# safijari/yag-slam

Hardware: AMD Instinct MI355X
Metric: pose hypotheses/sec (higher is better)
Workload: dtype u8

## Files before the change

include/yagmatch.h:

```cpp
#ifndef YAGMATCH_H
#define YAGMATCH_H

#include <stdint.h>

#ifdef __cplusplus
extern "C" {
#endif

#define YM_VERSION 1

enum {
    YM_OK = 0,
    YM_ERR_INVALID = -1,
    YM_ERR_NO_DEVICE = -2,
    YM_ERR_HIP = -3,
    YM_ERR_UNSUPPORTED = -4,
    YM_ERR_RANGE = -5,
    YM_ERR_BUSY = -6
};

enum { YM_SEM_KARTO = 0, YM_SEM_YAGPY = 1 };

typedef struct ym_config {
    double angle_variance_penalty;
// ... 11 lines not shown
    int32_t semantics;
} ym_config;

typedef struct ym_scan_desc {
    const double *ranges;
    int32_t n;
    int32_t reserved;
    double min_angle;
    double max_angle;
    double angle_increment;
    double min_range;
    double max_range;
    double range_threshold;
    double pose[3];
} ym_scan_desc;

typedef struct ym_result {
    double response;
    double pose[3];
    double cov[9];
    double coarse_response;
    int64_t hypotheses;
    int32_t coarse_dims[3];
    int32_t fine_dims[3];
    int32_t n_query_points;
    int32_t expansions;
    int32_t status;
    int32_t reserved;
} ym_result;

typedef struct ym_matcher ym_matcher;
typedef struct ym_scan ym_scan;

int ym_version(void);
const char *ym_build_id(void);
int ym_device_count(void);
const char *ym_last_error(void);

ym_matcher *ym_create(const ym_config *cfg, int device);
void ym_destroy(ym_matcher *m);
int ym_get_config(const ym_matcher *m, ym_config *out);
int ym_set_stream(ym_matcher *m, void *hip_stream);
int ym_synchronize(ym_matcher *m);

ym_scan *ym_scan_create(int device, const ym_scan_desc *desc);
int ym_scans_create(int device, const ym_scan_desc *descs, int n, ym_scan **out);
void ym_scans_destroy(ym_scan *const *scans, int n);
int ym_scan_set_pose(ym_scan *s, double x, double y, double heading);
int ym_scans_set_poses(ym_scan *const *scans, const double *xyz, int n);
int ym_scan_get_pose(const ym_scan *s, double pose[3]);
int ym_scan_size(const ym_scan *s);
int ym_scan_structure_trusted(const ym_scan *s, int semantics);
void ym_scan_destroy(ym_scan *s);

int ym_match(ym_matcher *m, const ym_scan_desc *query, const ym_scan_desc *base, int n_base,
             int penalize, int refine, ym_result *out);
int ym_match_scans(ym_matcher *m, const ym_scan *query, const ym_scan *const *base, int n_base,
                   int penalize, int refine, ym_result *out);

int ym_map_sequence(ym_matcher *m, ym_scan *const *scans, const double *odom, int n, int start, int buffer_len,
                    int penalize, int refine, int device_chain, ym_result *results, int32_t *n_done);

int ym_process_scan(ym_matcher *m, ym_scan *query, ym_scan *const *chain, int n_chain, const double *odom_last,
                    const double *odom_query, int penalize, int refine, ym_result *result);

int ym_sequence_stats(const ym_matcher *m, int64_t *segments, int64_t *faults, int64_t *sync_steps);

int ym_async_slots(const ym_matcher *m);
int ym_match_scans_async(ym_matcher *m, const ym_scan *query, const ym_scan *const *base, int n_base,
                         int penalize, int refine, int slot);
int ym_wait(ym_matcher *m, int slot, ym_result *out);

int ym_match_batch(ym_matcher *m, const ym_scan *query, const ym_scan *const *scans,
                   const int32_t *chain_offsets, int n_chains, int penalize, int refine,
                   ym_result *per_chain, ym_result *best, int32_t *best_chain);

typedef struct ym_batch ym_batch;
ym_batch *ym_batch_create(ym_matcher *m, const ym_scan *query, const ym_scan *const *scans,
                          const int32_t *chain_offsets, int n_chains);
void ym_batch_destroy(ym_batch *b);
int ym_batch_size(const ym_batch *b);
int ym_batch_run_async(ym_matcher *m, const ym_batch *b, int penalize, int refine, int slot,
                       int64_t chain_id_base, void *dev_best_out);
int ym_batch_wait(ym_matcher *m, int slot, ym_result *per_chain, ym_result *best, int32_t *best_chain);

int ym_match_pairs(ym_matcher *m, const ym_scan *const *queries, const ym_scan *const *scans,
                   const int32_t *chain_offsets, int n_items, int penalize, int refine, ym_result *per_item);
ym_batch *ym_pairs_create(ym_matcher *m, const ym_scan *const *queries, const ym_scan *const *scans,
                          const int32_t *chain_offsets, int n_items);

int ym_coarse_dims(const ym_matcher *m, int32_t dims[3]);
int ym_match_slice_begin(ym_matcher *m, const ym_scan *query, const ym_scan *const *base, int n_base, int penalize,
                         int refine, int k_begin, int k_end, double *dev_resp, double *dev_probs);
int ym_match_slice_finish(ym_matcher *m, ym_result *out);

typedef struct ym_map ym_map;
ym_map *ym_map_from_occupancy(ym_matcher *m, const uint8_t *image, int width, int height, int pitch, int occupied_value);
ym_map *ym_map_from_grid(ym_matcher *m, const double *cgrid, int width, int height);
int ym_map_size(const ym_map *map, int *width, int *height);
int ym_map_read(const ym_map *map, double *out, int64_t out_count);
void ym_map_destroy(ym_map *map);
typedef struct ym_map_search {
    double xy_search, xy_step;
    double angle_search, angle_step;
    double grid_resolution;
    int32_t penalize;
    int32_t reserved;
} ym_map_search;
int ym_match_map(ym_matcher *m, const ym_map *map, double ox, double oy, const ym_scan *const *queries, int n_queries,
                 int penalize, int refine, const ym_map_search *coarse, ym_result *out);

typedef struct ym_occupancy ym_occupancy;
typedef struct ym_occupancy_info {
    int32_t width, height;
    double offset_x, offset_y, resolution;
} ym_occupancy_info;
ym_occupancy *ym_occupancy_create(const ym_scan *const *scans, int n_scans, double resolution, double range_threshold);
int ym_occupancy_get_info(const ym_occupancy *og, ym_occupancy_info *info);
int ym_occupancy_read(const ym_occupancy *og, uint8_t *image, int64_t image_bytes);
void ym_occupancy_destroy(ym_occupancy *og);

typedef struct ym_raymap ym_raymap;
ym_raymap *ym_raymap_create(int device, const uint8_t *image, int width, int height, int pitch);
int ym_raymap_trace(ym_raymap *rm, const double *starts_xy, int n_starts, const double *dir_cs, int n_angles, float *end_xy,
                    double *length, int64_t *capped);
int ym_raymap_trace_each(ym_raymap *rm, const double *starts_xy, int n_starts, const double *dir_cs, int n_angles, float *end_xy,
                         double *length, int64_t *capped);
void ym_raymap_destroy(ym_raymap *rm);

typedef struct ym_segments ym_segments;
ym_segments *ym_segments_create(int device, const int32_t *labels, int width, int height, int pitch_elems);
int ym_segments_label_range(const ym_segments *sg, int32_t *min_label, int32_t *max_label);
int ym_segments_stats(ym_segments *sg, int n_labels, int64_t *count, int64_t *sum_x, int64_t *sum_y);
int ym_segments_boundaries(ym_segments *sg, uint8_t *mask, int64_t mask_bytes);
int ym_segments_pairs(ym_segments *sg, int table_slots, int cap, int32_t *pairs , int32_t *counts, int64_t *first_index,
                      int32_t *n_pairs);
void ym_segments_destroy(ym_segments *sg);

typedef struct ym_grid_info {
    int32_t width, height, pitch;
    int32_t origin_x, origin_y;
    int32_t storage_w, storage_h;
    int32_t roi_x, roi_y, roi_w, roi_h;
    double offset_x, offset_y;
} ym_grid_info;
int ym_debug_grid_info(ym_matcher *m, int item, ym_grid_info *info);
int ym_debug_grid(ym_matcher *m, int item, uint8_t *out, int64_t out_bytes);
int ym_debug_sums(ym_matcher *m, int item, int pass, uint32_t *out, int64_t out_count);
int ym_debug_query_local(ym_matcher *m, int item, double *out_xy, int32_t cap, int32_t *n);
int ym_debug_cells(ym_matcher *m, int item, int32_t *out, int64_t out_count, int32_t *max_n);

int ym_debug_option(ym_matcher *m, int option, int value);

#define YM_DEBUG_COUNTERS 8
int ym_debug_counters(ym_matcher *m, int64_t *out, int32_t count);

int ym_debug_stamps(ym_matcher *m, int enable, uint64_t *out, int32_t count);

int ym_profile_enable(ym_matcher *m, int on);
int ym_profile_read(ym_matcher *m, int which, double *ms_total, int64_t *launches, int reset);
int ym_cache_stats(const ym_matcher *m, int64_t *hits, int64_t *misses);

#ifdef __cplusplus
}
#endif
#endif
```

yag_slam_amd/_capi.py:

```python
import ctypes as C
import os
import subprocess

_HERE = os.path.dirname(os.path.abspath(__file__))
LIB_PATH = os.environ.get("YM_LIB_PATH") or os.path.join(_HERE, "libyagmatch.so")

YM_OK = 0
SEM = {"karto": 0, "yagpy": 1}

EXPORTS = (
    "ym_version", "ym_build_id", "ym_device_count", "ym_last_error", "ym_create", "ym_destroy", "ym_get_config",
    "ym_set_stream", "ym_synchronize", "ym_scan_create", "ym_scans_create", "ym_scans_destroy", "ym_scan_set_pose", "ym_scans_set_poses", "ym_scan_get_pose",
    "ym_scan_size", "ym_scan_structure_trusted", "ym_scan_destroy", "ym_match", "ym_match_scans", "ym_map_sequence", "ym_process_scan", "ym_sequence_stats", "ym_async_slots",
    "ym_match_scans_async", "ym_wait", "ym_match_batch", "ym_batch_create", "ym_batch_destroy", "ym_batch_size",
    "ym_match_pairs", "ym_pairs_create",
    "ym_batch_run_async", "ym_batch_wait", "ym_debug_grid_info",
    "ym_debug_grid", "ym_debug_sums", "ym_debug_query_local", "ym_debug_cells", "ym_debug_option", "ym_debug_stamps",
    "ym_profile_enable",
    "ym_profile_read", "ym_cache_stats", "ym_debug_counters",
    "ym_coarse_dims", "ym_match_slice_begin", "ym_match_slice_finish",
    "ym_occupancy_create", "ym_occupancy_get_info", "ym_occupancy_read", "ym_occupancy_destroy",
    "ym_map_from_occupancy", "ym_map_from_grid", "ym_map_size", "ym_map_read", "ym_map_destroy", "ym_match_map",
    "ym_raymap_create", "ym_raymap_trace", "ym_raymap_trace_each", "ym_raymap_destroy",
    "ym_segments_create", "ym_segments_label_range", "ym_segments_stats", "ym_segments_boundaries", "ym_segments_pairs",
    "ym_segments_destroy",
)


class YmError(RuntimeError):
    def __init__(self, code, msg):
        super().__init__("libyagmatch error %d: %s" % (code, msg))
        self.code = code


class YmConfig(C.Structure):
    _fields_ = [
        ("angle_variance_penalty", C.c_double),
        ("distance_variance_penalty", C.c_double),
        ("coarse_search_angle_offset", C.c_double),
        ("coarse_angle_resolution", C.c_double),
        ("fine_search_angle_resolution", C.c_double),
        ("range_threshold", C.c_double),
        ("minimum_angle_penalty", C.c_double),
        ("minimum_distance_penalty", C.c_double),
        ("search_size", C.c_double),
        ("resolution", C.c_double),
        ("smear_deviation", C.c_double),
        ("use_response_expansion", C.c_int32),
        ("semantics", C.c_int32),
    ]


class YmScanDesc(C.Structure):
    _fields_ = [
        ("ranges", C.POINTER(C.c_double)),
        ("n", C.c_int32),
        ("reserved", C.c_int32),
        ("min_angle", C.c_double),
        ("max_angle", C.c_double),
        ("angle_increment", C.c_double),
        ("min_range", C.c_double),
        ("max_range", C.c_double),
        ("range_threshold", C.c_double),
        ("pose", C.c_double * 3),
    ]


class YmResult(C.Structure):
    _fields_ = [
        ("response", C.c_double),
        ("pose", C.c_double * 3),
        ("cov", C.c_double * 9),
        ("coarse_response", C.c_double),
        ("hypotheses", C.c_int64),
        ("coarse_dims", C.c_int32 * 3),
        ("fine_dims", C.c_int32 * 3),
        ("n_query_points", C.c_int32),
        ("expansions", C.c_int32),
        ("status", C.c_int32),
        ("reserved", C.c_int32),
    ]


class YmOccupancyInfo(C.Structure):
    _fields_ = [("width", C.c_int32), ("height", C.c_int32), ("offset_x", C.c_double), ("offset_y", C.c_double),
                ("resolution", C.c_double)]


class YmMapSearch(C.Structure):
    _fields_ = [("xy_search", C.c_double), ("xy_step", C.c_double), ("angle_search", C.c_double), ("angle_step", C.c_double),
                ("grid_resolution", C.c_double), ("penalize", C.c_int32), ("reserved", C.c_int32)]


class YmGridInfo(C.Structure):
    _fields_ = [(n, C.c_int32) for n in ("width", "height", "pitch", "origin_x", "origin_y", "storage_w",
                                        "storage_h", "roi_x", "roi_y", "roi_w", "roi_h")] + [
        ("pad", C.c_int32), ("offset_x", C.c_double), ("offset_y", C.c_double)]


_lib = None


def build(verbose=False):
    cmd = ["make", "-C", os.path.join(_HERE, "csrc")]
    if not verbose:
        cmd.insert(1, "-s")
    subprocess.check_call(cmd)
    return LIB_PATH


def _share_hip_runtime_with_torch():
    import importlib.util
    import sys
    if "torch" in sys.modules or os.environ.get("YM_SKIP_TORCH_PRELOAD"):
        return
    if importlib.util.find_spec("torch") is not None:
        import torch


def lib():
    global _lib
    if _lib is not None:
        return _lib
    if not os.path.exists(LIB_PATH):
        build()
    _share_hip_runtime_with_torch()
    L = C.CDLL(LIB_PATH)
    vp, ip, dp = C.c_void_p, C.POINTER(C.c_int32), C.POINTER(C.c_double)
    L.ym_version.restype = C.c_int
    L.ym_device_count.restype = C.c_int
    L.ym_last_error.restype = C.c_char_p
    L.ym_build_id.restype = C.c_char_p
    L.ym_create.restype = vp
    L.ym_create.argtypes = [C.POINTER(YmConfig), C.c_int]
    L.ym_destroy.argtypes = [vp]
    L.ym_destroy.restype = None
    L.ym_get_config.argtypes = [vp, C.POINTER(YmConfig)]
    L.ym_set_stream.argtypes = [vp, vp]
    L.ym_synchronize.argtypes = [vp]
    L.ym_scan_create.restype = vp
    L.ym_scan_create.argtypes = [C.c_int, C.POINTER(YmScanDesc)]
    L.ym_scan_set_pose.argtypes = [vp, C.c_double, C.c_double, C.c_double]
    L.ym_scans_set_poses.argtypes = [C.POINTER(vp), dp, C.c_int]
    L.ym_scan_get_pose.argtypes = [vp, dp]
    L.ym_scan_size.argtypes = [vp]
    L.ym_scan_destroy.argtypes = [vp]
    L.ym_scans_create.argtypes = [C.c_int, vp, C.c_int, vp]
    L.ym_scans_destroy.argtypes = [vp, C.c_int]
    L.ym_scans_destroy.restype = None
    L.ym_scan_destroy.restype = None
    L.ym_match.argtypes = [vp, C.POINTER(YmScanDesc), C.POINTER(YmScanDesc), C.c_int, C.c_int, C.c_int,
                           C.POINTER(YmResult)]
    L.ym_match_scans.argtypes = [vp, vp, C.POINTER(vp), C.c_int, C.c_int, C.c_int, C.POINTER(YmResult)]
    L.ym_async_slots.argtypes = [vp]
    L.ym_match_scans_async.argtypes = [vp, vp, C.POINTER(vp), C.c_int, C.c_int, C.c_int, C.c_int]
    L.ym_wait.argtypes = [vp, C.c_int, C.POINTER(YmResult)]
    L.ym_match_batch.argtypes = [vp, vp, C.POINTER(vp), ip, C.c_int, C.c_int, C.c_int, C.POINTER(YmResult),
                                 C.POINTER(YmResult), ip]
    L.ym_batch_create.restype = vp
    L.ym_batch_create.argtypes = [vp, vp, C.POINTER(vp), ip, C.c_int]
    L.ym_pairs_create.restype = vp
    L.ym_pairs_create.argtypes = [vp, C.POINTER(vp), C.POINTER(vp), ip, C.c_int]
    L.ym_match_pairs.argtypes = [vp, C.POINTER(vp), C.POINTER(vp), ip, C.c_int, C.c_int, C.c_int, C.POINTER(YmResult)]
    L.ym_batch_destroy.argtypes = [vp]
    L.ym_batch_destroy.restype = None
    L.ym_batch_size.argtypes = [vp]
    L.ym_batch_run_async.argtypes = [vp, vp, C.c_int, C.c_int, C.c_int, C.c_int64, vp]
    L.ym_batch_wait.argtypes = [vp, C.c_int, C.POINTER(YmResult), C.POINTER(YmResult), ip]
    L.ym_debug_grid_info.argtypes = [vp, C.c_int, C.POINTER(YmGridInfo)]
    L.ym_debug_grid.argtypes = [vp, C.c_int, C.POINTER(C.c_uint8), C.c_int64]
    L.ym_debug_sums.argtypes = [vp, C.c_int, C.c_int, C.POINTER(C.c_uint32), C.c_int64]
    L.ym_debug_query_local.argtypes = [vp, C.c_int, dp, C.c_int32, ip]
    L.ym_debug_cells.argtypes = [vp, C.c_int, ip, C.c_int64, ip]
    L.ym_debug_option.argtypes = [vp, C.c_int, C.c_int]
    L.ym_debug_stamps.argtypes = [vp, C.c_int, C.POINTER(C.c_uint64), C.c_int32]
    L.ym_profile_enable.argtypes = [vp, C.c_int]
    L.ym_profile_read.argtypes = [vp, C.c_int, dp, C.POINTER(C.c_int64), C.c_int]
    L.ym_cache_stats.argtypes = [vp, C.POINTER(C.c_int64), C.POINTER(C.c_int64)]
    L.ym_debug_counters.argtypes = [vp, C.POINTER(C.c_int64), C.c_int32]
    L.ym_coarse_dims.argtypes = [vp, ip]
    L.ym_scan_structure_trusted.argtypes = [vp, C.c_int]
    L.ym_process_scan.argtypes = [vp, vp, C.POINTER(vp), C.c_int, dp, dp, C.c_int, C.c_int, C.POINTER(YmResult)]
    L.ym_sequence_stats.argtypes = [vp, C.POINTER(C.c_int64), C.POINTER(C.c_int64), C.POINTER(C.c_int64)]
    L.ym_map_sequence.argtypes = [vp, C.POINTER(vp), dp, C.c_int, C.c_int, C.c_int, C.c_int, C.c_int, C.c_int, C.POINTER(YmResult), ip]
    L.ym_match_slice_begin.argtypes = [vp, vp, C.POINTER(vp), C.c_int, C.c_int, C.c_int, C.c_int, C.c_int, vp, vp]
    L.ym_match_slice_finish.argtypes = [vp, C.POINTER(YmResult)]
    L.ym_occupancy_create.restype = vp
    L.ym_occupancy_create.argtypes = [C.POINTER(vp), C.c_int, C.c_double, C.c_double]
    L.ym_occupancy_get_info.argtypes = [vp, C.POINTER(YmOccupancyInfo)]
    L.ym_occupancy_read.argtypes = [vp, C.POINTER(C.c_uint8), C.c_int64]
    L.ym_occupancy_destroy.argtypes = [vp]
    L.ym_occupancy_destroy.restype = None
    L.ym_map_from_occupancy.restype = vp
    L.ym_map_from_occupancy.argtypes = [vp, C.POINTER(C.c_uint8), C.c_int, C.c_int, C.c_int, C.c_int]
    L.ym_map_from_grid.restype = vp
    L.ym_map_from_grid.argtypes = [vp, dp, C.c_int, C.c_int]
    L.ym_map_size.argtypes = [vp, ip, ip]
    L.ym_map_read.argtypes = [vp, dp, C.c_int64]
    L.ym_map_destroy.argtypes = [vp]
    L.ym_map_destroy.restype = None
    L.ym_match_map.argtypes = [vp, vp, C.c_double, C.c_double, C.POINTER(vp), C.c_int, C.c_int, C.c_int, C.POINTER(YmMapSearch),
                               C.POINTER(YmResult)]
    L.ym_raymap_create.restype = vp
    L.ym_raymap_create.argtypes = [C.c_int, C.POINTER(C.c_uint8), C.c_int, C.c_int, C.c_int]
    L.ym_raymap_trace.argtypes = [vp, dp, C.c_int, dp, C.c_int, C.POINTER(C.c_float), dp, C.POINTER(C.c_int64)]
    L.ym_raymap_trace_each.argtypes = [vp, dp, C.c_int, dp, C.c_int, C.POINTER(C.c_float), dp, C.POINTER(C.c_int64)]
    L.ym_raymap_destroy.argtypes = [vp]
    L.ym_raymap_destroy.restype = None
    lp = C.POINTER(C.c_int64)
    L.ym_segments_create.restype = vp
    L.ym_segments_create.argtypes = [C.c_int, ip, C.c_int, C.c_int, C.c_int]
    L.ym_segments_label_range.argtypes = [vp, ip, ip]
    L.ym_segments_stats.argtypes = [vp, C.c_int, lp, lp, lp]
    L.ym_segments_boundaries.argtypes = [vp, C.POINTER(C.c_uint8), C.c_int64]
    L.ym_segments_pairs.argtypes = [vp, C.c_int, C.c_int, ip, ip, lp, ip]
    L.ym_segments_destroy.argtypes = [vp]
    L.ym_segments_destroy.restype = None
    _lib = L
    return L


def build_id():
    return lib().ym_build_id().decode()


def check(rc):
    if rc != YM_OK:
        raise YmError(rc, lib().ym_last_error().decode(errors="replace"))
    return rc


def last_error():
    return lib().ym_last_error().decode(errors="replace")


def config_struct(cfg, semantics="karto"):
    d = cfg if isinstance(cfg, dict) else cfg.as_dict()
    c = YmConfig()
    for name, _ in YmConfig._fields_:
        if name == "semantics":
            c.semantics = SEM[semantics] if isinstance(semantics, str) else int(semantics)
        elif name == "use_response_expansion":
            c.use_response_expansion = int(bool(d["use_response_expansion"]))
        elif name == "minimum_distance_penalty":
            c.minimum_distance_penalty = float(d.get("minimum_distance_penalty", 0.5))
        else:
            setattr(c, name, float(d[name]))
    return c
```

yag_slam_amd/csrc/ym_abi_debug.hpp:

```cpp
int ym_debug_grid_info(ym_matcher *m, int item, ym_grid_info *info) {
    if (!m || !info) return set_err(YM_ERR_INVALID, "null argument");
    if (!m->last_valid || item < 0 || item >= m->last_B) return set_err(YM_ERR_INVALID, "no such item in the last call");
    const YmGeom &g = m->last_geom;
    info->width = g.win_w; info->height = g.win_w; info->pitch = g.pitch;
    info->origin_x = g.win_origin; info->origin_y = g.win_origin;
    info->storage_w = g.storage_w; info->storage_h = g.storage_w;
    info->roi_x = g.border; info->roi_y = g.border; info->roi_w = g.roi_w; info->roi_h = g.roi_w;
    YmItemState s;
    DEV_GUARD(m->device);
    HIP_TRY(hipStreamSynchronize(m->stream));
    HIP_TRY(hipMemcpy(&s, m->states.p + item, sizeof s, hipMemcpyDeviceToHost));
    info->offset_x = s.off_x; info->offset_y = s.off_y;
    return YM_OK;
}

int ym_debug_grid(ym_matcher *m, int item, uint8_t *out, int64_t out_bytes) {
    if (!m || !out) return set_err(YM_ERR_INVALID, "null argument");
    if (!m->last_valid || item < 0 || item >= m->last_B) return set_err(YM_ERR_INVALID, "no such item in the last call");
    const int64_t need = (int64_t)m->last_geom.pitch * m->last_geom.win_w;
    if (out_bytes < need) return set_err(YM_ERR_INVALID, "grid buffer too small: need %lld bytes", (long long)need);
    DEV_GUARD(m->device);
    HIP_TRY(hipStreamSynchronize(m->stream));
    HIP_TRY(hipMemcpy(out, m->grid.p + (size_t)item * m->last_grid_stride, (size_t)need, hipMemcpyDeviceToHost));
    return YM_OK;
}

int ym_debug_sums(ym_matcher *m, int item, int pass, uint32_t *out, int64_t out_count) {
    if (!m || !out || pass < 0 || pass > 1) return set_err(YM_ERR_INVALID, "bad argument");
    if (!m->last_valid || item < 0 || item >= m->last_B) return set_err(YM_ERR_INVALID, "no such item in the last call");
    const size_t n = m->last_sums_stride[pass];
    if (n == 0) return set_err(YM_ERR_INVALID, "pass %d did not run", pass);
    const size_t ncopy = std::min(n, (size_t)out_count);
    if (m->cfg.semantics == YM_SEM_KARTO && (size_t)out_count < n)
        return set_err(YM_ERR_INVALID, "sums buffer too small: need %zu entries", n);
    DEV_GUARD(m->device);
    HIP_TRY(hipStreamSynchronize(m->stream));
    HIP_TRY(hipMemcpy(out, m->sums.p + m->sums_pass_offset[pass] + (size_t)item * n, ncopy * sizeof(uint32_t),
                      hipMemcpyDeviceToHost));
    return YM_OK;
}

int ym_debug_query_local(ym_matcher *m, int item, double *out_xy, int32_t cap, int32_t *n) {
    if (!m || !out_xy || !n) return set_err(YM_ERR_INVALID, "null argument");
    if (!m->last_valid || item < 0 || item >= m->last_B) return set_err(YM_ERR_INVALID, "no such item in the last call");
    YmItemState s;
    DEV_GUARD(m->device);
    HIP_TRY(hipStreamSynchronize(m->stream));
    HIP_TRY(hipMemcpy(&s, m->states.p + item, sizeof s, hipMemcpyDeviceToHost));
    *n = s.nq;
    if (cap < s.nq) return set_err(YM_ERR_INVALID, "buffer too small: need %d points", s.nq);
    if (s.nq > 0)
        HIP_TRY(hipMemcpy(out_xy, s.ql, sizeof(double2) * s.nq, hipMemcpyDeviceToHost));
    return YM_OK;
}

int ym_debug_cells(ym_matcher *m, int item, int32_t *out, int64_t out_count, int32_t *max_n) {
    if (!m || !max_n) return set_err(YM_ERR_INVALID, "null argument");
    if (!m->last_valid || item < 0 || item >= m->last_B) return set_err(YM_ERR_INVALID, "no such item in the last call");
    *max_n = m->last_max_n;
    const size_t per = (size_t)m->last_max_base * m->last_max_n;
    if (!out) return YM_OK;
    if ((size_t)out_count < per * 2) return set_err(YM_ERR_INVALID, "buffer too small: need %zu ints", per * 2);
    DEV_GUARD(m->device);
    HIP_TRY(hipStreamSynchronize(m->stream));
    HIP_TRY(hipMemcpy(out, m->cells.p + (size_t)item * per, sizeof(int2) * per, hipMemcpyDeviceToHost));
    return YM_OK;
}

int ym_debug_option(ym_matcher *m, int option, int value) {
    if (m) { m->cache_gen++; m->list_key_valid = false; }
    if (!m) return set_err(YM_ERR_INVALID, "null matcher");
    if (option == 0) return set_err(YM_ERR_INVALID, "debug option 0 (an experimental correlate form) no longer exists");
    else if (option == 2) m->full_raster = value;
    else if (option == 3) m->corr_u = value;
    else if (option == 4) m->corr_pad_lds = value;
    else if (option == 5) m->corr_chunks = value;
    else if (option == 6) m->finish_form = value;
    else if (option == 9) m->corr_cw = value;
    else if (option == 10) m->select_global = value;
    else if (option == 41) m->select_split_max = value;
    else if (option == 11) m->finish_threads = value;
    else if (option == 12) m->keep_sums = value;
    else if (option == 13) m->corr_dedup = value;
    else if (option == 14) m->corr_region = value;
    else if (option == 15) m->corr_region_na = m->corr_region_nw = value;
    else if (option == 23) m->poll_completion = value != 0;
    else if (option == 24) m->use_scan_structure = value != 0;
    else if (option == 25) m->chain_margin = value;
    else if (option == 26) m->prepare_threads = value;
    else if (option == 28) {
        if (value == 0) { m->lds_min_batch = 64; m->rg_min_batch = 48; }
        else m->lds_min_batch = m->rg_min_batch = std::max(8, value);
    }
    else if (option == 42) m->rg_min_batch = value == 0 ? 48 : std::max(8, value);
    else if (option == 29) m->overlap_lists = value != 0;
    else if (option == 31) m->staged_queries = value != 0;
    else if (option == 30) m->tile_h_forced = value == YM_TILE_H || value == YM_TILE_H_TALL ? value : 0;
    else if (option == 16) m->raster_gx = value;
    else if (option == 17) m->corr_region_parts = value;
    else if (option == 21) m->corr_fuse_score = value;
    else if (option == 45) { m->list_cache_on = value != 0; m->list_key_valid = false; }
    else if (option == 46) m->yag_fast = value < 0 ? 0 : value > 2 ? 1 : value;
    else if (option == 43) m->rg2_h = value;
    else if (option == 44) {
#ifndef YM_EXPERIMENTAL
        return set_err(YM_ERR_UNSUPPORTED, "correlate_region2_kernel is compiled only into builds made with -DYM_EXPERIMENTAL");
#endif
        m->rg2_min_batch = value > 0 ? value : 1 << 30;
    }
    else if (option == 32) {
#ifndef YM_EXPERIMENTAL
        if (value >= 2) return set_err(YM_ERR_UNSUPPORTED, "correlate form %d is compiled only into builds made with -DYM_EXPERIMENTAL", value);
#endif
        m->corr_region_form = value;
    }
    else if (option == 33) m->corr_region_dbg = value;
    else if (option == 34) m->corr_region_rsplit = value;
    else if (option == 35) {
#ifndef YM_EXPERIMENTAL
        return set_err(YM_ERR_UNSUPPORTED, "correlate_item_kernel is compiled only into builds made with -DYM_EXPERIMENTAL");
#endif
        m->item_min_batch = value;
    }
    else if (option == 36) m->raster_planes_only = value;
    else if (option == 37) m->raster_no_rowtab = value;
    else if (option == 38) m->corr_region_pad_lds = value;
    else if (option == 39) m->keep_planes = value;
    else if (option == 40) m->tile_list_min_batch = value;
    else if (option == 19) m->corr_region_cap = value;
    else if (option == 20) m->corr_region_lds = value;
    else if (option == 18) m->raster_hits_per_tile = value;
    else if (option == 7) {
        m->cache_off = value == 1;
        m->cache_entries.clear();
        m->cache_index.clear();
        m->cache_used = 0;
    }
    else if (option == 8) {
        m->cache_limit = (size_t)std::max(1, value) << 10;
        HIP_TRY(hipStreamSynchronize(m->stream));
        m->cache_entries.clear();
        m->cache_index.clear();
        m->cache_used = 0;
        m->cache_arena.release();
    }
    else return set_err(YM_ERR_INVALID, "unknown option %d", option);
    return YM_OK;
}

int ym_debug_stamps(ym_matcher *m, int enable, uint64_t *out, int32_t count) {
    if (!m) return set_err(YM_ERR_INVALID, "null matcher");
    DEV_GUARD(m->device);
    HIP_TRY(hipStreamSynchronize(m->stream));
    if (out && count > 0)
        HIP_TRY(hipMemcpy(out, m->stamps.p, sizeof(uint64_t) * std::min(count, 32), hipMemcpyDeviceToHost));
    if (enable && !m->stamps_on) HIP_TRY(hipMemset(m->stamps.p, 0, 32 * sizeof(unsigned long long)));
    m->stamps_on = enable != 0;
    return YM_OK;
}

int ym_profile_enable(ym_matcher *m, int on) {
    if (!m) return set_err(YM_ERR_INVALID, "null matcher");
    m->profiling = on != 0;
    return YM_OK;
}

int ym_profile_read(ym_matcher *m, int which, double *ms_total, int64_t *launches, int reset) {
    if (!m || which < 0 || which > 2) return set_err(YM_ERR_INVALID, "bad argument");
    DEV_GUARD(m->device);
    HIP_TRY(hipStreamSynchronize(m->stream));
    int rc = prof_collect(m);
    if (rc) return rc;
    if (ms_total) *ms_total = m->prof[which].ms;
    if (launches) *launches = m->prof[which].launches;
    if (reset) { m->prof[which].ms = 0; m->prof[which].launches = 0; }
    return YM_OK;
}

int ym_sequence_stats(const ym_matcher *m, int64_t *segments, int64_t *faults, int64_t *sync_steps) {
    if (!m || !segments || !faults || !sync_steps) return set_err(YM_ERR_INVALID, "null argument");
    *segments = m->seq_segments; *faults = m->seq_faults; *sync_steps = m->seq_sync_steps;
    return YM_OK;
}

int ym_debug_counters(ym_matcher *m, int64_t *out, int32_t count) {
    if (!m || !out || count < 0) return set_err(YM_ERR_INVALID, "bad argument");
    int64_t v[YM_DEBUG_COUNTERS];
    std::memset(v, 0, sizeof v);
    if (m->yag_counters.p) {
        DEV_GUARD(m->device);
        unsigned long long c[4];
        HIP_TRY(hipStreamSynchronize(m->stream));
        HIP_TRY(hipMemcpy(c, m->yag_counters.p, sizeof c, hipMemcpyDeviceToHost));
        for (int i = 0; i < 4; i++) v[i] = (int64_t)c[i];
    }
    v[4] = m->list_cache_hits;
    v[5] = m->last_corr_form;
    for (int i = 0; i < std::min<int>(count, YM_DEBUG_COUNTERS); i++) out[i] = v[i];
    return YM_OK;
}

int ym_cache_stats(const ym_matcher *m, int64_t *hits, int64_t *misses) {
    if (!m) return set_err(YM_ERR_INVALID, "null matcher");
    if (hits) *hits = m->cache_hits;
    if (misses) *misses = m->cache_misses;
    return YM_OK;
}
```

yag_slam_amd/csrc/ym_host_call.hpp:

```cpp
int launch_call_body(ym_matcher *m, Slot &slot) {
    static const bool debug_host = getenv("YM_DEBUG_HOST") != nullptr;
    timespec t_[8];
    auto mark = [&](int i) { if (debug_host) clock_gettime(CLOCK_MONOTONIC, &t_[i]); };
    mark(7);
    DEV_GUARD(m->device);
    CallPlan P;
    int rc;
    mark(0);
    m->last_corr_form = -1;
    if ((rc = plan_sizes(m, slot, P))) return rc;
    mark(1);
    Call &pc = slot.call;
    const bool replay = pc.batch_uid != 0 && pc.plan_clean && pc.plan_gen == m->cache_gen && pc.pose_epoch == g_pose_epoch.load(std::memory_order_relaxed);
    if (!replay && (rc = plan_cache(m, slot, P))) return rc;
    mark(2);
    if ((rc = plan_jobs(m, slot, P, replay))) return rc;
    mark(3);
    if ((rc = plan_descriptor(m, slot, P, replay))) return rc;
    if (pc.batch_uid != 0 && !replay) {
        bool clean = !m->cache_off;
        for (const CallScan &cs : pc.scans) clean = clean && !cs.stale && !cs.qstale;
        pc.plan_clean = clean;
        pc.plan_gen = m->cache_gen;
    }
    mark(4);
    hipStream_t st = m->stream;
    hipEvent_t ev_call = nullptr;
    if ((rc = prof_begin(m, 2, &ev_call))) return rc;
    if ((rc = plan_raster(m, slot, P))) return rc;
    mark(5);

    timespec e_[8];
    auto emark = [&](int i) { if (debug_host) clock_gettime(CLOCK_MONOTONIC, &e_[i]); };
    emark(0);
    enqueue_prepare(m, P);
    emark(1);
    if (P.region26 && !P.yag) {
        ym_matcher::ListKey key;
        std::memset(&key, 0, sizeof key);
        const CallScan *q0 = P.n_qslots == 1 ? &slot.call.scans[slot.call.items[0].query] : nullptr;
        bool keyed = q0 && q0->id != 0 && m->list_cache_on && !P.stamps && !P.rg_ws;
        if (keyed) {
            key.qid = q0->id; key.pose[0] = q0->pose[0]; key.pose[1] = q0->pose[1]; key.pose[2] = q0->pose[2];
            key.g = P.g; key.lc = P.lc; key.nw = P.rg_nw; key.parts = P.rg_parts; key.nrx = P.rg_nrx; key.nry = P.rg_nry;
            key.rg_h = P.rg2 ? P.rg2_h : YM_RG_H; key.force = m->corr_region; key.nregions = P.rg_nregions; key.ng = P.rg_ng;
            key.es = P.rg_entries_stride; key.ss = P.rg_starts_stride;
            key.pe = m->rg_entries.p; key.ps = m->rg_starts.p; key.pb = m->rg_rbox.p;
            P.lists_cached = m->list_key_valid && std::memcmp(&key, &m->list_key, sizeof key) == 0;
        }
        if (P.lists_cached) m->list_cache_hits++;
        else { m->list_key = key; m->list_key_valid = keyed; }
    }
    const bool lists_aside = P.region26 && !P.yag && m->overlap_lists && !P.stamps && P.k_end > P.k_begin && !P.lists_cached;
    if (lists_aside && (rc = enqueue_region_lists_aside(m, P))) return rc;
    if ((rc = enqueue_select(m, P))) return rc;
    if ((rc = enqueue_raster(m, P))) return rc;
    if (lists_aside && (rc = enqueue_region_lists_joined(m, P))) return rc;
    emark(2);
    if (P.yag) {
        if ((rc = enqueue_yagpy_passes(m, slot, P))) return rc;
        emark(3); emark(4); emark(5);
    } else {
        if ((rc = enqueue_correlate(m, P))) return rc;
        emark(3);
        enqueue_score(m, slot, P);
        emark(4);
        if (!slot.call.slice) enqueue_finish(m, slot, P);
        else slot.plan = P;
        emark(5);
    }
    if (slot.dev_best_out)
        hipLaunchKernelGGL(ym::argbest_kernel, dim3(1), dim3(256), 0, st, m->states.p, P.B, (long long)slot.chain_id_base,
                           reinterpret_cast<double *>(slot.dev_best_out));
    HIP_TRY(hipGetLastError());
    if ((rc = prof_end(m, ev_call))) return rc;
    if (!slot.done) HIP_TRY(hipEventCreateWithFlags(&slot.done, hipEventDisableTiming));
    if (!slot.call.chain_step) HIP_TRY(hipEventRecord(slot.done, st));
    slot.in_flight = true;
    slot.n_items = P.B;
    HIP_TRY(hipGetLastError());
    mark(6);
    if (debug_host) {
        auto us = [&](int a, int b) { return (t_[b].tv_sec - t_[a].tv_sec) * 1e6 + (t_[b].tv_nsec - t_[a].tv_nsec) * 1e-3; };
        fprintf(stderr, "[ym] host us: guard %.1f sizes %.0f cache %.0f jobs %.0f descriptor %.0f raster-plan %.0f enqueue %.0f (B %d, %d scans)\n", us(7, 0), us(0, 1), us(1, 2),
                us(2, 3), us(3, 4), us(4, 5), us(5, 6), P.B, P.nscans);
        auto eus = [&](int a, int b) { return (e_[b].tv_sec - e_[a].tv_sec) * 1e6 + (e_[b].tv_nsec - e_[a].tv_nsec) * 1e-3; };
        fprintf(stderr, "[ym] enqueue us: prepare %.1f raster %.1f correlate %.1f score %.1f finish %.1f\n", eus(0, 1), eus(1, 2), eus(2, 3), eus(3, 4), eus(4, 5));
    }

    m->last_geom = P.g;
    m->last_lat[0] = P.lc;
    m->last_lat[1] = P.lf;
    m->last_B = P.B; m->last_max_n = P.max_n; m->last_max_base = P.max_base;
    m->last_nt_stride = P.nt_stride; m->last_dim_stride = P.dim_stride;
    m->last_grid_stride = P.grid_stride;
    m->last_sums_stride[0] = P.yag ? P.yvol : (m->keep_sums || (P.B < 8 && P.sums_c <= 65536)) ? P.sums_c : 0;
    m->last_sums_stride[1] = slot.call.refine ? (P.yag ? P.yvol : P.sums_f) : 0;
    m->last_valid = true;
    return YM_OK;
}

int launch_call(ym_matcher *m, Slot &slot) {
    const uint64_t before = m->call_counter;
    const int rc = launch_call_body(m, slot);
    if (rc != YM_OK) {
        if (m->side_stream && m->ev_join && hipEventRecord(m->ev_join, m->side_stream) == hipSuccess)
            (void)hipStreamWaitEvent(m->stream, m->ev_join, 0);
        if (m->call_counter != before)
            for (ym_matcher::CacheEntry &ce : m->cache_entries)
                if (ce.stale_in_call == m->call_counter) ce.pose[0] = ce.pose[1] = ce.pose[2] = std::nan("");
        slot.desc_live_bytes = 0;
        slot.call.plan_clean = false;
        slot.in_flight = false;
        m->list_key_valid = false;
    }
    return rc;
}

void state_to_result(const ym_matcher *m, const Slot &slot, const YmItemState &s, int expansions, int64_t prior_hyp,
                     ym_result *r) {
    std::memset(r, 0, sizeof *r);
    r->response = s.response;
    for (int i = 0; i < 3; i++) r->pose[i] = s.mean[i];
    for (int i = 0; i < 9; i++) r->cov[i] = s.cov[i];
    r->coarse_response = s.coarse_response;
    r->coarse_dims[0] = slot.coarse.nx; r->coarse_dims[1] = slot.coarse.ny; r->coarse_dims[2] = slot.coarse.nt;
    int64_t hyp = (int64_t)slot.coarse.nx * slot.coarse.ny * slot.coarse.nt;
    if (slot.call.refine) {
        r->fine_dims[0] = slot.fine.nx; r->fine_dims[1] = slot.fine.ny; r->fine_dims[2] = slot.fine.nt;
        hyp += (int64_t)slot.fine.nx * slot.fine.ny * slot.fine.nt;
    }
    if (m->cfg.semantics == YM_SEM_YAGPY) {
        for (int i = 0; i < 3; i++) { r->coarse_dims[i] = s.ydims[0][i]; r->fine_dims[i] = slot.call.refine ? s.ydims[1][i] : 0; }
        hyp = (int64_t)s.ydims[0][0] * s.ydims[0][1] * s.ydims[0][2];
        if (slot.call.refine) hyp += (int64_t)s.ydims[1][0] * s.ydims[1][1] * s.ydims[1][2];
    } else if (s.nq == 0) {
        hyp = 0;
        std::memset(r->coarse_dims, 0, sizeof r->coarse_dims);
        std::memset(r->fine_dims, 0, sizeof r->fine_dims);
    }
    r->hypotheses = prior_hyp + hyp;
    r->n_query_points = s.nq;
    r->expansions = expansions;
    r->status = s.status;
    (void)m;
}

int finish_call(ym_matcher *m, Slot &slot, ym_result *out ) {
    if (!slot.in_flight) return set_err(YM_ERR_BUSY, "slot has no call in flight");
    bool seen = false;
    if (slot.poll_serial) {
        const volatile uint32_t *flag = reinterpret_cast<const volatile uint32_t *>(slot.result.p + align_up(sizeof(YmItemState) * slot.n_items, 64));
        timespec t0, t1;
        clock_gettime(CLOCK_MONOTONIC, &t0);
        for (;;) {
            for (int spin = 0; spin < 2048 && !seen; spin++) {
                seen = *flag == slot.poll_serial;
                if (!seen) __builtin_ia32_pause();
            }
            if (seen) break;
            clock_gettime(CLOCK_MONOTONIC, &t1);
            if ((t1.tv_sec - t0.tv_sec) * 1e3 + (t1.tv_nsec - t0.tv_nsec) * 1e-6 > 2.0) break;
        }
        std::atomic_thread_fence(std::memory_order_acquire);
        slot.poll_serial = 0;
    }
    if (!seen) HIP_TRY(hipEventSynchronize(slot.done));
    slot.in_flight = false;
    const int B = slot.n_items;
    const YmItemState *hs = reinterpret_cast<const YmItemState *>(slot.result.p);
    std::vector<int> redo;
    std::vector<int64_t> prior(B, 0);
    for (int i = 0; i < B; i++) {
        state_to_result(m, slot, hs[i], 0, 0, &out[i]);
        if (m->cfg.semantics == YM_SEM_KARTO && m->cfg.use_response_expansion &&
            kt_double_equal_h(hs[i].coarse_response, 0.0))
            redo.push_back(i);
    }
    const Call base_call = slot.call;
    const int64_t nxy = (int64_t)slot.coarse.nx * slot.coarse.ny;
    const bool any_redo = !redo.empty();
    double off = m->cfg.coarse_search_angle_offset;
    for (int attempt = 1; attempt <= 3 && !redo.empty(); attempt++) {
        const int64_t prev_hyp = nxy * (int64_t)(kt_round_h(off * 2.0 / m->cfg.coarse_angle_resolution) + 1);
        off += 20.0 * YM_KT_PI / 180.0;
        Slot &s2 = m->slots[kAsyncSlots];
        if (&s2 != &slot && s2.in_flight && s2.call.slice)
            return set_err(YM_ERR_BUSY, "an angle-sliced match is in flight on this matcher: finish it (ym_match_slice_finish) first");
        Call sub;
        sub.scans = base_call.scans;
        sub.penalize = base_call.penalize;
        sub.refine = base_call.refine;
        sub.coarse_angle_off = off;
        for (int i : redo) {
            prior[i] += prev_hyp;
            sub.items.push_back(base_call.items[i]);
        }
        s2.call = sub;
// ... 150 lines not shown
```

yag_slam_amd/csrc/ym_host_enqueue.hpp:

```cpp
void enqueue_prepare(ym_matcher *m, const CallPlan &P) {
    ym::PrepareArgs a;
    a.scans = P.d_scans; a.items = P.d_items; a.g = P.g; a.lat = P.lc; a.states = m->states.p; a.qlocal = m->qlocal.p;
    a.cells = m->cells.p; a.bbox = m->bbox.p; a.ctrig = m->ctrig.p; a.hypcell = m->hypcell.p; a.probs = P.probs;
    a.max_n = P.max_n; a.max_base = P.max_base; a.nt_stride = P.nt_stride; a.dim_stride = P.dim_stride; a.stamps = P.stamps;
    a.use_inline = P.inline_desc ? 1 : 0;
    a.pad0 = 0;
    std::memset(&a.inl, 0, sizeof a.inl);
    if (a.use_inline) {
        a.inl.item = P.hi[0];
        for (int i = 0; i < P.nscans; i++) a.inl.scans[i] = P.hs[i];
    }
    a.qnp = m->qnp.p; a.jobs = P.d_jobs; a.job_slot = P.d_job_slot;
    a.fault = nullptr; a.step = 0; a.pad1 = 0;
    for (int k = 0; k < 4; k++) a.cell_box[k] = P.cell_box[k];
    if (P.chain_step) { a.fault = m->seq_fault.p; a.step = P.chain_step; }
    a.tile_max_zero = P.use_tile_list ? m->tile_max.p : nullptr;
    const size_t lds = YM_PREP_LDS_BYTES(P.max_n);
    if (P.split_prepare) {
        if (P.n_jobs > 0) hipLaunchKernelGGL(ym::points_kernel, dim3(P.n_jobs), dim3(YM_POINTS_THREADS), lds, m->stream, a);
        hipLaunchKernelGGL(ym::cells_kernel, dim3(P.max_base + 1, P.B), dim3(256), 0, m->stream, a);
    } else {
        if (P.B == 1 && m->prepare_threads != 512)
            hipLaunchKernelGGL(ym::prepare_kernel<1024>, dim3(P.max_base + 2, P.B), dim3(1024), lds, m->stream, a);
        else
// ... 11 lines not shown
                       m->cfg.smear_deviation / m->cfg.resolution);
    if (log2cap > 14 || m->select_global) {
        const size_t cap = (size_t)1 << log2cap;
        const int nb = 5;
        int rc = m->sel_scratch.ensure((size_t)P.B * cap * (3 + (nb - 1)));
        if (rc) return rc;
        ym::SelectGlobalArgs g;
        g.cells = m->cells.p; g.max_n = P.max_n; g.max_base = P.max_base; g.z2max = m->z2max; g.log2cap = log2cap;
        g.keys = m->sel_scratch.p; g.status = g.keys + (size_t)P.B * cap; g.minidx = g.status + (size_t)P.B * cap; g.nbr = g.minidx + (size_t)P.B * cap;
        HIP_TRY(hipMemsetAsync(g.keys, 0, (size_t)2 * P.B * cap * sizeof(unsigned), m->stream));
        HIP_TRY(hipMemsetAsync(g.minidx, 0xff, (size_t)P.B * cap * sizeof(unsigned), m->stream));
        const size_t lds = cap;
        hipLaunchKernelGGL(ym::select_global_kernel<5>, dim3(P.B), dim3(1024), lds, m->stream, g);
        return YM_OK;
    }
    if (m->z2max <= 1 && P.B <= m->select_split_max) {
        const size_t cap = (size_t)1 << log2cap;
        const size_t had = m->sel_tables.cap;
        int rc = m->sel_tables.ensure((size_t)2 * P.B * cap);
        if (rc) return rc;
        if (m->sel_tables.cap != had) HIP_TRY(hipMemsetAsync(m->sel_tables.p, 0, m->sel_tables.cap * sizeof(unsigned), m->stream));
        if ((rc = m->sel_rec.ensure((size_t)P.B * 12 * 1024))) return rc;
        if ((rc = m->sel_slot.ensure((size_t)P.B * pts))) return rc;
        ym::SelectSplitArgs s;
        s.cells = m->cells.p; s.max_n = P.max_n; s.max_base = P.max_base; s.log2cap = log2cap; s.pad = 0;
        s.keys = m->sel_tables.p; s.mx = s.keys + (size_t)P.B * cap; s.rec = m->sel_rec.p; s.slot_of = m->sel_slot.p; s.stamps = P.stamps;
        const dim3 grid((unsigned)((pts + YM_SELECT_SPLIT_THREADS - 1) / YM_SELECT_SPLIT_THREADS), P.B);
        hipLaunchKernelGGL(ym::select_hash_kernel, grid, dim3(YM_SELECT_SPLIT_THREADS), 0, m->stream, s);
        hipLaunchKernelGGL(ym::select_neighbours_kernel, grid, dim3(YM_SELECT_SPLIT_THREADS), 0, m->stream, s);
        hipLaunchKernelGGL(ym::select_relax_kernel, dim3(P.B), dim3(1024), cap, m->stream, s);
        return YM_OK;
    }
    ym::SelectArgs a;
    a.cells = m->cells.p; a.max_n = P.max_n; a.max_base = P.max_base; a.z2max = m->z2max; a.log2cap = log2cap; a.stamps = P.stamps;
    const size_t lds = (size_t)9 << log2cap;
    hipLaunchKernelGGL(ym::select_kernel<5>, dim3(P.B), dim3(1024), lds, m->stream, a);
    return YM_OK;
}

int enqueue_raster(ym_matcher *m, const CallPlan &P) {
    hipStream_t st = m->stream;
    const YmGeom &g = P.g;
    if (P.use_tile_list) {
        ym::TilesArgs t;
        t.bbox = m->bbox.p; t.tile_list = m->tile_list.p; t.tile_count = m->tile_count.p; t.tile_zero = m->tile_zero.p;
        t.tile_max = m->tile_max.p;
        t.hits = P.use_tile_hits ? m->tile_hits.p : nullptr; t.tile_h = P.tile_h;
        t.hit_limit = m->raster_hits_per_tile > 0 ? std::min(m->raster_hits_per_tile, YM_TILE_HITS) : YM_TILE_HITS;
        t.max_n = P.max_n; t.max_base = P.max_base; t.half_kernel = g.half_kernel;
        t.tiles_x = P.tiles_x; t.tiles_y = P.tiles_y; t.tile_cap = P.tile_cap;
        for (int k = 0; k < 4; k++) t.launch[k] = P.launch[k];
        hipLaunchKernelGGL(ym::tiles_kernel, dim3(P.B), dim3(YM_TILES_THREADS),
                           (size_t)4 * ((P.tiles_x * P.tiles_y + 31) / 32) + (P.use_tile_hits ? (size_t)8 * P.tile_cap : 0), st, t);
    }
    ym::RasterArgs a;
    a.tiles_x = P.tiles_x; a.tiles_y = P.tiles_y; a.tile_x0 = P.launch[0]; a.tile_y0 = P.launch[1]; a.ltx = P.ltx;
    a.tile_list = P.use_tile_list ? m->tile_list.p : nullptr; a.tile_count = m->tile_count.p; a.tile_cap = P.tile_cap;
    a.cells = m->cells.p; a.bbox = m->bbox.p; a.states = m->states.p; a.g = g; a.grid = m->grid.p;
    a.grid_stride = P.grid_stride; a.planes = m->planes.p; a.lut = m->ktab.p; a.max_n = P.max_n; a.max_base = P.max_base; a.stamps = P.stamps;
    a.tile_zero = m->tile_zero.p; a.sub_zero = m->sub_zero.p; a.planes_only = m->raster_planes_only;
    a.n_rowtab = m->raster_no_rowtab ? 0 : m->n_rowtab; a.rowtab = reinterpret_cast<const uint2 *>(m->rowtab.p); a.rowtab_shift = m->rowtab_shift; a.no_planes = P.win_only ? 1 : 0;
    const size_t rlds = YM_RASTER_LDS_BYTES(P.tile_h, g.half_kernel, a.n_rowtab);
    a.tile_max = m->tile_max.p; a.tile_max_host = P.use_tile_list ? m->tile_max_host : nullptr;
    a.hits = (P.use_tile_list && P.use_tile_hits) ? m->tile_hits.p : nullptr; a.lty = P.lty; a.pad0 = 0;
    int rc;
    hipEvent_t ev_k = nullptr;
    if ((rc = prof_begin(m, 1, &ev_k))) return rc;
    if (P.ltx > 0 && P.lty > 0) {
        const int hint = m->tile_max_host ? *reinterpret_cast<volatile int32_t *>(m->tile_max_host) : 0;
        const int gx = m->raster_gx > 0 ? std::min(P.ltx * P.lty, m->raster_gx)
                                        : hint > 0 ? std::min(P.ltx * P.lty, hint + hint / 8 + 2) : P.ltx * P.lty;
        a.first_overflow = gx;
        if (P.use_tile_list) {
            if (P.tile_h == YM_TILE_H_TALL) {
                hipLaunchKernelGGL((ym::raster_kernel<128, false, YM_TILE_H_TALL, true>), dim3(gx, P.B), dim3(128), rlds, st, a);
                if (gx < P.ltx * P.lty) hipLaunchKernelGGL((ym::raster_kernel<128, true, YM_TILE_H_TALL, true>), dim3(4, P.B), dim3(128), rlds, st, a);
            } else {
                hipLaunchKernelGGL((ym::raster_kernel<128, false, YM_TILE_H, true>), dim3(gx, P.B), dim3(128), rlds, st, a);
                if (gx < P.ltx * P.lty) hipLaunchKernelGGL((ym::raster_kernel<128, true, YM_TILE_H, true>), dim3(4, P.B), dim3(128), rlds, st, a);
            }
        } else {
            if (P.tile_h == YM_TILE_H_TALL) hipLaunchKernelGGL((ym::raster_kernel<256, false, YM_TILE_H_TALL, false>), dim3(P.ltx * P.lty, P.B), dim3(256), rlds, st, a);
            else hipLaunchKernelGGL((ym::raster_kernel<256, false, YM_TILE_H, false>), dim3(P.ltx * P.lty, P.B), dim3(256), rlds, st, a);
        }
    }
    return prof_end(m, ev_k);
}

int enqueue_correlate(ym_matcher *m, const CallPlan &P);
void enqueue_score(ym_matcher *m, Slot &slot, const CallPlan &P);

int enqueue_yagpy_passes(ym_matcher *m, Slot &slot, const CallPlan &P) {
    const Call &call = slot.call;
    const YmGeom &g = P.g;
    m->sums_pass_offset[0] = 0;
    m->sums_pass_offset[1] = (size_t)P.B * P.yvol;
    for (int pass = 0; pass < (call.refine ? 2 : 1); pass++) {
        ym::YagArgs a;
        std::memset(&a, 0, sizeof a);
        a.g = g; a.pass = pass; a.penalize = call.penalize; a.refine = call.refine;
        a.last = (pass == 1 || !call.refine) ? 1 : 0;
        if (pass == 0) {
            a.search_xy = m->cfg.search_size * 0.5; a.step_xy = g.res * 2;
            a.search_t = m->cfg.coarse_search_angle_offset * 0.5; a.step_t = m->cfg.coarse_angle_resolution;
        } else {
            a.search_xy = g.res * 2; a.step_xy = g.res; a.search_t = 0.0349 * 0.5; a.step_t = 0.00349;
        }
        a.coarse_angle_res = m->cfg.coarse_angle_resolution;
        a.states = m->states.p; a.host_out = reinterpret_cast<YmItemState *>(slot.result.dp);
        a.qlocal = m->qlocal.p; a.axes = m->yaxes.p; a.rot = nullptr;
        a.sums = m->sums.p + m->sums_pass_offset[pass]; a.out = m->resp.p;
        a.grid = m->grid.p; a.grid_stride = P.grid_stride; a.vol_stride = P.yvol;
        a.max_n = P.max_n; a.maxd = P.ymaxd; a.maxt = P.ymaxt;
        hipLaunchKernelGGL(ym::yag_setup_kernel, dim3(1, P.B), dim3(256), 0, m->stream, a);
        if (pass == 0 && P.lc.nx > 0) {
            a.lat_nx = P.lc.nx; a.lat_ny = P.lc.ny; a.lat_nt = P.lc.nt; a.step_cells = P.sx;
            a.nt_stride = P.nt_stride; a.dim_stride = P.dim_stride; a.ctrig = m->ctrig.p; a.hypcell = m->hypcell.p;
            a.lsums = m->sums.p + (size_t)2 * P.B * P.yvol; a.lsums_stride = P.sums_c; a.counters = m->yag_counters.p;
            hipLaunchKernelGGL(ym::yag_lattice_kernel, dim3(P.B), dim3(256), 0, m->stream, a);
            int rc = enqueue_correlate(m, P);
            if (rc) return rc;
            enqueue_score(m, slot, P);
        }
        if (pass == 1 && m->yag_fast) {
            a.fine_rows = m->yag_fast;
            a.n_items = P.B;
            if (P.B >= 64) hipLaunchKernelGGL(ym::yag_fine_kernel<64>, dim3(8 * P.ymaxt * ((P.B + 7) / 8)), dim3(64), 0, m->stream, a);
            else hipLaunchKernelGGL(ym::yag_fine_kernel<256>, dim3(8 * P.ymaxt * ((P.B + 7) / 8)), dim3(256), 0, m->stream, a);
        }
        hipLaunchKernelGGL(ym::yag_score_kernel, dim3((P.ymaxd * P.ymaxd + 255) / 256, P.ymaxt, P.B), dim3(256), 0, m->stream, a);
        if (P.B >= 16) hipLaunchKernelGGL(ym::yag_reduce_kernel<256>, dim3(P.B), dim3(256), 0, m->stream, a);
        else hipLaunchKernelGGL(ym::yag_reduce_kernel<1024>, dim3(P.B), dim3(1024), 0, m->stream, a);
    }
    return YM_OK;
}

ym::RegionArgs region_args(ym_matcher *m, const CallPlan &P) {
    ym::RegionArgs r;
    r.g = P.g; r.lat = P.lc; r.grid = m->grid.p; r.planes = m->planes.p; r.grid_stride = P.grid_stride; r.ctrig = m->ctrig.p;
    r.hypcell = m->hypcell.p; r.states = m->states.p; r.qrep = P.d_qrep; r.entries = m->rg_entries.p; r.entries_stride = P.rg_entries_stride;
    r.starts = m->rg_starts.p; r.starts_stride = P.rg_starts_stride; r.partial = m->partial.p; r.partial_stride = P.partial_stride;
    r.rbox = m->rg_rbox.p; r.rbox_stride = (size_t)P.rg_nregions * P.rg_parts; r.nw = P.rg_nw; r.parts = P.rg_parts;
    r.nt_stride = P.nt_stride; r.dim_stride = P.dim_stride; r.nrx = P.rg_nrx; r.nry = P.rg_nry; r.ng = P.rg_ng; r.nbins = P.rg_nbins;
    r.force_irregular = (m->corr_region == 2 || m->corr_region == 3) ? m->corr_region - 1 : 0; r.pad = m->corr_region_dbg; r.stamps = P.stamps;
    r.fuse_score = P.fuse_score ? 1 : 0; r.resp = P.resp; r.sums_stride = P.sums_c; r.blockmax = m->blockmax.p;
    r.probs = P.probs; r.probs_stride = (size_t)P.lc.nx * P.lc.ny; r.n_blocks = P.score_blocks;
    r.rg_h = YM_RG_H; r.rg_cls = YM_RG_CLS; r.rg_zero = YM_RG_ZERO; r.pad2 = 0;
#ifdef YM_EXPERIMENTAL
    r.rg_h = P.rg_ws ? YM_WS_H : YM_RG_H; r.rg_cls = P.rg_ws ? YM_WS_CLS : P.rg_item ? YM_IT_CLS : YM_RG_CLS;
    r.rg_zero = P.rg_ws ? YM_WS_ZERO : P.rg_item ? YM_IT_ZERO : YM_RG_ZERO;
#endif
    if (P.rg2) { r.rg_h = P.rg2_h; r.rg_cls = YM_RG_PITCH * (P.rg2_h + 26); r.rg_zero = 4 * r.rg_cls; }
    r.pad2 = ((1 << 21) + r.rg_h - 1) / r.rg_h;
    r.rg_w = 0; r.rg_pitch = YM_RG_PITCH; r.nregions = P.rg_nregions; r.pad3 = 0;
    r.walk = m->rg_walk.p; r.nitems = P.B; r.rsplit = P.rg_rsplit; r.pad4 = 0;
    r.lnw = P.rg_lnw; r.lparts = P.rg_lparts; r.entries_pstride = P.rg_entries_pstride;
    r.gpx = std::max(1, std::min((2 * std::max(m->n_cus, 8) / 8) / std::max(1, P.rg_parts), (P.B + 7) / 8));
    return r;
}

int enqueue_region_lists(ym_matcher *m, const CallPlan &P, hipStream_t st) {
    const ym::RegionArgs r = region_args(m, P);
#ifdef YM_EXPERIMENTAL
    if (P.rg_lparts == 1 && P.rg_lnw == P.lc.nt && (P.rg_ws || P.rg2 || P.rg_item || P.rg_pool)) {
        const size_t bin_lds = YM_BIN_LDS_BYTES(P.rg_nbins, P.rg_entries_stride, P.rg_nregions * P.rg_parts);
        if (bin_lds > m->bin_lds_limit) {
            HIP_TRY(hipFuncSetAttribute(reinterpret_cast<const void *>(ym::bin_whole_kernel<false>), hipFuncAttributeMaxDynamicSharedMemorySize, (int)bin_lds));
            m->bin_lds_limit = bin_lds;
        }
        hipLaunchKernelGGL(ym::bin_whole_kernel<false>, dim3(P.n_qslots), dim3(YM_BIN_THREADS), bin_lds, st, r);
        if (P.rg_ws) hipLaunchKernelGGL(ym::region_walk_kernel, dim3(P.rg_parts, P.n_qslots), dim3(64), 0, st, r);
        return YM_OK;
    }
#endif
    const size_t bin_lds = YM_BINP_LDS_BYTES(P.rg_nbins, P.rg_entries_pstride, P.rg_nregions);
    if (bin_lds > m->binp_lds_limit) {
#define YM_BINP_ATTR(Y, M) HIP_TRY(hipFuncSetAttribute(reinterpret_cast<const void *>(ym::bin_kernel<Y, M>), hipFuncAttributeMaxDynamicSharedMemorySize, (int)bin_lds))
        YM_BINP_ATTR(false, 18); YM_BINP_ATTR(false, 32); YM_BINP_ATTR(false, 64); YM_BINP_ATTR(true, 18); YM_BINP_ATTR(true, 32); YM_BINP_ATTR(true, 64);
#undef YM_BINP_ATTR
        m->binp_lds_limit = bin_lds;
    }
    const int per_thread = (P.rg_lnw * P.max_n + YM_BINP_THREADS - 1) / YM_BINP_THREADS;
    const dim3 bgrid(P.rg_lparts, P.n_qslots);
#define YM_BINP_LAUNCH(Y, M) hipLaunchKernelGGL((ym::bin_kernel<Y, M>), bgrid, dim3(YM_BINP_THREADS), bin_lds, st, r)
    if (P.yag) { if (per_thread <= 18) YM_BINP_LAUNCH(true, 18); else if (per_thread <= 32) YM_BINP_LAUNCH(true, 32); else YM_BINP_LAUNCH(true, 64); }
    else { if (per_thread <= 18) YM_BINP_LAUNCH(false, 18); else if (per_thread <= 32) YM_BINP_LAUNCH(false, 32); else YM_BINP_LAUNCH(false, 64); }
#undef YM_BINP_LAUNCH
    return YM_OK;
}

int enqueue_region_lists_aside(ym_matcher *m, CallPlan &P) {
    if (!m->side_stream) {
        HIP_TRY(hipStreamCreateWithFlags(&m->side_stream, hipStreamNonBlocking));
        pool_register_stream(m->device, m->side_stream, true);
        HIP_TRY(hipEventCreateWithFlags(&m->ev_fork, hipEventDisableTiming));
        HIP_TRY(hipEventCreateWithFlags(&m->ev_join, hipEventDisableTiming));
    }
    HIP_TRY(hipEventRecord(m->ev_fork, m->stream));
    return YM_OK;
}
int enqueue_region_lists_joined(ym_matcher *m, CallPlan &P) {
    HIP_TRY(hipStreamWaitEvent(m->side_stream, m->ev_fork, 0));
    int rc = enqueue_region_lists(m, P, m->side_stream);
    if (rc) return rc;
    HIP_TRY(hipEventRecord(m->ev_join, m->side_stream));
    P.lists_on_side_stream = true;
    return YM_OK;
}

int enqueue_correlate(ym_matcher *m, const CallPlan &P) {
    hipStream_t st = m->stream;
    ym::CorrArgs a;
    a.g = P.g; a.lat = P.lc; a.grid = m->grid.p; a.grid_stride = P.grid_stride; a.planes = m->planes.p; a.ctrig = m->ctrig.p;
    a.qlocal = m->qlocal.p; a.hypcell = m->hypcell.p; a.states = m->states.p; a.partial = m->partial.p; a.partial_stride = P.partial_stride;
    a.max_n = P.max_n; a.nt_stride = P.nt_stride; a.dim_stride = P.dim_stride; a.chunk = P.chunk; a.n_chunks = P.n_chunks;
    a.ngx = P.ngx; a.nx_pad = P.nx_pad; a.sx = P.sx; a.stamps = P.stamps; a.tpb = P.tpb; a.cw = P.cw;
    a.k_begin = P.k_begin; a.nk = std::max(0, P.k_end - P.k_begin);
    a.dedup = P.dedup; a.pad2 = 0;
    if (a.nk == 0) return YM_OK;
    int rc;
    hipEvent_t ev_k = nullptr;
    m->last_corr_form = P.region26 ? 1 : P.region ? 2 : 0;
    if (P.region26) {
        const ym::RegionArgs r = region_args(m, P);
        if (P.lists_on_side_stream) HIP_TRY(hipStreamWaitEvent(st, m->ev_join, 0));
        else if (!P.lists_cached && (rc = enqueue_region_lists(m, P, st))) return rc;
        if ((rc = prof_begin(m, 0, &ev_k))) return rc;
        const dim3 rgrid(P.rg_parts * P.rg_rsplit, P.B);
#ifdef YM_EXPERIMENTAL
        if (P.rg2) {
            const size_t lds = (size_t)r.rg_zero + 26 * YM_RG_PITCH + 32 + (size_t)m->corr_region_pad_lds;
            if (lds > m->rg2_lds_limit) {
                const int want = 144 * 1024;
                HIP_TRY(hipFuncSetAttribute(reinterpret_cast<const void *>(ym::correlate_region2_kernel<80>), hipFuncAttributeMaxDynamicSharedMemorySize, want));
                HIP_TRY(hipFuncSetAttribute(reinterpret_cast<const void *>(ym::correlate_region2_kernel<100>), hipFuncAttributeMaxDynamicSharedMemorySize, want));
                HIP_TRY(hipFuncSetAttribute(reinterpret_cast<const void *>(ym::correlate_region2_kernel<128>), hipFuncAttributeMaxDynamicSharedMemorySize, want));
                m->rg2_lds_limit = (size_t)want;
            }
            if (P.rg2_h == 80) hipLaunchKernelGGL(ym::correlate_region2_kernel<80>, rgrid, dim3(64 * YM_R2_NW), lds, st, r);
            else if (P.rg2_h == 100) hipLaunchKernelGGL(ym::correlate_region2_kernel<100>, rgrid, dim3(64 * YM_R2_NW), lds, st, r);
            else hipLaunchKernelGGL(ym::correlate_region2_kernel<128>, rgrid, dim3(64 * YM_R2_NW), lds, st, r);
            return prof_end(m, ev_k);
        }
#endif
#ifdef YM_EXPERIMENTAL
        if (P.rg_item) {
            const size_t lds = YM_IT_ACC_BYTES(P.lc.nt);
            if (!m->item_lds_set) {
                HIP_TRY(hipFuncSetAttribute(reinterpret_cast<const void *>(ym::correlate_item_kernel), hipFuncAttributeMaxDynamicSharedMemorySize, (int)YM_IT_ACC_BYTES(YM_IT_MAX_NT)));
                m->item_lds_set = true;
            }
            hipLaunchKernelGGL(ym::correlate_item_kernel, dim3(P.B), dim3(64 * YM_IT_NW), lds, st, r);
            return prof_end(m, ev_k);
        }
        if (P.rg_pool) {
            if (P.win_only) hipLaunchKernelGGL(ym::correlate_pool_kernel<true>, rgrid, dim3(64 * YM_PL_NW), 0, st, r);
            else hipLaunchKernelGGL(ym::correlate_pool_kernel<false>, rgrid, dim3(64 * YM_PL_NW), 0, st, r);
            return prof_end(m, ev_k);
        }
        if (P.rg_ws) {
            hipLaunchKernelGGL(ym::correlate_region_ws_kernel, dim3(8 * r.gpx * P.rg_parts), dim3(64 * (YM_WS_NG + YM_WS_NL)), 0, st, r);
            hipLaunchKernelGGL(ym::region_percell_kernel, rgrid, dim3(64 * YM_WS_NG), 0, st, r);
            return prof_end(m, ev_k);
        }
#endif
        switch (P.rg_nw) {
        case 4: hipLaunchKernelGGL(ym::correlate_region_kernel<4>, rgrid, dim3(256), 0, st, r); break;
        case 5: hipLaunchKernelGGL(ym::correlate_region_kernel<5>, rgrid, dim3(320), 0, st, r); break;
        case 6: hipLaunchKernelGGL(ym::correlate_region_kernel<6>, rgrid, dim3(384), 0, st, r); break;
        case 7: hipLaunchKernelGGL(ym::correlate_region_kernel<7>, rgrid, dim3(448), 0, st, r); break;
        case 10: hipLaunchKernelGGL(ym::correlate_region_kernel<10>, rgrid, dim3(640), 0, st, r); break;
        case 11: hipLaunchKernelGGL(ym::correlate_region_kernel<11>, rgrid, dim3(704), 0, st, r); break;
        case 16: hipLaunchKernelGGL(ym::correlate_region_kernel<16>, rgrid, dim3(1024), 0, st, r); break;
        default:
            if (P.win_only) hipLaunchKernelGGL((ym::correlate_region_kernel<8, true>), rgrid, dim3(512), (size_t)m->corr_region_pad_lds, st, r);
            else hipLaunchKernelGGL(ym::correlate_region_kernel<8>, rgrid, dim3(512), (size_t)m->corr_region_pad_lds, st, r);
            break;
        }
        return prof_end(m, ev_k);
    }
    if (P.region) {
        ym::GatherArgs r;
        std::memset(&r, 0, sizeof r);
        r.g = P.g; r.lat = P.lc; r.grid = m->grid.p; r.planes = m->planes.p; r.grid_stride = P.grid_stride; r.ctrig = m->ctrig.p;
        r.hypcell = m->hypcell.p; r.states = m->states.p; r.qrep = P.d_qrep;
        r.units = m->ga_units.p; r.units_stride = P.ga_units_stride; r.starts = m->ga_starts.p; r.starts_stride = P.ga_starts_stride;
        r.work = m->ga_work.p; r.work_stride = P.ga_work_stride; r.counters = m->ga_counters.p; r.lane_job = m->ga_lane_job.p;
        r.partial = m->partial.p; r.partial_stride = P.partial_stride; r.nt_stride = P.nt_stride; r.dim_stride = P.dim_stride;
        r.W = P.ga_W; r.H = P.ga_H; r.P = P.ga_P; r.rows = P.ga_rows; r.nrx = P.ga_nrx; r.nry = P.ga_nry; r.nseg = P.ga_nseg; r.NP = P.ga_np;
        r.ng = P.ga_ng; r.parts = P.ga_parts; r.kpp = P.ga_kpp; r.unit_cap = P.ga_cap;
        r.force_irregular = (m->corr_region == 2 || m->corr_region == 3) ? m->corr_region - 1 : 0; r.stamps = P.stamps;
        r.sums = P.yag ? m->sums.p + (size_t)2 * P.B * P.yvol : m->keep_sums ? m->sums.p : nullptr; r.resp = P.resp; r.sums_stride = P.sums_c; r.blockmax = m->blockmax.p;
        r.probs = P.probs; r.probs_stride = (size_t)P.lc.nx * P.lc.ny; r.n_blocks = P.score_blocks;
        HIP_TRY(hipMemsetAsync(m->ga_counters.p, 0, (size_t)P.n_qslots * 4 * P.ga_nbins2 * YM_GA_CLS * sizeof(uint32_t), st));
        const dim3 pgrid(((unsigned)P.lc.nt * P.max_n + YM_GBIN_THREADS - 1) / YM_GBIN_THREADS, P.n_qslots);
        hipLaunchKernelGGL(ym::gbin_pieces_kernel<false>, pgrid, dim3(YM_GBIN_THREADS), 0, st, r);
        hipLaunchKernelGGL(ym::gbin_scan_kernel, dim3(P.n_qslots), dim3(1024), 0, st, r);
        hipLaunchKernelGGL(ym::gbin_pieces_kernel<true>, pgrid, dim3(YM_GBIN_THREADS), 0, st, r);
        if (P.ga_lds > m->ga_lds_limit) {
            const int want = (int)std::min<size_t>(160 * 1024, P.ga_lds);
#ifdef YM_EXPERIMENTAL
#define YM_GA_512(NA, NP) reinterpret_cast<const void *>(ym::gather_kernel<NA, NP, YM_GA_PER, 512>)
#else
#define YM_GA_512(NA, NP) reinterpret_cast<const void *>(ym::gather_kernel<NA, NP, YM_GA_PER>)
#endif
            const void *kernels[21] = {
#define YM_GA_BOTH(NA, NP) reinterpret_cast<const void *>(ym::gather_kernel<NA, NP, YM_GA_PER>), YM_GA_512(NA, NP), reinterpret_cast<const void *>(ym::gather_percell_kernel<NA, NP>)
                YM_GA_BOTH(1, 1), YM_GA_BOTH(2, 1), YM_GA_BOTH(3, 1), YM_GA_BOTH(4, 1), YM_GA_BOTH(1, 2), YM_GA_BOTH(2, 2), YM_GA_BOTH(1, 3)};
#undef YM_GA_BOTH
#undef YM_GA_512
            for (const void *k : kernels) HIP_TRY(hipFuncSetAttribute(k, hipFuncAttributeMaxDynamicSharedMemorySize, want));
            m->ga_lds_limit = P.ga_lds;
        }
        if ((rc = prof_begin(m, 0, &ev_k))) return rc;
        const dim3 rgrid(P.ga_parts, P.B), rblock(64 * P.ga_nwv);
#ifdef YM_EXPERIMENTAL
#define YM_GA_LAUNCH_512(NA, NP) if (P.ga_nwv <= 8 && m->corr_region_form == 6) hipLaunchKernelGGL((ym::gather_kernel<NA, NP, YM_GA_PER, 512>), rgrid, rblock, P.ga_lds, st, r); else
#else
#define YM_GA_LAUNCH_512(NA, NP)
#endif
#define YM_GA_LAUNCH(NA, NP)                                                                                               \
    do {                                                                                                                   \
        YM_GA_LAUNCH_512(NA, NP)                                                                                           \
        hipLaunchKernelGGL((ym::gather_kernel<NA, NP, YM_GA_PER>), rgrid, rblock, P.ga_lds, st, r);                        \
        hipLaunchKernelGGL((ym::gather_percell_kernel<NA, NP>), rgrid, rblock, P.ga_lds, st, r);                           \
    } while (0)
        if (P.ga_np == 1) {
            if (P.ga_na == 1) YM_GA_LAUNCH(1, 1);
            else if (P.ga_na == 2) YM_GA_LAUNCH(2, 1);
            else if (P.ga_na == 3) YM_GA_LAUNCH(3, 1);
            else YM_GA_LAUNCH(4, 1);
        } else if (P.ga_np == 2) {
            if (P.ga_na == 1) YM_GA_LAUNCH(1, 2);
            else YM_GA_LAUNCH(2, 2);
        } else YM_GA_LAUNCH(1, 3);
#undef YM_GA_LAUNCH
#undef YM_GA_LAUNCH_512
        return prof_end(m, ev_k);
    }
    if ((rc = prof_begin(m, 0, &ev_k))) return rc;
    const dim3 grid_dim(P.job_blocks, a.nk * P.n_groups, P.B);
    const size_t pad_lds = (size_t)m->corr_pad_lds;
    {
#define YM_CORR_LAUNCH(SX, U, CW) hipLaunchKernelGGL((ym::correlate_kernel<SX, U, CW>), grid_dim, dim3(YM_CORR_THREADS), pad_lds, st, a)
#define YM_CORR_BY_CW(SX, U)                                  \
    do {                                                      \
        if (P.cw == 4) YM_CORR_LAUNCH(SX, U, 4);              \
        else if (P.cw == 2) YM_CORR_LAUNCH(SX, U, 2);         \
        else YM_CORR_LAUNCH(SX, U, 1);                        \
    } while (0)
        if (P.sx == 2 && P.corr_u == 16) YM_CORR_BY_CW(2, 16);
        else if (P.sx == 2 && P.corr_u == 32) YM_CORR_BY_CW(2, 32);
        else if (P.sx == 2) YM_CORR_LAUNCH(2, 48, 1);
        else YM_CORR_BY_CW(1, 16);
#undef YM_CORR_BY_CW
#undef YM_CORR_LAUNCH
    }
    return prof_end(m, ev_k);
}

void enqueue_score(ym_matcher *m, Slot &slot, const CallPlan &P) {
    hipStream_t st = m->stream;
    const YmLattice &lc = P.lc;
    if (!P.yag) {
        m->sums_pass_offset[0] = 0;
        m->sums_pass_offset[1] = (size_t)P.B * P.sums_c;
    }
    ym::ScoreArgs a;
    a.g = P.g; a.lat = lc; a.partial = m->partial.p; a.partial_stride = P.partial_stride; a.states = m->states.p;
    a.sums = (m->keep_sums || (P.B < 8 && P.sums_c <= 65536)) ? m->sums.p : nullptr;
    if (P.yag) a.sums = m->sums.p + (size_t)2 * P.B * P.yvol;
    a.sums_stride = P.sums_c; a.resp = P.resp; a.blockmax = m->blockmax.p;
    a.n_chunks = P.n_groups; a.nx_pad = P.nx_pad; a.n_blocks = P.score_blocks; a.stamps = P.stamps;
    a.probs = P.probs; a.probs_stride = (size_t)lc.nx * lc.ny;
    a.k_begin = P.k_begin; a.k_end = P.k_end; a.lane_layout = P.region26 ? 1 : 0;
// ... 45 lines not shown
```

yag_slam_amd/csrc/ym_host_matcher.hpp:

```cpp
struct ym_map {
    int device;
    int width, height;
    double *d_cgrid;
    uint8_t *d_g8;
};

struct ym_occupancy {
    int device;
    ym_occupancy_info info;
    std::vector<uint8_t> image;
};

struct ym_batch {
    std::vector<const ym_scan *> queries;
    std::vector<int32_t> item_query;
    std::vector<const ym_scan *> scans;
    std::vector<int32_t> offsets;
    mutable std::vector<int> cache_hints;
    mutable std::vector<int> query_hints;
    uint64_t uid = 0;
};

struct ym_matcher {
    ym_config cfg;
    int device;
    hipStream_t own_stream, stream;
    hipStream_t side_stream = nullptr;
    hipEvent_t ev_fork = nullptr, ev_join = nullptr;
    bool overlap_lists = true;
    bool staged_queries = true;
    int tile_h_forced = 0;
    int sticky_tall_left = 0;
    int tall_pattern = 0;
    bool tall_alternates = false;
    int tall_tiles_min_window = 768;
    YmGeom geom;
    std::vector<uint8_t> kernel;
    std::vector<double> kernel_f;
    DevBuf<double> kernel_f_dev;
    DevBuf<double2> map_pts;
    int z2max = 0;
    DevBuf<uint8_t> ktab;
    DevBuf<uint8_t> rowtab;
    int n_rowtab = 0, rowtab_shift = -1;
    DevBuf<unsigned char> desc_dev;
    DevBuf<YmItemState> states;
    DevBuf<double2> qlocal;
    DevBuf<int32_t> qnp;
    DevBuf<unsigned char> tmp_cache;
    DevBuf<int2> cells;
    DevBuf<int4> bbox;
    DevBuf<uint8_t> grid;
    DevBuf<uint8_t> planes;
    DevBuf<uint8_t> tile_zero;
    DevBuf<uint8_t> sub_zero;
    size_t tz_sig[6] = {0, 0, 0, 0, 0, 0};
    std::vector<std::array<int, 4>> item_dirty;
    int tz_covered = 0;
    std::vector<unsigned char> planes_stale;
    DevBuf<double2> ctrig;
    DevBuf<int32_t> foffsets;
    DevBuf<int32_t> hypcell;
    DevBuf<uint16_t> partial;
    DevBuf<uint16_t> rg_entries;
    DevBuf<int32_t> rg_starts;
    DevBuf<uint32_t> rg_rbox;
    DevBuf<uint32_t> rg_walk;
    int n_cus = 0;
    size_t bin_lds_limit = 64 * 1024;
    size_t binp_lds_limit = 64 * 1024;
    int chain_margin = 1;
    uint64_t cache_gen = 1;
    int64_t seq_segments = 0, seq_faults = 0, seq_sync_steps = 0;
    int lds_min_batch = 64;
    int rg_min_batch = 48;
    int prepare_threads = 0;
    int last_wh = 0;
    bool use_scan_structure = true;
    bool poll_completion = true;
    int corr_region_nw = 0;
    int item_min_batch = 1 << 30;
    bool item_lds_set = false;
    int raster_planes_only = 0;
    int raster_no_rowtab = 0;
    int corr_region_rsplit = 0;
    int tile_list_min_batch = 48;
    int keep_planes = 0;
    int corr_region_pad_lds = 0;
    int corr_region_dbg = 0;
    int corr_region_form = 0;
    struct ListKey {
        uint64_t qid; double pose[3]; YmGeom g; YmLattice lc;
        int32_t nw, parts, nrx, nry, rg_h, force, nregions, ng; size_t es, ss; const void *pe, *ps, *pb;
    };
    ListKey list_key;
    bool list_key_valid = false, list_cache_on = true;
    int64_t list_cache_hits = 0;
    int rg2_min_batch = 1 << 30;
    int rg2_h = 128;
    size_t rg2_lds_limit = 0;
    int corr_fuse_score = 0;
    DevBuf<uint32_t> ga_units;
    DevBuf<int32_t> ga_starts;
    DevBuf<int32_t> ga_work;
    DevBuf<uint32_t> ga_counters;
    DevBuf<uint32_t> ga_lane_job;
    std::vector<uint32_t> ga_lane_job_host;
    size_t ga_lds_limit = 64 * 1024;
    DevBuf<uint32_t> sums;
    DevBuf<double> resp;
    DevBuf<double> blockmax;
    DevBuf<double> probs;
    int yag_fast = 1;
    int last_corr_form = -1;
    DevBuf<unsigned long long> yag_counters;
    DevBuf<double> yaxes;
    DevBuf<double2> yrot;
    DevBuf<double> seq_pose;
    DevBuf<int32_t> seq_fault;
    PinnedBuf seq_results;
    DevBuf<unsigned long long> stamps;
    bool stamps_on = false;
    int corr_u = 0;
    int full_raster = 0;
    struct CacheEntry { uint64_t id; size_t off; int n; double pose[3]; uint64_t stale_in_call; };
    uint64_t call_counter = 0;
    std::vector<CacheEntry> cache_entries;
    std::unordered_map<uint64_t, int> cache_index;
    DevBuf<unsigned char> cache_arena;
    size_t cache_used = 0;
    size_t cache_limit = (size_t)16 << 30;
    int cache_off = 0;
    int64_t cache_hits = 0, cache_misses = 0;
    DevBuf<unsigned> sel_scratch;
    DevBuf<unsigned> sel_tables;
    DevBuf<uint4> sel_rec;
    DevBuf<unsigned> sel_slot;
    DevBuf<uint32_t> tile_list;
    DevBuf<int32_t> tile_count;
    DevBuf<int32_t> tile_max;
    DevBuf<uint16_t> tile_hits;
    int32_t *tile_max_host = nullptr;
    int finish_form = 0;
    int corr_chunks = 0;
    int corr_pad_lds = 0;
    int corr_cw = 0;
    int corr_dedup = 0;
    int corr_region = 0;
    int corr_region_na = 0;
    int corr_region_parts = 0;
    int corr_region_cap = 0;
    int corr_region_lds = 0;
    int raster_gx = 0;
    int raster_hits_per_tile = 0;
    int keep_sums = 0;
    int finish_threads = 0;
    int select_global = 0;
    int select_split_max = 8;
    DevBuf<double> tmp_ranges;
    PinnedBuf tmp_ranges_host;
    Slot slots[kAsyncSlots + 1];
    YmGeom last_geom;
    YmLattice last_lat[2];
    int last_B = 0, last_max_n = 0, last_max_base = 0, last_nt_stride = 0, last_dim_stride = 0;
    size_t last_grid_stride = 0, last_sums_stride[2] = {0, 0};
    size_t sums_pass_offset[2] = {0, 0};
    bool last_valid = false;
    bool profiling = false;
    ProfEvents prof[3];
};
```

yag_slam_amd/csrc/ym_host_plan.hpp:

```cpp
int plan_sizes(ym_matcher *m, Slot &slot, CallPlan &P) {
    Call &call = slot.call;
    P.B = (int)call.items.size();
    P.nscans = (int)call.scans.size();
    if (P.B <= 0) return set_err(YM_ERR_INVALID, "empty call");
    const int B = P.B;
    YmGeom &g = P.g;
    g = m->geom;
    double rq = 0;
    for (const CallItem &it : call.items) {
        P.max_base = std::max(P.max_base, it.base_count);
        rq = std::max(rq, call.scans[it.query].max_valid);
    }
    for (const CallScan &s : call.scans) P.max_n = std::max(P.max_n, s.n);
    const int max_n = P.max_n, max_base = P.max_base;
    const bool wrap = g.semantics == YM_SEM_KARTO && rq > m->cfg.range_threshold;
    g.kpitch = wrap ? (g.storage_w + 7) / 8 * 8 : 0;
    if (max_n > YM_MAX_BEAMS) return set_err(YM_ERR_UNSUPPORTED, "scan has %d readings; limit is %d", max_n, YM_MAX_BEAMS);

    const bool yag = P.yag = g.semantics == YM_SEM_YAGPY;
    P.chain_step = call.chain_step;
    const double coarse_off = yag ? 0.5 * m->cfg.search_size : 0.5 * (g.side - 1) * g.res;
    const double coarse_step = 2 * g.res;
    YmLattice &lc = P.lc, &lf = P.lf;
    if (yag) {
        std::memset(&lc, 0, sizeof lc);
        std::memset(&lf, 0, sizeof lf);
        lc.step_x = lc.step_y = coarse_step;
        lc.angle_res = m->cfg.coarse_angle_resolution;
        lf.fine = 1;
        if (m->yag_fast) {
            lc.nx = lc.ny = (int)std::floor(m->cfg.search_size / coarse_step + 1e-6) + 1;
            lc.nt = (int)std::floor(m->cfg.coarse_search_angle_offset / m->cfg.coarse_angle_resolution + 1e-6) + 1;
            lc.off_x = lc.off_y = coarse_off;
            lc.angle_off = 0.5 * m->cfg.coarse_search_angle_offset;
            if (lc.nx > YM_YAG_MAX_DIM || lc.nt > YM_MAX_COARSE_NT) lc.nx = lc.ny = lc.nt = 0;
        }
    } else {
        lc = make_lattice(g, coarse_off, coarse_step, call.coarse_angle_off, m->cfg.coarse_angle_resolution, 0,
                          call.penalize);
        lf = make_lattice(g, coarse_step * 0.5, g.res, 0.5 * m->cfg.coarse_angle_resolution,
                          m->cfg.fine_search_angle_resolution, 1, call.penalize);
    }
    slot.coarse = lc;
    slot.fine = lf;

    const int centre = g.border + (g.roi_w - 1) / 2;
    const double reach = rq + coarse_off + (yag ? 3 : 1) * g.res;
    int wh = (int)std::ceil(reach / g.res) + 3;
    wh = (wh + 63) / 64 * 64;
    if (m->last_wh >= wh && m->last_wh - wh <= 256) wh = m->last_wh;
    m->last_wh = wh;
    wh = wrap ? centre : std::min(wh, centre);
    g.win_origin = centre - wh;
    g.win_w = std::min(2 * wh + 1 + (yag ? 1 : 0), g.storage_w - g.win_origin);
    if (wrap) { g.win_origin = 0; g.win_w = g.storage_w; }
    {
        bool tall = B >= 512 && g.win_w >= m->tall_tiles_min_window;
        if (tall) {
            if (m->tall_pattern == 2) m->tall_alternates = true;
            m->tall_pattern = 1;
            m->sticky_tall_left = m->tall_alternates ? 64 : 0;
        } else if (g.win_w >= m->tall_tiles_min_window && !call.chain_step) {
            if (m->tall_pattern == 1) m->tall_pattern = 2;
            if (m->sticky_tall_left > 0) { tall = true; m->sticky_tall_left--; }
        }
        P.tile_h = m->tile_h_forced ? m->tile_h_forced : tall ? YM_TILE_H_TALL : YM_TILE_H;
    }
    P.tiles_x = (g.win_w + YM_TILE_W - 1) / YM_TILE_W;
    P.tiles_y = (g.win_w + P.tile_h - 1) / P.tile_h;
    g.pitch = P.tiles_x * YM_TILE_W + 64;
    P.grid_stride = align_up((size_t)g.pitch * g.win_w + 64, 256);
    if ((double)g.pitch * g.win_w > 2.0e9) return set_err(YM_ERR_UNSUPPORTED, "correlation window too large");
    if (lf.nx > 64 || lf.ny > 64 || lf.nt > YM_MAX_FINE_NT || (int64_t)lf.nx * lf.ny * lf.nt > YM_MAX_FINE_HYP)
        return set_err(YM_ERR_UNSUPPORTED, "fine lattice %dx%dx%d exceeds the built-in limit", lf.nx, lf.ny, lf.nt);
    if (lc.nt > YM_MAX_COARSE_NT)
        return set_err(YM_ERR_UNSUPPORTED, "%d coarse angles exceed the built-in limit of %d", lc.nt, YM_MAX_COARSE_NT);

    P.sx = yag ? 2 : (int)kt_round_h(lc.step_x * g.scale);
    if (P.sx != 1 && P.sx != 2) return set_err(YM_ERR_UNSUPPORTED, "coarse lattice step of %d cells", P.sx);
    P.ymaxd = yag ? std::max(8, (int)std::ceil(m->cfg.search_size / coarse_step) + 2) : 0;
    P.ymaxt = yag ? std::max(13, (int)std::ceil(m->cfg.coarse_search_angle_offset / m->cfg.coarse_angle_resolution) + 2) : 0;
    if (yag && (P.ymaxd > YM_YAG_MAX_DIM || P.ymaxt > YM_YAG_MAX_NT))
        return set_err(YM_ERR_UNSUPPORTED, "yagpy lattice %d x %d x %d exceeds the built-in limit", P.ymaxd, P.ymaxd, P.ymaxt);
    P.yvol = (size_t)P.ymaxt * P.ymaxd * P.ymaxd;
    const int G = 16;
    P.ngx = (lc.nx + G - 1) / G;
    P.nx_pad = P.ngx * G;
    const int njobs = P.njobs = lc.ny * P.ngx;
    P.tpb = 1;
    P.ktiles = lc.nt;
    P.cw = m->corr_cw > 0 ? m->corr_cw : njobs <= 64 ? 4 : njobs <= 128 ? 2 : 1;
    P.job_blocks = (njobs + (4 / P.cw) * 64 - 1) / ((4 / P.cw) * 64);
    const double waves_one_chunk = (double)((njobs + 63) / 64) * lc.nt * B;
    int n_chunks = (int)std::ceil(2048.0 / std::max(1.0, waves_one_chunk));
    n_chunks = std::max(1, std::min(n_chunks, (max_n + 31) / 32));
    n_chunks = std::max(n_chunks, (max_n + 511) / 512);
    if (njobs <= 128) n_chunks = std::max(n_chunks, (max_n + 63) / 64);
    if (m->corr_chunks > 0) n_chunks = std::max(m->corr_chunks, (max_n + 511) / 512);
    int chunk = (max_n + n_chunks - 1) / n_chunks;
    P.corr_u = m->corr_u > 0 ? m->corr_u : (chunk <= 32 && njobs <= 128 ? 32 : 16);
    chunk = (chunk + P.corr_u - 1) / P.corr_u * P.corr_u;
    while (P.cw > 1 && P.cw * chunk > 640) P.cw /= 2;
    if (P.corr_u == 48) P.cw = 1;
    P.job_blocks = (njobs + (4 / P.cw) * 64 - 1) / ((4 / P.cw) * 64);
    P.chunk = chunk;
    P.n_chunks = (max_n + chunk - 1) / chunk;
    P.n_groups = (P.n_chunks + P.cw - 1) / P.cw;
    {
        const double spacing = call.scans[call.items[0].query].beam_spacing;
        const bool likely = spacing > 0 && spacing < 0.6 * g.res;
        P.dedup = (!wrap && P.sx == 2 && chunk == 64 && (m->corr_dedup ? m->corr_dedup == 1 : likely)) ? 1 : 0;
    }

    {
        const int half_w = (g.win_w + 1) / 2;
        P.rg_nw = m->corr_region_nw > 0 ? std::min(m->corr_region_nw, 16) : lc.nt <= 8 ? lc.nt : 8;
        if (P.rg_nw < 4 || P.rg_nw == 9 || (P.rg_nw > 11 && P.rg_nw != 16)) P.rg_nw = lc.nt <= 4 ? 4 : 8;
        P.rg_parts = (lc.nt + P.rg_nw - 1) / P.rg_nw;
        int rg_h = YM_RG_H;
#ifdef YM_EXPERIMENTAL
        P.rg_ws = m->corr_region_nw == 0 && m->corr_region_form == 2;
        if (P.rg_ws) {
            P.rg_nw = YM_WS_NG;
            P.rg_parts = (lc.nt + YM_WS_NG - 1) / YM_WS_NG;
        }
        P.rg2 = !P.rg_ws && m->corr_region_nw == 0 && !m->keep_planes && lc.nt > 0 &&
                (m->corr_region_form == 5 || (m->corr_region_form == 0 && B >= m->rg2_min_batch && 3 * B >= 2 * m->n_cus));
        P.rg2_h = m->rg2_h == 80 ? 80 : m->rg2_h == 100 ? 100 : 128;
        if (P.rg2) { P.rg_nw = lc.nt <= 8 ? lc.nt : 8; P.rg_parts = (lc.nt + P.rg_nw - 1) / P.rg_nw; }
        rg_h = P.rg_ws ? YM_WS_H : P.rg2 ? P.rg2_h : YM_RG_H;
#endif
        P.rg_nrx = (half_w + YM_RG_W - 1) / YM_RG_W;
        P.rg_nry = (half_w + rg_h - 1) / rg_h;
        P.rg_nregions = P.rg_nrx * P.rg_nry;
        P.rg_ng = ((max_n * 23 + 19) / 20 + YM_RG_FLUSH - 1) / YM_RG_FLUSH;
        P.rg_nbins = P.rg_nregions * lc.nt;
        P.region26 = !wrap && (!yag || lc.nx > 0) && !P.dedup && !call.slice && P.sx == 2 && B >= m->rg_min_batch && m->corr_region != 1 && m->corr_region != 4 && lc.nx <= 2 * YM_RG_G &&
                     lc.ny <= 32 && P.rg_ng <= 8 && (int64_t)lc.nt * max_n <= YM_RG_MAX_ENTRIES && P.rg_nbins < YM_RG_MAX_BINS && max_n < 2048 &&
                     half_w <= 4096;
        if (P.region26) {
            P.rg_rsplit = 1;
            if (!P.rg_ws && !P.rg2 && m->corr_region_rsplit != 1 && m->corr_region_form != 3 && m->corr_region_form != 4) {
                const int blocks = B * P.rg_parts;
                P.rg_rsplit = m->corr_region_rsplit > 1 ? m->corr_region_rsplit : std::max(1, std::min(8, (3 * m->n_cus) / std::max(1, blocks)));
            }
            P.n_groups = P.rg_ng * P.rg_rsplit;
#ifdef YM_EXPERIMENTAL
            P.rg_item = !P.rg_ws && !P.rg2 && P.rg_rsplit == 1 && lc.nt <= YM_IT_MAX_NT && m->corr_region_form != 1 &&
                        (m->corr_region_form == 3 || B >= m->item_min_batch);
            P.n_groups = P.rg_ng * P.rg_rsplit * (P.rg2 ? YM_R2_MAX_WPA : 1);
            P.rg_pool = !P.rg_ws && !P.rg2 && !P.rg_item && P.rg_rsplit == 1 && m->corr_region_form == 4 && lc.nt <= 2 * YM_PL_MAX_NK && m->corr_region_nw == 0;
            if (P.rg_pool) {
                P.rg_nw = lc.nt <= YM_PL_MAX_NK ? lc.nt : (lc.nt + 1) / 2;
                P.rg_parts = (lc.nt + P.rg_nw - 1) / P.rg_nw;
            }
#endif
            P.win_only = !P.rg_ws && !P.rg_item && (P.rg_nw == 8 || P.rg_pool || P.rg2) && !m->keep_planes;
            const bool whole = P.rg_ws || P.rg2 || P.rg_item || P.rg_pool;
            P.rg_lnw = whole ? lc.nt : P.rg_nw;
            P.rg_lparts = whole ? 1 : P.rg_parts;
            P.rg_nbins = P.rg_nregions * P.rg_lnw;
            P.rg_entries_pstride = std::min((size_t)YM_RG_MAX_ENTRIES, ((size_t)P.rg_lnw * max_n * 11 / 10 + 63) / 64 * 64);
            P.rg_entries_stride = P.rg_entries_pstride * P.rg_lparts;
            P.rg_starts_stride = ((size_t)P.rg_lparts * (P.rg_nbins + 1) + P.rg_lparts + 15) / 16 * 16;
        }
    }
    P.region = !wrap && !P.region26 && (!yag || lc.nx > 0) && !call.slice && P.sx == 2 && B >= m->lds_min_batch && m->corr_region != 1 && lc.nx <= 16 * YM_GA_MAX_SEG && lc.ny <= 64;
    if (P.region) {
        std::vector<std::vector<uint32_t>> groups;
        P.ga_nseg = (lc.nx + YM_GA_G - 1) / YM_GA_G;
        for (int sgm = 0; sgm < P.ga_nseg; sgm++) {
            groups.emplace_back();
            for (int r = 0; r < std::min(lc.ny, 32); r++) groups.back().push_back((uint32_t)r | (uint32_t)sgm << 8 | 1u << 16);
        }
        if (lc.ny > 32) {
            const int tn = lc.ny - 32, per = 32 / tn;
            for (int sgm = 0; sgm < P.ga_nseg; sgm++) {
                if (sgm % per == 0) groups.emplace_back();
                for (int r = 32; r < lc.ny; r++) groups.back().push_back((uint32_t)r | (uint32_t)sgm << 8 | 1u << 16);
            }
        }
        P.ga_np = ((int)groups.size() + 1) / 2;
        std::vector<uint32_t> tab((size_t)P.ga_np * 64);
        for (int w = 0; w < P.ga_np; w++)
            for (int l = 0; l < 64; l++) {
                const size_t gi = (size_t)2 * w + l / 32;
                uint32_t v = groups[2 * w][0] & 0xffffu;
                if (gi < groups.size()) v = (size_t)(l % 32) < groups[gi].size() ? groups[gi][l % 32] : (groups[gi][0] & 0xffffu);
                tab[(size_t)w * 64 + l] = v;
            }
        if (P.ga_np > YM_GA_MAX_NP) P.region = false;
        if (P.region && tab != m->ga_lane_job_host) {
            int rc2 = m->ga_lane_job.ensure(tab.size());
            if (rc2) return rc2;
            HIP_TRY(hipStreamSynchronize(m->stream));
            HIP_TRY(hipMemcpy(m->ga_lane_job.p, tab.data(), tab.size() * sizeof(uint32_t), hipMemcpyHostToDevice));
            m->ga_lane_job_host = tab;
        }
    }
    if (P.region) {
        int parts = m->corr_region_parts > 0 ? m->corr_region_parts : (lc.nt + 7) / 8;
        parts = std::min(parts, lc.nt);
        const int na_max = P.ga_np == 1 ? 4 : P.ga_np == 2 ? 2 : 1;
        for (;; parts++) {
            P.ga_kpp = (lc.nt + parts - 1) / parts;
            P.ga_na = m->corr_region_na > 0 ? std::min(na_max, m->corr_region_na) : 1;
            if ((P.ga_kpp + P.ga_na - 1) / P.ga_na > 16 && m->corr_region_na <= 0) P.ga_na = na_max;
            P.ga_nwv = (P.ga_kpp + P.ga_na - 1) / P.ga_na;
            if (P.ga_nwv <= 16) break;
        }
        if (P.ga_nwv == 7) P.ga_nwv = 8;
        P.ga_parts = (lc.nt + P.ga_kpp - 1) / P.ga_kpp;
        P.ga_cap = std::min(64 * P.ga_nwv, m->corr_region_cap > 0 ? (m->corr_region_cap + 63) / 64 * 64 : 512);
        const int per = YM_GA_PER;
        const int blocks_per_cu = std::max(1, std::min(3, 32 / P.ga_nwv));
        const size_t budget = m->corr_region_lds > 0 ? (size_t)m->corr_region_lds : (size_t)(160 * 1024) / blocks_per_cu - 512;
        const int tasks = per * 64 * P.ga_nwv;
        const int half_w = (g.win_w + 1) / 2;
        double best = 1e300;
        for (int nrx = 1; nrx <= 256; nrx++) {
            const int W = (half_w + nrx - 1) / nrx;
            if (nrx > 1 && (half_w + nrx - 2) / (nrx - 1) == W) continue;
            const int cpr = (W + YM_GA_G * P.ga_nseg + 3 + 15) / 16, Pp = 16 * cpr + 8;
            for (int nry = 1; nry <= 256; nry++) {
                const int H = (half_w + nry - 1) / nry, rows = H + lc.ny;
                const int rows_lds = (tasks + cpr - 1) / cpr + 1;
                if (cpr * rows > tasks || (size_t)Pp * rows > 65528 || YM_GA_LDS_BYTES(Pp, rows_lds, P.ga_cap, P.ga_kpp) > budget) continue;
                const double cost = (double)nrx * nry * Pp * rows;
                if (cost < best) { best = cost; P.ga_W = W; P.ga_H = H; P.ga_P = Pp; P.ga_rows = rows_lds; P.ga_nrx = nrx; P.ga_nry = nry; }
                break;
            }
        }
        if (best == 1e300) P.region = false;
    }
    if (P.region) {
        P.ga_lds = YM_GA_LDS_BYTES(P.ga_P, P.ga_rows, P.ga_cap, P.ga_kpp);
        const size_t epi = (size_t)lc.nx * lc.ny * 16 + (size_t)P.ga_kpp * ((lc.nx * lc.ny + YM_SCORE_THREADS - 1) / YM_SCORE_THREADS) * 8;
        P.ga_lds = std::max(P.ga_lds, epi + 64);
        P.ga_ng = max_n / (YM_GA_FLUSH - 16) + 1;
        P.ga_nbins2 = P.ga_nrx * P.ga_nry * 4 * lc.nt * 2;
        P.ga_units_stride = ((size_t)lc.nt * max_n + 128 + 63) / 64 * 64;
        P.ga_starts_stride = ((size_t)2 * P.ga_nbins2 + 1 + 64 + 15) / 16 * 16;
        P.ga_work_stride = 1 + 3 * ((size_t)P.ga_nrx * P.ga_nry * 4 + P.ga_units_stride / P.ga_cap + 1);
        P.n_groups = P.ga_ng;
    }
    {
        static const bool debug_plan = getenv("YM_DEBUG_PLAN") != nullptr;
        if (debug_plan)
            fprintf(stderr, "[ym] B %d region %d gather %d W %d H %d P %d rows %d nrx %d nry %d nseg %d np %d parts %d kpp %d na %d nwv %d lds %zu max_n %d nx %d ny %d nt %d\n",
                    B, (int)P.region26, (int)P.region, P.ga_W, P.ga_H, P.ga_P, P.ga_rows, P.ga_nrx, P.ga_nry, P.ga_nseg, P.ga_np, P.ga_parts, P.ga_kpp, P.ga_na,
                    P.ga_nwv, P.ga_lds, max_n, lc.nx, lc.ny, lc.nt);
    }

    P.nt_stride = lc.nt;
    P.dim_stride = std::max(lc.nx, lc.ny);
    P.sums_c = (size_t)lc.nt * lc.ny * lc.nx;
    P.sums_f = (size_t)lf.nt * lf.ny * lf.nx;
    P.partial_stride = P.region26 ? (size_t)P.n_groups * lc.nt * 64 * 16 : P.region ? (size_t)P.ga_ng * lc.nt * P.ga_np * 64 * 16 : (size_t)P.n_groups * lc.nt * lc.ny * P.nx_pad;
    P.cell_blocks = (lc.nx * lc.ny + YM_SCORE_THREADS - 1) / YM_SCORE_THREADS;
    P.score_blocks = P.cell_blocks * lc.nt;

    int rc;
    if ((rc = m->states.ensure(B))) return rc;
    if ((rc = m->qlocal.ensure((size_t)B * max_n))) return rc;
    if ((rc = m->qnp.ensure(B))) return rc;
    if ((rc = m->cells.ensure((size_t)B * max_base * max_n))) return rc;
    if ((rc = m->bbox.ensure((size_t)B * max_base * YM_N_BOXES(max_n)))) return rc;
    size_t window_slack = YM_RG_WINDOW_SLACK(g.pitch), planes_slack = YM_RG_PLANES_SLACK(g.pitch / 2);
#ifdef YM_EXPERIMENTAL
    window_slack = std::max(window_slack, YM_R2_WINDOW_SLACK(g.pitch, 128));
    planes_slack = std::max(planes_slack, YM_WS_PLANES_SLACK(g.pitch / 2));
#endif
    if ((rc = m->grid.ensure((size_t)B * P.grid_stride + window_slack))) return rc;
    if ((rc = m->planes.ensure((size_t)B * P.grid_stride + std::max(planes_slack, YM_GA_PLANES_SLACK(g.pitch / 2, std::max(P.ga_rows, P.ga_nry + P.ga_H), lc.ny, P.ga_P))))) return rc;
    if ((rc = m->ctrig.ensure((size_t)B * P.nt_stride))) return rc;
    if ((rc = m->foffsets.ensure((size_t)B * lf.nt * max_n))) return rc;
    if ((rc = m->hypcell.ensure((size_t)B * 2 * P.dim_stride))) return rc;
    if ((rc = m->partial.ensure((size_t)B * P.partial_stride + 16))) return rc;
    if ((rc = m->sums.ensure((size_t)B * std::max(P.sums_c + P.sums_f, 2 * P.yvol + (yag ? P.sums_c : 0))))) return rc;
    if ((rc = m->resp.ensure((size_t)B * std::max(P.sums_c, P.yvol)))) return rc;
    if (yag) {
        if (!m->yag_counters.p) {
            if ((rc = m->yag_counters.ensure(8))) return rc;
            HIP_TRY(hipMemsetAsync(m->yag_counters.p, 0, m->yag_counters.cap * sizeof(unsigned long long), m->stream));
        }
        if ((rc = m->yaxes.ensure((size_t)B * 3 * YM_YAG_MAX_DIM))) return rc;
    }
    if ((rc = m->blockmax.ensure((size_t)B * P.score_blocks))) return rc;
    if ((rc = m->probs.ensure((size_t)B * lc.nx * lc.ny))) return rc;
    P.resp = call.ext_resp ? call.ext_resp : m->resp.p;
    P.probs = call.ext_probs ? call.ext_probs : m->probs.p;
    P.fuse_score = P.region26 && !P.rg_ws && P.rg_rsplit == 1 && !m->keep_sums && m->corr_fuse_score != 2 && !yag;
    P.k_begin = call.slice ? std::max(0, call.k_begin) : 0;
    P.k_end = call.slice ? std::min(lc.nt, call.k_end) : lc.nt;
    if (call.slice && (yag || B != 1)) return set_err(YM_ERR_UNSUPPORTED, "angle-sliced matches are single Karto matches");
    P.stamps = m->stamps_on ? m->stamps.p : nullptr;
    return YM_OK;
}

int plan_cache(ym_matcher *m, Slot &slot, const CallPlan &P) {
    Call &call = slot.call;
    const int n = (int)call.scans.size();
    for (CallScan &s : call.scans) {
        s.cache = s.qcache = nullptr;
        s.stale = s.qstale = 0;
        s.direct = m->use_scan_structure && s.gov && s.cidx && std::fabs(s.pose[0]) < YM_CHAIN_POSE_LIMIT && std::fabs(s.pose[1]) < YM_CHAIN_POSE_LIMIT &&
                   std::fabs(s.pose[2]) < YM_CHAIN_HEADING_LIMIT;
    }
    if (m->cache_off) return YM_OK;
    const uint64_t this_call = ++m->call_counter;
    std::vector<unsigned char> role(n, 0);
    for (const CallItem &it : call.items) {
        for (int j = 0; j < it.base_count; j++) role[it.base_begin + j] |= 1;
        if (P.B >= 8 && call.scans[it.query].query_uses > 0) role[it.query] |= 2;
    }
    struct Want { int scan, kind; };
    std::vector<Want> wants;
    for (int i = 0; i < n; i++) {
        if (call.scans[i].id == 0 || call.scans[i].n <= 0) continue;
        if ((role[i] & 1) && !(P.B < 8 && call.scans[i].direct)) wants.push_back(Want{i, 0});
        if (role[i] & 2) wants.push_back(Want{i, 1});
    }
    auto bytes_of = [](const CallScan &s, int kind) { return align_up(kind ? YM_QCACHE_BYTES(s.n) : YM_CACHE_BYTES(s.n), 16); };
    for (int attempt = 0; attempt < 2; attempt++) {
        size_t need = 0;
        std::vector<int> found(wants.size(), -1);
        for (size_t w = 0; w < wants.size(); w++) {
            CallScan &s = call.scans[wants[w].scan];
            const uint64_t key = s.id * 2 + wants[w].kind;
            const int hint = wants[w].kind ? s.qcache_hint : s.cache_hint;
            int e = -1;
            if (hint >= 0 && (size_t)hint < m->cache_entries.size() && m->cache_entries[hint].id == key)
                e = hint;
            else {
                auto it = m->cache_index.find(key);
                if (it != m->cache_index.end()) e = it->second;
            }
            if (e >= 0 && m->cache_entries[e].n != s.n) e = -1;
            found[w] = e;
            if (e < 0) need += bytes_of(s, wants[w].kind);
        }
        if (m->cache_used + need > m->cache_arena.cap) {
            if (attempt == 0 && need <= m->cache_limit) {
                size_t want = std::max(m->cache_used + need, 2 * m->cache_arena.cap);
                if (want > m->cache_limit) want = std::max(need, std::min(m->cache_limit, 2 * need));
                m->cache_entries.clear();
                m->cache_index.clear();
                m->cache_used = 0;
                m->cache_gen++;
                if (want > m->cache_arena.cap) {
                    HIP_TRY(hipStreamSynchronize(m->stream));
                    int rc = m->cache_arena.ensure(want);
                    if (rc) return rc;
                }
                continue;
            }
        }
        for (size_t w = 0; w < wants.size(); w++) {
            CallScan &s = call.scans[wants[w].scan];
            const int kind = wants[w].kind;
            const uint64_t key = s.id * 2 + kind;
            int e = found[w];
            int stale = 0;
            if (e < 0) {
                auto it = m->cache_index.find(key);
                if (it != m->cache_index.end()) e = it->second;
            }
            if (e < 0) {
                const size_t bytes = bytes_of(s, kind);
                if (m->cache_used + bytes > m->cache_arena.cap) continue;
                e = (int)m->cache_entries.size();
                m->cache_entries.push_back(ym_matcher::CacheEntry{key, m->cache_used, s.n, {s.pose[0], s.pose[1], s.pose[2]}, this_call});
                m->cache_index.emplace(key, e);
                m->cache_used += bytes;
                stale = 1;
                m->cache_misses++;
            } else {
                ym_matcher::CacheEntry &ce = m->cache_entries[e];
                if (ce.stale_in_call == this_call) {
                    stale = 1;
                } else if (ce.pose[0] != s.pose[0] || ce.pose[1] != s.pose[1] || ce.pose[2] != s.pose[2]) {
                    ce.pose[0] = s.pose[0]; ce.pose[1] = s.pose[1]; ce.pose[2] = s.pose[2];
                    ce.stale_in_call = this_call;
                    stale = 1;
                    m->cache_misses++;
                } else {
                    m->cache_hits++;
                }
            }
            unsigned char *p = m->cache_arena.p + m->cache_entries[e].off;
            if (kind) { s.qcache = p; s.qstale = stale; s.qcache_hint = e; }
            else { s.cache = p; s.stale = stale; s.cache_hint = e; }
            if (stale) m->cache_gen++;
        }
        break;
    }
    return YM_OK;
}

int plan_jobs(ym_matcher *m, Slot &slot, CallPlan &P, bool replay = false) {
    Call &call = slot.call;
    P.split_prepare = P.B >= 8;
    if (!P.split_prepare) return YM_OK;
    const int n = (int)call.scans.size();
    auto ensure_lists = [&](int n_q) {
        int rc;
        if (P.region26) {
            if ((rc = m->rg_entries.ensure((size_t)n_q * P.rg_entries_stride))) return rc;
            if ((rc = m->rg_starts.ensure((size_t)n_q * P.rg_starts_stride))) return rc;
            if ((rc = m->rg_rbox.ensure((size_t)n_q * P.rg_nregions * P.rg_parts))) return rc;
#ifdef YM_EXPERIMENTAL
            if (P.rg_ws && (rc = m->rg_walk.ensure((size_t)n_q * P.rg_parts * YM_WS_WALK_WORDS))) return rc;
#endif
        }
        if (P.region) {
            if ((rc = m->ga_units.ensure((size_t)n_q * P.ga_units_stride))) return rc;
            if ((rc = m->ga_starts.ensure((size_t)n_q * P.ga_starts_stride))) return rc;
            if ((rc = m->ga_work.ensure((size_t)n_q * P.ga_parts * P.ga_work_stride))) return rc;
            if ((rc = m->ga_counters.ensure((size_t)n_q * 4 * P.ga_nbins2 * YM_GA_CLS))) return rc;
        }
        return (int)YM_OK;
    };
    if (replay) {
        P.jobs = call.plan_jobs; P.job_slot = call.plan_job_slot; P.qrep = call.plan_qrep;
        P.n_jobs = (int)P.jobs.size();
// ... 227 lines not shown
```

yag_slam_amd/csrc/ym_host_types.hpp:

```cpp
struct ScanStage;

namespace {

thread_local std::string g_err;

std::atomic<uint64_t> g_pose_epoch{1};

int set_err(int code, const char *fmt, ...) {
    char buf[512];
    va_list ap;
    va_start(ap, fmt);
    vsnprintf(buf, sizeof buf, fmt, ap);
    va_end(ap);
    g_err = buf;
    return code;
}

#define HIP_TRY(expr)                                                                          \
    do {                                                                                       \
        hipError_t e_ = (expr);                                                                \
        if (e_ != hipSuccess)                                                                  \
            return set_err(YM_ERR_HIP, "%s failed: %s (%s:%d)", #expr, hipGetErrorString(e_),  \
                           __FILE__, __LINE__);                                                \
    } while (0)

double kt_round_h(double v) { return v >= 0.0 ? std::floor(v + 0.5) : std::ceil(v - 0.5); }
bool kt_double_equal_h(double a, double b) {
    double d = a - b;
    return d < 0.0 ? d >= -YM_KT_TOLERANCE : d <= YM_KT_TOLERANCE;
}
size_t align_up(size_t v, size_t a) { return (v + a - 1) / a * a; }

constexpr int kAsyncSlots = 64;

struct DevGuard {
    int prev = -1, dev;
    bool ok = true;
    explicit DevGuard(int d) : dev(d) {
        if (hipGetDevice(&prev) != hipSuccess) prev = -1;
        if (prev != dev) ok = hipSetDevice(dev) == hipSuccess;
    }
    ~DevGuard() {
        if (prev >= 0 && prev != dev) (void)hipSetDevice(prev);
    }
    DevGuard(const DevGuard &) = delete;
    DevGuard &operator=(const DevGuard &) = delete;
};
#define DEV_GUARD(d)                                                                     \
    DevGuard dev_guard_(d);                                                              \
    if (!dev_guard_.ok) return set_err(YM_ERR_HIP, "cannot make device %d current", (d))

template <typename T>
struct DevBuf {
    T *p = nullptr;
    size_t cap = 0;
    int ensure(size_t n) {
        if (n <= cap) return YM_OK;
        if (p) (void)hipFree(p);
        p = nullptr;
        cap = 0;
        size_t want = n + n / 4 + 64;
        HIP_TRY(hipMalloc(reinterpret_cast<void **>(&p), want * sizeof(T)));
        cap = want;
        return YM_OK;
    }
    void release() {
        if (p) (void)hipFree(p);
        p = nullptr;
        cap = 0;
    }
};

struct PinnedBuf {
    unsigned char *p = nullptr;
    unsigned char *dp = nullptr;
    size_t cap = 0;
    int ensure(size_t n) {
        if (n <= cap) return YM_OK;
        if (p) (void)hipHostFree(p);
        p = dp = nullptr;
        cap = 0;
        size_t want = align_up(n + n / 4 + 256, 256);
        HIP_TRY(hipHostMalloc(reinterpret_cast<void **>(&p), want, hipHostMallocMapped));
        HIP_TRY(hipHostGetDevicePointer(reinterpret_cast<void **>(&dp), p, 0));
        cap = want;
        return YM_OK;
    }
    void release() {
        if (p) (void)hipHostFree(p);
        p = dp = nullptr;
        cap = 0;
    }
};

struct CallScan {
    const double *d_ranges;
    int n;
    double min_angle, angle_inc, min_range, range_threshold;
    double pose[3];
    double max_valid;
    double lbox[4];
    double wbox[4];
    double beam_spacing = 0;
    uint64_t id = 0;
    int cache_hint = -1;
    unsigned char *cache = nullptr;
    int stale = 0;
    ScanStage *staged = nullptr;
    int qcache_hint = -1;
    unsigned char *qcache = nullptr;
    int qstale = 0;
    uint32_t query_uses = 1;
    const int32_t *gov = nullptr;
    const int32_t *cidx = nullptr;
    int cnp = 0;
    bool direct = false;
    const double *pose_dev = nullptr;
};

struct CallItem {
    int query;
    int base_begin, base_count;
    int qslot = 0;
};

struct Call {
    std::vector<CallScan> scans;
    std::vector<CallItem> items;
    int penalize = 1, refine = 1;
    double coarse_angle_off = 0;
    int expansions = 0;
    int k_begin = 0, k_end = -1;
    double *ext_resp = nullptr, *ext_probs = nullptr;
    bool slice = false;
    uint64_t batch_uid = 0, pose_epoch = 0, plan_gen = 0;
    bool plan_clean = false;
    std::vector<int32_t> plan_jobs, plan_job_slot, plan_qrep;
    int plan_want[4] = {0, 0, -1, -1};
    int plan_want_geom[3] = {0, 0, 0};
    bool plan_want_valid = false;
    int chain_step = 0;
    double *chain_pose_out = nullptr;
    double chain_next_diff[3] = {0, 0, 0};
    YmItemState *chain_out = nullptr;
};

struct CallPlan {
    int B = 0, nscans = 0, max_n = 1, max_base = 1;
    int tile_h = YM_TILE_H;
    bool lists_cached = false;
    bool lists_on_side_stream = false;
    bool yag = false;
    YmGeom g;
    YmLattice lc, lf;
    int tiles_x = 0, tiles_y = 0;
    size_t grid_stride = 0;
    int sx = 2, ngx = 0, nx_pad = 0, njobs = 0, tpb = 1, job_blocks = 0, ktiles = 0, n_chunks = 1, chunk = 0, corr_u = 16;
    int dedup = 0;
    int cw = 1, n_groups = 1;
    bool region26 = false;
    bool fuse_score = false;
    int rg_nrx = 0, rg_nry = 0, rg_ng = 1, rg_nbins = 0, rg_nw = 7, rg_parts = 1, rg_nregions = 0;
    int rg_rsplit = 1;
    bool rg_item = false;
    bool rg_pool = false;
    bool win_only = false;
    bool rg_ws = false;
    bool rg2 = false;
    int rg2_h = 0;
    size_t rg_entries_stride = 0, rg_starts_stride = 0, rg_entries_pstride = 0;
    int rg_lnw = 0, rg_lparts = 1;
    bool region = false;
    int ga_W = 0, ga_H = 0, ga_P = 0, ga_rows = 0, ga_nrx = 0, ga_nry = 0, ga_nseg = 1, ga_np = 1, ga_ng = 1, ga_parts = 1, ga_kpp = 1;
    int ga_na = 1, ga_nwv = 1, ga_cap = 512, ga_nbins2 = 0, n_qslots = 1;
    size_t ga_units_stride = 0, ga_starts_stride = 0, ga_work_stride = 0, ga_lds = 0;
    std::vector<int32_t> qrep;
    const int32_t *d_qrep = nullptr;
    int ymaxd = 0, ymaxt = 0;
    size_t yvol = 0;
    int nt_stride = 0, dim_stride = 0, score_blocks = 0, cell_blocks = 0;
    size_t sums_c = 0, sums_f = 0, partial_stride = 0;
    size_t scans_bytes = 0, desc_bytes = 0;
    bool inline_desc = false;
    YmScanRef *hs = nullptr;
    YmItem *hi = nullptr;
    const YmScanRef *d_scans = nullptr;
    const YmItem *d_items = nullptr;
    int launch[4] = {0, 0, -1, -1}, ltx = 0, lty = 0, tile_cap = 1;
    int chain_step = 0;
    int cell_box[4] = {INT32_MIN, INT32_MIN, INT32_MAX, INT32_MAX};
    bool use_tile_list = false;
    bool use_tile_hits = false;
    unsigned long long *stamps = nullptr;
    bool split_prepare = false;
    int n_jobs = 0;
    std::vector<int32_t> jobs, job_slot;
    double *resp = nullptr, *probs = nullptr;
    int k_begin = 0, k_end = 0;
    const int32_t *d_jobs = nullptr, *d_job_slot = nullptr;
};

struct Slot {
    PinnedBuf desc;
    DevBuf<unsigned char> desc_dev;
    size_t desc_live_bytes = 0;
    PinnedBuf result;
    hipEvent_t done = nullptr;
    bool in_flight = false;
    Call call;
    YmLattice coarse{}, fine{};
    int n_items = 0;
    int64_t chain_id_base = 0;
    CallPlan plan;
    void *dev_best_out = nullptr;
    void *dev_best_user = nullptr;
    uint32_t poll_serial = 0;
    uint32_t serial_counter = 0;
};

struct ProfEvents {
    std::vector<std::pair<hipEvent_t, hipEvent_t>> pairs;
    size_t used = 0;
    double ms = 0;
    int64_t launches = 0;
};

}
```

yag_slam_amd/csrc/ym_k_region.hpp:

```cpp
#pragma once

namespace ym {

#ifndef YM_RG_PROF
#define YM_RG_PROF 0
#endif
#if YM_RG_PROF
#if YM_RG_PROF == 2
#define YM_RG_PH(i) do { if ((i) == 7 || (i) == 8 || (i) == 1 || (i) == 2 || (i) == 5) { const uint32_t t_ = (uint32_t)__builtin_amdgcn_s_memtime(); \
    if ((i) != 5) ph[(i) == 7 ? 0 : (i) == 8 ? 1 : (i) == 1 ? 2 : 3] += t_ - pt; pt = t_; } } while (0)
#else
#define YM_RG_PH(i) do { const uint32_t t_ = (uint32_t)__builtin_amdgcn_s_memtime(); if ((i) >= 2 && (i) <= 5) ph[(i) - 2] += t_ - pt; pt = t_; } while (0)
#endif
#else
#define YM_RG_PH(i) do { } while (0)
#endif

#ifndef YM_RG_ABLATE
#define YM_RG_ABLATE 0
#endif
#ifndef YM_RG_PRIO
#define YM_RG_PRIO 0
#endif
#define YM_RG_W 64
#ifndef YM_RG_H
#define YM_RG_H 80
#endif
#define YM_RG_PITCH 100
#define YM_RG_ROWS (YM_RG_H + 26)
#define YM_RG_SEGS 6
#define YM_RG_CLS (YM_RG_PITCH * YM_RG_ROWS)
#define YM_RG_G 13
#define YM_RG_ZERO (4 * YM_RG_CLS)
#define YM_RG_LDS_BYTES (YM_RG_ZERO + 26 * YM_RG_PITCH + 32)
#define YM_RG_PLANES_SLACK(half_pitch) ((size_t)(2 * YM_RG_ROWS + 2 * YM_RG_H + 2) * (size_t)(half_pitch) + 256)
#define YM_RG_WINDOW_SLACK(pitch) ((size_t)(2 * YM_RG_ROWS + 2 * YM_RG_H + 2) * (size_t)(pitch) + 512)
static_assert(2 * YM_RG_ROWS + 2 * YM_RG_H + 2 >= 2 * (YM_RG_H - 1 + YM_RG_ROWS - 1) + 1 + 1, "YM_RG_PLANES_SLACK does not cover the rows a staged region reads");
static_assert(256 >= 16 * YM_RG_SEGS, "YM_RG_PLANES_SLACK does not cover the bytes a staged row reads");
static_assert(16 * YM_RG_SEGS >= YM_RG_W + 2 * YM_RG_G + 3 && YM_RG_PITCH >= 16 * YM_RG_SEGS && (YM_RG_PITCH / 4) % 2 == 1,
              "a staged row must hold the region, the patch margin and the misalignment, at an odd number of dwords per row");
#define YM_RG_MAX_BINS 8192
#define YM_RG_MAX_REGIONS 96
#define YM_RG_MAX_ENTRIES 28672
#define YM_RG_FLUSH 652
#define YM_BIN_THREADS 1024
#ifndef YM_BIN_MIN_WAVES
#define YM_BIN_MIN_WAVES 8
#endif
#define YM_BIN_LDS_BYTES(nbins, entries, nboxes) ((size_t)(YM_BIN_THREADS / 64 + YM_MAX_COARSE_NT + YM_RG_MAX_BINS / 32 + 1) * 4 + (size_t)(nbins) * 8 + ((size_t)(entries) * 2 + 15) / 16 * 16 + (size_t)(nboxes) * 16)

struct RegionArgs {
    YmGeom g;
    YmLattice lat;
    const uint8_t *grid;
    const uint8_t *planes;
    size_t grid_stride;
    const double2 *ctrig;
    const int32_t *hypcell;
    const YmItemState *states;
    const int32_t *qrep;
    uint16_t *entries;
    size_t entries_stride;
    int32_t *starts;
    size_t starts_stride;
    uint32_t *rbox;
    size_t rbox_stride;
    int32_t nw, parts;
    uint16_t *partial;
    size_t partial_stride;
    int32_t nt_stride, dim_stride;
    int32_t nrx, nry, ng, nbins;
    int32_t force_irregular;
    int32_t fuse_score;
    double *resp;
    size_t sums_stride;
    double *blockmax;
    double *probs;
    size_t probs_stride;
    int32_t n_blocks, pad;
    int32_t rg_h, rg_cls, rg_zero, pad2;
    int32_t rg_w, rg_pitch, nregions, pad3;
    uint32_t *walk;
    int32_t nitems, gpx;
    int32_t rsplit, pad4;
    unsigned long long *stamps;
    int32_t lnw, lparts;
    size_t entries_pstride;
};
__device__ __forceinline__ const int32_t *rg_part_starts(const RegionArgs &a, int qslot, int p) {
    return a.starts + (size_t)qslot * a.starts_stride + (size_t)p * (a.nbins + 1);
}
__device__ __forceinline__ bool rg_part_listed(const RegionArgs &a, int qslot, int p) {
    return a.starts[(size_t)qslot * a.starts_stride + (size_t)a.lparts * (a.nbins + 1) + p] >= 0;
}

__device__ __forceinline__ bool region_entry(const RegionArgs &a, int2 cell, int cx0, int cy0, int k, int &bin, unsigned &entry, int &region,
                                             unsigned &er, unsigned &ex, int bin_nw = -1) {
    const int X = cx0 + cell.x, Y = cy0 + cell.y;
    if (X < 0 || Y < 0) return false;
    const unsigned xc = (unsigned)X >> 1, yc = (unsigned)Y >> 1;
    const unsigned cls = (unsigned)((X & 1) | ((Y & 1) << 1));
#ifdef YM_EXPERIMENTAL
    if (a.rg_w) {
        const unsigned rx = xc / (unsigned)a.rg_w, ry = yc / (unsigned)a.rg_h;
        if ((int)rx >= a.nrx || (int)ry >= a.nry) return false;
        region = (int)((ry * (unsigned)a.nrx + rx) * 4u + cls);
        bin = region * a.lat.nt + k;
        er = yc - ry * (unsigned)a.rg_h;
        ex = xc - rx * (unsigned)a.rg_w;
        entry = er * (unsigned)a.rg_pitch + ex;
        return true;
    }
#endif
    if (yc >= 4096u) return false;
    const unsigned rx = xc / (unsigned)YM_RG_W, ry = __umul24(yc, (unsigned)a.pad2) >> 21;
    if ((int)rx >= a.nrx || (int)ry >= a.nry) return false;
    region = (int)(__umul24(ry, (unsigned)a.nrx) + rx);
    bin = (int)__umul24((unsigned)region, (unsigned)(bin_nw < 0 ? a.lat.nt : bin_nw)) + k;
    er = yc - __umul24(ry, (unsigned)a.rg_h);
    ex = xc - rx * YM_RG_W;
    entry = __umul24(cls, (unsigned)a.rg_cls) + __umul24(er, (unsigned)YM_RG_PITCH) + ex;
    return true;
}

#define YM_BINP_THREADS 512
#define YM_BINP_LDS_BYTES(nbins, entries, nboxes) ((size_t)(YM_BINP_THREADS / 64 + 16 + YM_RG_MAX_BINS / 32 + 1) * 4 + (size_t)(nbins) * 8 + ((size_t)(entries) * 2 + 15) / 16 * 16 + (size_t)(nboxes) * 16)
template <bool YAG, int MAXP>
__global__ __launch_bounds__(YM_BINP_THREADS, MAXP <= 18 ? 4 : 2) void bin_kernel(RegionArgs a) {
    constexpr int NT = YM_BINP_THREADS;
    extern __shared__ __attribute__((aligned(16))) unsigned char bin_smem[];
    int *wave_tot = reinterpret_cast<int *>(bin_smem);
    int *angle_tot = wave_tot + NT / 64;
    unsigned *region_bits = reinterpret_cast<unsigned *>(angle_tot + 16);
    int *regions_used = reinterpret_cast<int *>(region_bits + YM_RG_MAX_BINS / 32);
    unsigned (*cnt)[2] = reinterpret_cast<unsigned (*)[2]>(regions_used + 1);
    unsigned short *ent = reinterpret_cast<unsigned short *>(cnt + a.nbins);
    const int nboxes = a.nregions;
    unsigned (*box)[4] = reinterpret_cast<unsigned (*)[4]>(bin_smem + ((reinterpret_cast<unsigned char *>(ent + a.entries_pstride) - bin_smem) + 15) / 16 * 16);
    const int part = blockIdx.x, qs = blockIdx.y, b = a.qrep[qs], tid = threadIdx.x, lane = tid & 63;
    const YmItemState &st = a.states[b];
    const int nw = a.lnw, k_lo = part * nw, nk = min(a.lat.nt, k_lo + nw) - k_lo;
    const int nq = st.nq;
    const int total = nq * nk;
    const int32_t *cx = a.hypcell + (size_t)b * 2 * a.dim_stride;
    const int cx0 = cx[0], cy0 = cx[a.dim_stride];
    const double off_x = st.off_x, off_y = st.off_y;
    const double2 *ql = reinterpret_cast<const double2 *>(st.ql);
    const double2 *trig = a.ctrig + (size_t)b * a.nt_stride + k_lo;
    int32_t *starts = a.starts + (size_t)qs * a.starts_stride + (size_t)part * (a.nbins + 1);
    int32_t *flag = a.starts + (size_t)qs * a.starts_stride + (size_t)a.lparts * (a.nbins + 1) + part;
    const int pos0 = part * (int)a.entries_pstride;
    double2 *qls = reinterpret_cast<double2 *>(bin_smem + ((reinterpret_cast<unsigned char *>(ent) - bin_smem) + 15) / 16 * 16);
    const bool ql_in_lds = (size_t)(nq + nk) * sizeof(double2) + 16 <= (size_t)a.entries_pstride * 2;
    double2 *trigs = qls + nq;
    if (ql_in_lds) {
        for (int i = tid; i < nq; i += NT) qls[i] = ql[i];
        if (tid < nk) trigs[tid] = trig[tid];
    }
    for (int i = tid; i < a.nbins * 2; i += NT) (&cnt[0][0])[i] = 0u;
    if (tid < 16) angle_tot[tid] = 0;
    if (tid < YM_RG_MAX_BINS / 32) region_bits[tid] = 0u;
    if (tid == 0) *regions_used = 0;
    for (int i = tid; i < nboxes; i += NT) { box[i][0] = 255u; box[i][1] = 0u; box[i][2] = 255u; box[i][3] = 0u; }
    __syncthreads();
    unsigned key[MAXP];
    unsigned rank_hi[(MAXP + 3) / 4];
#pragma unroll
    for (int q = 0; q < (MAXP + 3) / 4; q++) rank_hi[q] = 0u;
    const int per_thread = (total + NT - 1) / NT;
    const int p0 = tid * per_thread;
    int k = p0 / max(nq, 1), i = p0 - k * nq;
    int cur = -1;
    unsigned r0 = 255u, r1 = 0u, x0 = 255u, x1 = 0u;
    auto send_box = [&]() {
        if (cur >= 0) {
            unsigned *bx = box[cur];
            atomicMin(&bx[0], r0); atomicMax(&bx[1], r1); atomicMin(&bx[2], x0); atomicMax(&bx[3], x1);
        }
    };
    bool overflow = per_thread > MAXP;
    auto pass1 = [&](auto point_of, auto trig_of) {
#pragma unroll
        for (int q = 0; q < MAXP; q++) {
            const int pp = p0 + q;
            key[q] = 0xffffffffu;
            if (q < per_thread && pp < total) {
                const double2 cs = trig_of(k);
                const double2 pt = point_of(i);
                int bin, region; unsigned e, er, ex;
                const int2 lc = YAG ? lookup_cell_sem(a.g, pt, cs.x, cs.y, off_x, off_y, st.ylat[0], st.ylat[1]) : lookup_cell(pt, cs.x, cs.y, off_x, off_y, a.g.scale);
                if (region_entry(a, lc, cx0, cy0, k, bin, e, region, er, ex, nw)) {
                    const unsigned rank = (atomicAdd(&cnt[bin][(e >> 1) & 1u], 1u << (16 * (e & 1u))) >> (16 * (e & 1u))) & 0xffffu;
                    key[q] = (rank & 7u) << 29 | (unsigned)bin << 16 | e;
                    rank_hi[q >> 2] |= ((rank >> 3) & 0xffu) << (8 * (q & 3));
                    if (region != cur) { send_box(); cur = region; r0 = r1 = er; x0 = x1 = ex; }
                    else { r0 = min(r0, er); r1 = max(r1, er); x0 = min(x0, ex); x1 = max(x1, ex); }
                }
            }
            if (++i >= nq) { i = 0; k++; }
        }
    };
    if (ql_in_lds) pass1([&](int i_) { return qls[i_]; }, [&](int k_) { return trigs[k_]; });
    else pass1([&](int i_) { return ql[i_]; }, [&](int k_) { return trig[k_]; });
    send_box();
    __syncthreads();
    {
        uint32_t *rb = a.rbox + (size_t)qs * a.rbox_stride;
        for (int r = tid; r < nboxes; r += NT) rb[(size_t)r * a.lparts + part] = box[r][0] | box[r][1] << 8 | box[r][2] << 16 | box[r][3] << 24;
    }
    const int per = (a.nbins + NT - 1) / NT;
    const int first = tid * per;
    int padded_total;
    {
        int local = 0;
        for (int j = 0; j < per; j++)
            if (first + j < a.nbins) {
                const unsigned c01 = cnt[first + j][0], c23 = cnt[first + j][1];
                const int c[4] = {(int)(c01 & 0xffffu), (int)(c01 >> 16), (int)(c23 & 0xffffu), (int)(c23 >> 16)};
                const int padded = (((c[0] + 1) & ~1) + ((c[1] + 1) & ~1) + ((c[2] + 1) & ~1) + ((c[3] + 1) & ~1) + 3) & ~3;
                local += padded;
                if (padded) {
                    atomicAdd(&angle_tot[(first + j) % nw], padded);
                    const int R = (first + j) / nw;
                    atomicOr(&region_bits[R >> 5], 1u << (R & 31));
                }
            }
        int incl = local;
#pragma unroll
        for (int d = 1; d < 64; d <<= 1) {
            const int v = __shfl_up(incl, d);
            if (lane >= d) incl += v;
        }
        if (lane == 63) wave_tot[tid >> 6] = incl;
        __syncthreads();
        if (tid < YM_RG_MAX_BINS / 32 && region_bits[tid]) atomicAdd(regions_used, __popc(region_bits[tid]));
        __syncthreads();
        int base = 0, all = 0;
        for (int w = 0; w < NT / 64; w++) {
            if (w < (tid >> 6)) base += wave_tot[w];
            all += wave_tot[w];
        }
        padded_total = all;
        bool fits = all <= (int)a.entries_pstride && pos0 + all <= 65532 && a.force_irregular != 2 && !overflow;
        for (int kk = 0; kk < nk; kk++) fits = fits && angle_tot[kk] <= a.ng * YM_RG_FLUSH;
        fits = fits && *regions_used <= YM_RG_MAX_REGIONS;
        int run = base + incl - local;
        for (int j = 0; j < per; j++)
            if (first + j < a.nbins) {
                const unsigned c01 = cnt[first + j][0], c23 = cnt[first + j][1];
                const int c[4] = {(int)(c01 & 0xffffu), (int)(c01 >> 16), (int)(c23 & 0xffffu), (int)(c23 >> 16)};
                starts[first + j] = pos0 + run;
                int pos = run;
                unsigned fill[4];
                for (int r = 0; r < 4; r++) {
                    fill[r] = (unsigned)pos;
                    if (fits && (c[r] & 1)) ent[pos + c[r]] = (unsigned short)(a.rg_zero + r);
                    pos += (c[r] + 1) & ~1;
                }
                if (fits && ((pos - run) & 3)) { ent[pos] = (unsigned short)a.rg_zero; ent[pos + 1] = (unsigned short)a.rg_zero; }
                pos = run + ((pos - run + 3) & ~3);
                cnt[first + j][0] = fill[0] | fill[1] << 16;
                cnt[first + j][1] = fill[2] | fill[3] << 16;
                run = pos;
            }
        if (tid == 0) {
            starts[a.nbins] = pos0 + all;
            *flag = fits ? all : -1;
            if (a.stamps && qs == 0 && part == 0) a.stamps[26] = (unsigned long long)all;
        }
        if (!fits) return;
    }
    __syncthreads();
#pragma unroll
    for (int q = 0; q < MAXP; q++) {
        if (key[q] == 0xffffffffu) continue;
        const unsigned bin = (key[q] >> 16) & 0x1fffu, e = key[q] & 0xffffu;
        const unsigned rank = key[q] >> 29 | ((rank_hi[q >> 2] >> (8 * (q & 3))) & 0xffu) << 3;
        const unsigned f = cnt[bin][(e >> 1) & 1u];
        ent[((e & 1u) ? f >> 16 : f & 0xffffu) + rank] = (unsigned short)e;
    }
    __syncthreads();
    uint32_t *out = reinterpret_cast<uint32_t *>(a.entries + (size_t)qs * a.entries_stride + pos0);
    const uint32_t *src = reinterpret_cast<const uint32_t *>(ent);
    for (int i2 = tid; i2 < (padded_total + 1) / 2; i2 += NT) out[i2] = src[i2];
}

typedef unsigned int rg_u32x2 __attribute__((ext_vector_type(2)));
__device__ __forceinline__ void rg_perm_pair(const rg_u32x2 &pa, const rg_u32x2 &qa, const rg_u32x2 &pb, const rg_u32x2 &qb, uint32_t rr,
                                             uint32_t (&e)[4], uint32_t (&o)[4]) {
    const uint32_t s0 = pa.x + pb.x, s1 = pa.y + pb.y, s2 = qa.x + qb.x, s3 = qa.y + qb.y;
    const uint32_t selE = rr * 0x00010001u + 0x0c020c00u, selO = selE + 0x00010001u;
    e[0] = __builtin_amdgcn_perm(s1, s0, selE); o[0] = __builtin_amdgcn_perm(s1, s0, selO);
    e[1] = __builtin_amdgcn_perm(s2, s1, selE); o[1] = __builtin_amdgcn_perm(s2, s1, selO);
    e[2] = __builtin_amdgcn_perm(s3, s2, selE); o[2] = __builtin_amdgcn_perm(s3, s2, selO);
    e[3] = __builtin_amdgcn_perm(0u, s3, selE);
    o[3] = 0u;
}
__device__ __forceinline__ void rg_gather4(uint32_t (&acc)[8], uint32_t lane_off, uint2 ee ) {
    const uint32_t ad0 = lane_off + (ee.x & 0xffffu), ad1 = lane_off + (ee.x >> 16), ad2 = lane_off + (ee.y & 0xffffu), ad3 = lane_off + (ee.y >> 16);
#if YM_RG_ABLATE & 1
    acc[0] += ad0 ^ ad1 ^ ad2 ^ ad3;
    return;
#endif
    rg_u32x2 p0, q0, p1, q1, p2, q2, p3, q3;
    asm volatile("ds_read2_b32 %0, %8 offset1:1\n\tds_read2_b32 %1, %8 offset0:2 offset1:3\n\t"
                 "ds_read2_b32 %2, %9 offset1:1\n\tds_read2_b32 %3, %9 offset0:2 offset1:3\n\t"
                 "ds_read2_b32 %4, %10 offset1:1\n\tds_read2_b32 %5, %10 offset0:2 offset1:3\n\t"
                 "ds_read2_b32 %6, %11 offset1:1\n\tds_read2_b32 %7, %11 offset0:2 offset1:3\n\t"
                 "s_waitcnt lgkmcnt(4)"
                 : "=&v"(p0), "=&v"(q0), "=&v"(p1), "=&v"(q1), "=&v"(p2), "=&v"(q2), "=&v"(p3), "=&v"(q3)
                 : "v"(ad0 & ~3u), "v"(ad1 & ~3u), "v"(ad2 & ~3u), "v"(ad3 & ~3u)
                 : "memory");
    uint32_t e[2][4], o[2][4];
    rg_perm_pair(p0, q0, p1, q1, ad0 & 3u, e[0], o[0]);
    asm volatile("s_waitcnt lgkmcnt(0)" : "+v"(p2), "+v"(q2), "+v"(p3), "+v"(q3) : : "memory");
    rg_perm_pair(p2, q2, p3, q3, ad2 & 3u, e[1], o[1]);
#pragma unroll
    for (int j = 0; j < 4; j++) {
        acc[2 * j] = acc[2 * j] + e[0][j] + e[1][j];
        if (j < 3) acc[2 * j + 1] = acc[2 * j + 1] + o[0][j] + o[1][j];
    }
}

__device__ __forceinline__ void rg_odd(uint32_t (&)[8]) {}

template <int NW, bool WIN = false>
__global__ __launch_bounds__(64 * NW, NW <= 8 ? (3 * NW + 3) / 4 : 1 ) void correlate_region_kernel(RegionArgs a) {
    constexpr int NT = 64 * NW;
    constexpr int PER = (YM_RG_ROWS + (NT / 4) / YM_RG_SEGS - 1) / ((NT / 4) / YM_RG_SEGS);
    __shared__ __attribute__((aligned(16))) unsigned char region[YM_RG_LDS_BYTES];
    __shared__ int rlist[YM_RG_MAX_REGIONS];
    __shared__ uint32_t rboxl[YM_RG_MAX_REGIONS];
    __shared__ unsigned short seginfo[NW][YM_RG_MAX_REGIONS][2];
    __shared__ int rcount;
    int p;
    const int b = xcd_item_of_block_2d(p);
    const int rsplit = a.rsplit > 1 ? a.rsplit : 1, rsi = p / a.parts;
    p -= rsi * a.parts;
    const int tid = threadIdx.x, lane = tid & 63, wave = __builtin_amdgcn_readfirstlane(tid >> 6);
    const YmItemState &st = a.states[b];
    const int nt = a.lat.nt, nx = a.lat.nx, ny = a.lat.ny, ng = a.ng;
    const int k = p * NW + wave;
    const bool kvalid = k < nt;
    const int row = lane & 31, half = lane >> 5;
    const bool job = row < ny && half * YM_RG_G < nx;
    const int half_pitch = a.g.pitch / 2;
    const int plane_bytes = half_pitch * a.g.win_w;
    const uint8_t *__restrict__ planes = a.planes + (size_t)b * a.grid_stride;
    const int32_t *__restrict__ starts = rg_part_starts(a, st.qslot, p);
    const uint16_t *__restrict__ entries = a.entries + (size_t)st.qslot * a.entries_stride;
    const uint32_t lds0 = (uint32_t)(size_t)region;
    const uint32_t lane_off = lds0 + (uint32_t)((job ? row : 0) * YM_RG_PITCH + (half * YM_RG_G < nx ? half * YM_RG_G : 0));
    uint32_t acc[8];
#pragma unroll
    for (int j = 0; j < 8; j++) acc[j] = 0u;
    int in_set = 0, flushed = 0;
    auto flush = [&]() {
        if (flushed < ng) {
            rg_odd(acc);
            store_partial16(a.partial + (size_t)b * a.partial_stride + (((size_t)(rsi * ng + flushed) * nt + k) * 64 + lane) * 16, acc);
        }
#pragma unroll
        for (int j = 0; j < 8; j++) acc[j] = 0u;
        flushed++;
        in_set = 0;
    };
#if !YM_RG_PROF
    YM_STAMP(a, 8);
#endif
#if YM_RG_PROF
    uint32_t ph[4] = {0u, 0u, 0u, 0u};
    uint32_t pt = (uint32_t)__builtin_amdgcn_s_memtime();
    const uint32_t pt_begin = pt;
    const unsigned long long rt_begin = __builtin_amdgcn_s_memrealtime();
#endif
    const bool regular = st.regular[0] && a.force_irregular != 1 && rg_part_listed(a, st.qslot, p);
    if (regular) {
        const int k_lo = p * NW, k_hi = min(nt, k_lo + NW);
        const int nreg = a.nrx * a.nry;
        for (int i = tid; i < (YM_RG_LDS_BYTES - YM_RG_ZERO) / 4; i += NT) reinterpret_cast<uint32_t *>(region + YM_RG_ZERO)[i] = 0u;
        if (wave == 0) {
            int n = 0;
            for (int R0 = 0; R0 < nreg; R0 += 64) {
                const int R = R0 + lane;
                const bool has = R < nreg && starts[(size_t)R * NW] != starts[(size_t)R * NW + (k_hi - k_lo)];
                const unsigned long long mask = __ballot(has);
                const int at = n + __popcll(mask & ((1ull << lane) - 1ull));
                if (has && at % rsplit == rsi) rlist[at / rsplit] = R;
                n += __popcll(mask);
            }
            if (lane == 0) rcount = n > rsi ? (n - rsi + rsplit - 1) / rsplit : 0;
        }
        __syncthreads();
        const int nlist = rcount;
        {
            const uint32_t *rb = a.rbox + (size_t)st.qslot * a.rbox_stride;
            const uint32_t reach = (uint32_t)(nx > YM_RG_G ? 15 + YM_RG_G : 15);
            for (int i = tid; i < nlist; i += NT) {
                const uint32_t v = rb[(size_t)rlist[i] * a.parts + p];
                const uint32_t r0 = v & 0xffu, r1 = min((uint32_t)(YM_RG_ROWS - 1), ((v >> 8) & 0xffu) + (uint32_t)ny - 1u);
                const uint32_t s0 = ((v >> 16) & 0xfcu) >> 4, s1 = min((uint32_t)(YM_RG_SEGS - 1), ((v >> 24) + reach) >> 4);
                rboxl[i] = r0 | r1 << 8 | s0 << 16 | s1 << 24;
            }
        }
        if (kvalid)
            for (int i = lane; i < nlist; i += 64) {
                const int32_t *srow = starts + (size_t)rlist[i] * NW + wave;
                seginfo[wave][i][0] = (unsigned short)srow[0]; seginfo[wave][i][1] = (unsigned short)srow[1];
            }
        __syncthreads();
        constexpr int TPC = WIN ? NT / 2 : NT / 4;
        constexpr int NSEG = WIN ? 2 * YM_RG_SEGS : YM_RG_SEGS;
        constexpr int LPS = TPC / NSEG;
        constexpr int RSTEP = LPS;
        static_assert(LPS >= 1 && LPS * PER >= YM_RG_ROWS, "the copy tasks must cover a class image");
        const uint32_t cls = WIN ? 2u * ((uint32_t)tid / TPC) : (uint32_t)tid / TPC, j = (uint32_t)tid % TPC;
        const uint32_t seg = j % NSEG, r0 = j / NSEG;
        const bool copier = j < (uint32_t)(LPS * NSEG);
        const uint32_t src0 = WIN ? (2u * r0 + (cls >> 1)) * (uint32_t)a.g.pitch + 16u * seg
                                  : (cls & 1u) * (uint32_t)plane_bytes + (2u * r0 + (cls >> 1)) * (uint32_t)half_pitch + 16u * seg;
        const uint32_t src_step = WIN ? 2u * RSTEP * (uint32_t)a.g.pitch : 2u * RSTEP * (uint32_t)half_pitch;
        const uint32_t dst0 = (cls * YM_RG_ROWS + r0) * YM_RG_PITCH + (WIN ? 8u : 16u) * seg;
        uint4 v[PER];
        auto in_box = [&](int q, uint32_t bx, bool seg_in) {
            (void)q; (void)bx;
            return seg_in;
        };
        auto band_in = [&](int q, uint32_t bx) {
            return (uint32_t)(q * RSTEP) <= ((bx >> 8) & 0xffu) && (uint32_t)(q * RSTEP + RSTEP - 1) >= (bx & 0xffu);
        };
        const uint8_t *__restrict__ window = a.grid + (size_t)b * a.grid_stride;
        auto seg_inside = [&](uint32_t bx) {
            return WIN ? copier && seg >= 2u * ((bx >> 16) & 0xffu) && seg <= 2u * (bx >> 24) + 1u
                       : copier && seg >= ((bx >> 16) & 0xffu) && seg <= (bx >> 24);
        };
        auto stage_load = [&](int R, uint32_t bx) {
            const int RX = R % a.nrx, RY = R / a.nrx;
            const uint8_t *src = WIN ? window + ((size_t)(2 * RY * YM_RG_H) * a.g.pitch + (size_t)RX * (2 * YM_RG_W))
                                     : planes + ((size_t)(2 * RY * YM_RG_H) * half_pitch + (size_t)RX * YM_RG_W);
            const bool seg_in = seg_inside(bx);
#pragma unroll
            for (int q = 0; q < PER; q++)
#if YM_RG_ABLATE & 2
                v[q] = make_uint4((uint32_t)(size_t)src, seg_in, bx, q);
#else
                if (band_in(q, bx)) v[q] = *reinterpret_cast<const uint4 *>(src + (in_box(q, bx, seg_in) ? src0 + (uint32_t)q * src_step : 0u));
#endif
        };
        auto stage_store = [&](uint32_t bx) {
            const bool seg_in = seg_inside(bx);
#pragma unroll
            for (int q = 0; q < PER; q++) {
                uint32_t *d = reinterpret_cast<uint32_t *>(region + dst0 + (uint32_t)(q * RSTEP * YM_RG_PITCH));
                if (band_in(q, bx) && in_box(q, bx, seg_in) && (!(YM_RG_ABLATE & 4) || v[q].x == 0x12345u)) {
                    if (WIN) {
                        d[0] = __builtin_amdgcn_perm(v[q].y, v[q].x, 0x06040200u); d[1] = __builtin_amdgcn_perm(v[q].w, v[q].z, 0x06040200u);
                        d[YM_RG_CLS / 4] = __builtin_amdgcn_perm(v[q].y, v[q].x, 0x07050301u); d[YM_RG_CLS / 4 + 1] = __builtin_amdgcn_perm(v[q].w, v[q].z, 0x07050301u);
                    } else { d[0] = v[q].x; d[1] = v[q].y; d[2] = v[q].z; d[3] = v[q].w; }
                }
            }
        };
        auto segment = [&](int ri, int &t0, int &t2) {
            t0 = t2 = 0;
            if (kvalid) {
                t0 = __builtin_amdgcn_readfirstlane((int)seginfo[wave][ri][0]);
                t2 = __builtin_amdgcn_readfirstlane((int)seginfo[wave][ri][1]);
            }
        };
        const uint2 *__restrict__ entries4 = reinterpret_cast<const uint2 *>(entries);
        uint2 ev = make_uint2(0u, 0u), cev = make_uint2(0u, 0u);
        auto entries_load = [&](int t0, int t2) {
            ev = make_uint2(0u, 0u);
            if (t0 + 4 * lane < t2) ev = entries4[(t0 >> 2) + lane];
        };
        auto gather = [&](int lo, int hi) {
            const int lds_hi = min(hi, lo + 256);
#if YM_RG_PRIO
            {
                const int n = hi - lo;
                if (n >= 3 * YM_RG_PRIO) __builtin_amdgcn_s_setprio(3);
                else if (n >= 2 * YM_RG_PRIO) __builtin_amdgcn_s_setprio(2);
                else if (n >= YM_RG_PRIO) __builtin_amdgcn_s_setprio(1);
            }
#endif
            if (lo < lds_hi) {
                const int n4 = (lds_hi - lo) >> 2;
                for (int c = 0; c < n4; c++) {
                    rg_gather4(acc, lane_off, make_uint2(__builtin_amdgcn_readlane(cev.x, c), __builtin_amdgcn_readlane(cev.y, c)));
                    in_set += 4;
                    if (in_set == YM_RG_FLUSH) flush();
                }
            }
            for (int c = lds_hi; c < hi; c += 4) {
                rg_gather4(acc, lane_off, entries4[c >> 2]);
                in_set += 4;
                if (in_set == YM_RG_FLUSH) flush();
            }
#if YM_RG_PRIO
            __builtin_amdgcn_s_setprio(0);
#endif
        };
        int s0 = 0, s2 = 0;
        if (nlist > 0) {
            const uint32_t bx = __builtin_amdgcn_readfirstlane(rboxl[0]);
            segment(0, s0, s2);
            entries_load(s0, s2);
            stage_load(rlist[0], bx);
            stage_store(bx);
            cev = ev;
        }
        __syncthreads();
        YM_RG_PH(0);
        for (int ri = 0; ri < nlist; ri++) {
            const bool has_next = ri + 1 < nlist;
            int n0 = 0, n2 = 0;
            uint32_t nbx = 0u;
            if (has_next) {
                nbx = __builtin_amdgcn_readfirstlane(rboxl[ri + 1]);
                segment(ri + 1, n0, n2);
                YM_RG_PH(7);
                entries_load(n0, n2);
                YM_RG_PH(8);
                stage_load(rlist[ri + 1], nbx);
            }
            YM_RG_PH(1);
            gather(s0, s2);
            YM_RG_PH(2);
            __syncthreads();
            YM_RG_PH(3);
            if (has_next) {
                stage_store(nbx);
                cev = ev;
            }
            s0 = n0; s2 = n2;
            YM_RG_PH(4);
            __syncthreads();
            YM_RG_PH(5);
        }
    } else if (kvalid && job && rsi == 0) {
        const uint8_t *__restrict__ grid = a.grid + (size_t)b * a.grid_stride;
        const unsigned limit = (unsigned)(a.g.pitch * a.g.win_w);
        const int32_t *cx = a.hypcell + (size_t)b * 2 * a.dim_stride;
        const int32_t *cy = cx + a.dim_stride;
        const double2 cs = a.ctrig[(size_t)b * a.nt_stride + k];
        const double2 *ql = reinterpret_cast<const double2 *>(st.ql);
        const int nq = st.nq;
        const double add_x = a.g.semantics == 1 ? st.ylat[0] : st.off_x, add_y = a.g.semantics == 1 ? st.ylat[1] : st.off_y;
        for (int g = 0; g < ng; g++) {
            for (int j = 0; j < YM_RG_G; j++) {
                const int ix = half * YM_RG_G + j;
                if (ix >= nx) break;
                const int base = cy[row] * lin_pitch(a.g) + cx[ix];
                unsigned sum = 0;
                const int i1 = min(nq, (g + 1) * YM_RG_FLUSH);
                for (int i = g * YM_RG_FLUSH; i < i1; i++)
                    sum += cell_value(a.g, grid, limit, (unsigned)(base + lookup_offset_sem(a.g, ql[i], cs.x, cs.y, st.off_x, st.off_y, add_x, add_y, lin_pitch(a.g))));
                acc[2 * (j >> 2) + (j & 1)] += sum << (16 * ((j >> 1) & 1));
            }
            flush();
        }
    }
#if !YM_RG_PROF
    YM_STAMP(a, 9);
#endif
#if YM_RG_PROF
    auto prof_out = [&]() {
        if (a.stamps && lane == 0) {
            for (int i = 0; i < 4; i++) atomicAdd(a.stamps + 10 + i, (unsigned long long)ph[i]);
            atomicAdd(a.stamps + 8, (unsigned long long)(pt - pt_begin));
            atomicAdd(a.stamps + 9, __builtin_amdgcn_s_memrealtime() - rt_begin);
        }
    };
#endif
    if (!a.fuse_score) {
        if (!kvalid) return;
        while (flushed < ng) flush();
        return;
    }
    unsigned long long *pmax = reinterpret_cast<unsigned long long *>(region);
    const int nxy = nx * ny;
    double *dpen = reinterpret_cast<double *>(region) + ((nxy + 1) & ~1);
    __syncthreads();
    for (int i = tid; i < nxy; i += NT) {
        pmax[i] = 0ull;
        const int iy = i / nx, ix = i - iy * nx;
        const double x = -a.lat.off_x + ix * a.lat.step_x, y = -a.lat.off_y + iy * a.lat.step_y;
        dpen[i] = dist_penalty(a.g, x * x + y * y);
    }
    __syncthreads();
    if (kvalid) {
        unsigned tot[YM_RG_G];
        rg_odd(acc);
// ... 43 lines not shown
```

yag_slam_amd/scan_matching.py:

```python
import ctypes as C
import os
import struct
from collections import namedtuple

import numpy as np

from . import _capi
from .config import default_config, default_config_loop, make_config
from .models import LocalizedRangeScan
from .transform import Transform

ScanMatcherResult = namedtuple('ScanMatcherResult', ['response', 'covariance', 'best_pose', 'meta'])


def _pose_of(scan):
    p = scan.corrected_pose
    return float(p.x), float(p.y), float(p.euler[-1])


def _desc_of(scan, keep):
    d = _capi.YmScanDesc()
    r = np.ascontiguousarray(scan.ranges, dtype=np.float64)
    keep.append(r)
    d.ranges = r.ctypes.data_as(C.POINTER(C.c_double))
# ... 222 lines not shown
        if not queries:
            return BatchResults(np.zeros(0, dtype=_RESULT_DTYPE))
        flat, offs = [], [0]
        for ch in chains:
            flat.extend(ch)
            offs.append(len(flat))
        hq = (C.c_void_p * len(queries))(*self._handles(queries))
        hs = (C.c_void_p * max(1, len(flat)))(*self._handles(flat))
        co = (C.c_int32 * len(offs))(*offs)
        per = (_capi.YmResult * len(chains))()
        _capi.check(self._lib.ym_match_pairs(self._m, hq, hs, co, len(chains), int(bool(penalty)), int(bool(do_fine)), per))
        return _results(per, check=True)

    def make_pairs_batch(self, queries, chains):
        return MatchBatch(self, queries, chains, pairs=True)

    def _handles(self, scans):
        dev, out = self.device, []
        for s in scans:
            h = getattr(s, "_native", None)
            if h is None or getattr(s, "_native_device", None) != dev or not isinstance(s, LocalizedRangeScan):
                h = self._require_native(s)
            out.append(h)
        return out

    def _require_native(self, scan):
        h = self._native(scan)
        if h is None:
            raise TypeError("match_scan_batch needs yag_slam_amd.models.LocalizedRangeScan instances")
        return h

    def coarse_dims(self):
        d = (C.c_int32 * 3)()
        _capi.check(self._lib.ym_coarse_dims(self._m, d))
        return tuple(d[:])

    def slice_begin(self, query, base_scans, penalty, do_fine, k_begin, k_end, dev_resp, dev_probs):
        hq = self._require_native(query)
        arr = (C.c_void_p * max(1, len(base_scans)))(*self._handles(base_scans))
        _capi.check(self._lib.ym_match_slice_begin(self._m, hq, arr, len(base_scans), int(bool(penalty)), int(bool(do_fine)),
                                                   int(k_begin), int(k_end), C.c_void_p(dev_resp), C.c_void_p(dev_probs)))

    def slice_finish(self):
        res = _capi.YmResult()
        _capi.check(self._lib.ym_match_slice_finish(self._m, C.byref(res)))
        if res.status != 0:
            raise _capi.YmError(res.status, "Mapper FATAL ERROR - unable to find best position / index out of range")
        return _result(res)

    def correlation_grid_from_occupancy(self, map_im, occupied_value=0):
        im = np.ascontiguousarray(map_im, dtype=np.uint8)
        if im.ndim != 2:
            raise ValueError("occupancy image must be 2-D")
        h = self._lib.ym_map_from_occupancy(self._m, im.ctypes.data_as(C.POINTER(C.c_uint8)), im.shape[1], im.shape[0],
                                            im.strides[0], int(occupied_value))
        if not h:
            raise _capi.YmError(-1, _capi.last_error())
        return CorrelationMap(self, h)

    def upload_correlation_grid(self, cgrid):
        g = np.ascontiguousarray(cgrid, dtype=np.float64)
        if g.ndim != 2:
            raise ValueError("correlation grid must be 2-D")
        h = self._lib.ym_map_from_grid(self._m, g.ctypes.data_as(C.POINTER(C.c_double)), g.shape[1], g.shape[0])
        if not h:
            raise _capi.YmError(-1, _capi.last_error())
        return CorrelationMap(self, h)

    def match_scan_sets_with_map(self, cgrid, ox, oy, query_scans, penalty=True, do_fine=True, coarse=None):
        own = not isinstance(cgrid, CorrelationMap)
        mp = self.upload_correlation_grid(cgrid) if own else cgrid
        try:
            hs = (C.c_void_p * len(query_scans))(*[self._require_native(q) for q in query_scans])
            cs = None
            if coarse:
                cs = _capi.YmMapSearch(float(coarse.get("xy_search", 0.25)), float(coarse.get("xy_step", 0.01)),
                                       float(coarse.get("angle_search", 0.1)), float(coarse.get("angle_step", 0.01)),
                                       float(coarse.get("grid_resolution", 0.05)), int(bool(coarse.get("penalize", False))), 0)
            res = _capi.YmResult()
            _capi.check(self._lib.ym_match_map(self._m, mp._h, float(ox), float(oy), hs, len(query_scans), int(bool(penalty)),
                                               int(bool(do_fine)), C.byref(cs) if cs else None, C.byref(res)))
        finally:
            if own:
                mp.close()
        if res.status != 0:
            raise _capi.YmError(res.status, "empty search lattice or no query point")
        r = _result(res)
        xs = [float(q.corrected_pose.x) for q in query_scans]
        ys = [float(q.corrected_pose.y) for q in query_scans]
        oxy = Transform.from_position_euler(sum(xs) / float(len(xs)), sum(ys) / float(len(ys)), 0, 0, 0, 0)
        diff = r.best_pose - oxy
        r.meta["centre"] = (oxy.x, oxy.y, 0.0)
        r.meta["corrected_centre"] = (r.best_pose.x, r.best_pose.y, r.best_pose.euler[-1])
        return ScanMatcherResult(r.response, r.covariance, [q.corrected_pose + diff for q in query_scans], r.meta)

    def match_scan_async(self, query, base_scans, penalty=True, do_fine=False, slot=0):
        hq = self._require_native(query)
        arr = (C.c_void_p * max(1, len(base_scans)))(*self._handles(base_scans))
        _capi.check(self._lib.ym_match_scans_async(self._m, hq, arr, len(base_scans), int(bool(penalty)),
                                                   int(bool(do_fine)), int(slot)))

    def wait(self, slot=0):
        res = _capi.YmResult()
        _capi.check(self._lib.ym_wait(self._m, int(slot), C.byref(res)))
        return _result(res)

    def synchronize(self):
        _capi.check(self._lib.ym_synchronize(self._m))

    def set_stream(self, stream_handle):
        _capi.check(self._lib.ym_set_stream(self._m, C.c_void_p(stream_handle) if stream_handle else None))

    def debug_grid(self, item=0):
        info = _capi.YmGridInfo()
        _capi.check(self._lib.ym_debug_grid_info(self._m, item, C.byref(info)))
        buf = np.zeros((info.height, info.pitch), dtype=np.uint8)
        _capi.check(self._lib.ym_debug_grid(self._m, item, buf.ctypes.data_as(C.POINTER(C.c_uint8)), buf.size))
        return buf[:, :info.width], info

    def debug_sums(self, pass_=0, item=0, dims=None):
        nx, ny, nt = dims
        buf = np.zeros((nt, ny, nx), dtype=np.uint32)
        _capi.check(self._lib.ym_debug_sums(self._m, item, pass_, buf.ctypes.data_as(C.POINTER(C.c_uint32)), buf.size))
        return buf

    def debug_query_local(self, item=0, cap=8192):
        buf = np.zeros((cap, 2))
        n = C.c_int32()
        _capi.check(self._lib.ym_debug_query_local(self._m, item, buf.ctypes.data_as(C.POINTER(C.c_double)), cap,
                                                   C.byref(n)))
        return buf[:n.value].copy()

    def debug_cells(self, item=0, cap=1 << 16):
        buf = np.zeros((cap, 2), dtype=np.int32)
        max_n = C.c_int32()
        _capi.check(self._lib.ym_debug_cells(self._m, item, buf.ctypes.data_as(C.POINTER(C.c_int32)), buf.size,
                                             C.byref(max_n)))
        return buf.reshape(-1, 2), max_n.value

    def debug_option(self, option, value):
        _capi.check(self._lib.ym_debug_option(self._m, int(option), int(value)))

    def debug_stamps(self, enable=True):
        buf = (C.c_uint64 * 32)()
        _capi.check(self._lib.ym_debug_stamps(self._m, int(bool(enable)), buf, 32))
        return list(buf)

    def cache_stats(self):
        h, ms = C.c_int64(0), C.c_int64(0)
        _capi.check(self._lib.ym_cache_stats(self._m, C.byref(h), C.byref(ms)))
        return int(h.value), int(ms.value)

    def debug_counters(self):
        buf = (C.c_int64 * 8)()
        _capi.check(self._lib.ym_debug_counters(self._m, buf, 8))
        return dict(yag_fast_items=int(buf[0]), yag_fallback_items=int(buf[1]), yag_pairs_checked=int(buf[2]),
                    yag_pairs_failed=int(buf[3]), list_cache_hits=int(buf[4]),
                    last_correlate={-1: None, 0: "correlate_kernel", 1: "correlate_region_kernel", 2: "gather_kernel"}[int(buf[5])])

    def profile(self, on=True):
        _capi.check(self._lib.ym_profile_enable(self._m, int(bool(on))))

    def profile_read(self, which=0, reset=True):
        ms, n = C.c_double(), C.c_int64()
        _capi.check(self._lib.ym_profile_read(self._m, which, C.byref(ms), C.byref(n), int(bool(reset))))
        return ms.value, n.value


class CorrelationMap(object):

    def __init__(self, matcher, handle):
        self.m, self._h = matcher, handle
        w, h = C.c_int32(), C.c_int32()
        _capi.check(matcher._lib.ym_map_size(handle, C.byref(w), C.byref(h)))
        self.shape = (h.value, w.value)

    def to_numpy(self):
        out = np.empty(self.shape, dtype=np.float64)
        _capi.check(self.m._lib.ym_map_read(self._h, out.ctypes.data_as(C.POINTER(C.c_double)), out.size))
        return out

    def close(self):
        if getattr(self, "_h", None):
            self.m._lib.ym_map_destroy(self._h)
            self._h = None

    def __del__(self):
        try:
            self.close()
        except Exception:
            pass


class MatchBatch(object):

    def __init__(self, matcher, query, chains, pairs=False):
        self.m = matcher
        self.query = query
        self.chains = [list(c) for c in chains]
        self._queries = list(query) if pairs else [query]
        if pairs and len(self._queries) != len(self.chains):
            raise ValueError("a pairs batch needs one chain per query")
        flat, offs = [], [0]
        for ch in self.chains:
            flat.extend(ch)
            offs.append(len(flat))
        self._flat = flat
        hs = (C.c_void_p * max(1, len(flat)))(*matcher._handles(flat))
        co = (C.c_int32 * len(offs))(*offs)
        if pairs:
            hq = (C.c_void_p * max(1, len(self._queries)))(*matcher._handles(self._queries))
            self._h = matcher._lib.ym_pairs_create(matcher._m, hq, hs, co, len(self.chains))
        else:
            hq = matcher._require_native(query)
            self._h = matcher._lib.ym_batch_create(matcher._m, hq, hs, co, len(self.chains))
        if not self._h:
            raise _capi.YmError(-1, _capi.last_error())
        self.n = len(self.chains)

    @classmethod
    def from_handles(cls, matcher, query_handles, scan_handles, offsets):
        self = cls.__new__(cls)
        self.m, self.query, self.chains, self._queries, self._flat = matcher, None, None, None, None
        qh = np.ascontiguousarray(query_handles, dtype=np.uint64)
        sh = np.ascontiguousarray(scan_handles, dtype=np.uint64)
        co = np.ascontiguousarray(offsets, dtype=np.int32)
        if co.shape[0] != qh.shape[0] + 1:
            raise ValueError("a pairs batch needs one chain per query")
        self._h = matcher._lib.ym_pairs_create(matcher._m, qh.ctypes.data_as(C.POINTER(C.c_void_p)), sh.ctypes.data_as(C.POINTER(C.c_void_p)),
                                               co.ctypes.data_as(C.POINTER(C.c_int32)), int(qh.shape[0]))
        if not self._h:
            raise _capi.YmError(-1, _capi.last_error())
        self.n = int(qh.shape[0])
        return self

    def close(self):
        if getattr(self, "_h", None):
            try:
                self.m._lib.ym_batch_destroy(self._h)
            except Exception:
                pass
            self._h = None

    def __del__(self):
        self.close()

    def push_poses(self):
        scans = self._queries + self._flat
        hs = self.m._handles(scans)
        xyz = np.array([_pose_of(s) for s in scans], dtype=np.float64).reshape(len(scans), 3)
        _capi.check(self.m._lib.ym_scans_set_poses((C.c_void_p * len(hs))(*hs), xyz.ctypes.data_as(C.POINTER(C.c_double)), len(hs)))

    def run_async(self, penalty=False, do_fine=False, slot=0, chain_id_base=0, dev_best_out=None):
        _capi.check(self.m._lib.ym_batch_run_async(self.m._m, self._h, int(bool(penalty)), int(bool(do_fine)), int(slot),
                                                   int(chain_id_base), C.c_void_p(dev_best_out) if dev_best_out else None))

    def wait(self, slot=0, per_chain=True):
        per = (_capi.YmResult * self.n)() if per_chain else None
        best = _capi.YmResult()
        bi = C.c_int32(-1)
        _capi.check(self.m._lib.ym_batch_wait(self.m._m, int(slot), per, C.byref(best), C.byref(bi)))
        return (_results(per, check=True) if per_chain else None), _result(best), int(bi.value)


Scan2DMatcherCpp = ScanMatcher
Scan2DMatcher = ScanMatcher
```

Before: 13.46 billion.

## Anchor region grid at per-part minimum cell to cut occupied regions

Measured after the change: 13.69 billion (median of 6 runs). +1.7%, better.

```diff
diff --git a/include/yagmatch.h b/include/yagmatch.h
--- a/include/yagmatch.h
+++ b/include/yagmatch.h
@@ -187,8 +187,10 @@
 
 int ym_debug_option(ym_matcher *m, int option, int value);
 
-#define YM_DEBUG_COUNTERS 8
+#define YM_DEBUG_COUNTERS 12
+#define YM_REGION_TOTALS 5
 int ym_debug_counters(ym_matcher *m, int64_t *out, int32_t count);
+int ym_debug_region_rounds(ym_matcher *m, int32_t *out, int64_t out_count, int32_t *parts, int32_t *items);
 
 int ym_debug_stamps(ym_matcher *m, int enable, uint64_t *out, int32_t count);
 
diff --git a/yag_slam_amd/_capi.py b/yag_slam_amd/_capi.py
--- a/yag_slam_amd/_capi.py
+++ b/yag_slam_amd/_capi.py
@@ -17,7 +17,7 @@
     "ym_batch_run_async", "ym_batch_wait", "ym_debug_grid_info",
     "ym_debug_grid", "ym_debug_sums", "ym_debug_query_local", "ym_debug_cells", "ym_debug_option", "ym_debug_stamps",
     "ym_profile_enable",
-    "ym_profile_read", "ym_cache_stats", "ym_debug_counters",
+    "ym_profile_read", "ym_cache_stats", "ym_debug_counters", "ym_debug_region_rounds",
     "ym_coarse_dims", "ym_match_slice_begin", "ym_match_slice_finish",
     "ym_occupancy_create", "ym_occupancy_get_info", "ym_occupancy_read", "ym_occupancy_destroy",
     "ym_map_from_occupancy", "ym_map_from_grid", "ym_map_size", "ym_map_read", "ym_map_destroy", "ym_match_map",
@@ -178,6 +178,7 @@
     L.ym_profile_read.argtypes = [vp, C.c_int, dp, C.POINTER(C.c_int64), C.c_int]
     L.ym_cache_stats.argtypes = [vp, C.POINTER(C.c_int64), C.POINTER(C.c_int64)]
     L.ym_debug_counters.argtypes = [vp, C.POINTER(C.c_int64), C.c_int32]
+    L.ym_debug_region_rounds.argtypes = [vp, C.POINTER(C.c_int32), C.c_int64, C.POINTER(C.c_int32), C.POINTER(C.c_int32)]
     L.ym_coarse_dims.argtypes = [vp, ip]
     L.ym_scan_structure_trusted.argtypes = [vp, C.c_int]
     L.ym_process_scan.argtypes = [vp, vp, C.POINTER(vp), C.c_int, dp, dp, C.c_int, C.c_int, C.POINTER(YmResult)]
diff --git a/yag_slam_amd/csrc/ym_abi_debug.hpp b/yag_slam_amd/csrc/ym_abi_debug.hpp
--- a/yag_slam_amd/csrc/ym_abi_debug.hpp
+++ b/yag_slam_amd/csrc/ym_abi_debug.hpp
@@ -102,6 +102,8 @@
     else if (option == 45) { m->list_cache_on = value != 0; m->list_key_valid = false; }
     else if (option == 46) m->yag_fast = value < 0 ? 0 : value > 2 ? 1 : value;
     else if (option == 43) m->rg2_h = value;
+    else if (option == 47) m->rg_fixed_grid = value != 0;
+    else if (option == 48) m->rg_count = value != 0;
     else if (option == 44) {
 #ifndef YM_EXPERIMENTAL
         return set_err(YM_ERR_UNSUPPORTED, "correlate_region2_kernel is compiled only into builds made with -DYM_EXPERIMENTAL");
@@ -183,6 +185,58 @@
     return YM_OK;
 }
 
+static int region_rounds(ym_matcher *m, int32_t *out, int64_t out_count, int64_t *totals) {
+    const ym_matcher::LastLists &L = m->last_lists;
+    for (int i = 0; i < YM_REGION_TOTALS; i++) totals[i] = 0;
+    if (out && out_count < (int64_t)L.B * L.lparts * 2) return set_err(YM_ERR_INVALID, "buffer too small: need %lld ints", (long long)L.B * L.lparts * 2);
+    DEV_GUARD(m->device);
+    HIP_TRY(hipStreamSynchronize(m->stream));
+    std::vector<YmItemState> states(L.B);
+    HIP_TRY(hipMemcpy(states.data(), m->states.p, sizeof(YmItemState) * L.B, hipMemcpyDeviceToHost));
+    int nq = 0;
+    for (const YmItemState &s : states) nq = std::max(nq, s.qslot + 1);
+    std::vector<int32_t> starts((size_t)nq * L.starts_stride);
+    HIP_TRY(hipMemcpy(starts.data(), m->rg_starts.p, starts.size() * sizeof(int32_t), hipMemcpyDeviceToHost));
+    const int NT = 64 * L.nw, TPC = L.win ? NT / 2 : NT / 4, NSEG = L.win ? 2 * YM_RG_SEGS : YM_RG_SEGS, LPS = TPC / NSEG;
+    const int PER = (YM_RG_ROWS + (NT / 4) / YM_RG_SEGS - 1) / ((NT / 4) / YM_RG_SEGS);
+    const int64_t row_bytes = L.win ? L.pitch : L.pitch / 2, plane_bytes = (int64_t)(L.pitch / 2) * L.win_w;
+    const int64_t reach = (int64_t)(2 * (LPS * PER - 1) + 1) * row_bytes + 16 * NSEG + (L.win ? 0 : plane_bytes);
+    int64_t lo = INT64_MAX, hi = 0;
+    for (int b = 0; b < L.B; b++) {
+        const int32_t *row = starts.data() + (size_t)states[b].qslot * L.starts_stride;
+        const int32_t *meta = row + (size_t)L.lparts * (L.nbins + 1);
+        for (int p = 0; p < L.lparts; p++) {
+            const bool listed = states[b].regular[0] && meta[p] >= 0;
+            const int regions = listed ? meta[2 * L.lparts + p] : 0, maxima = listed ? meta[3 * L.lparts + p] : 0;
+            if (out) { out[((size_t)b * L.lparts + p) * 2] = regions; out[((size_t)b * L.lparts + p) * 2 + 1] = maxima; }
+            totals[0] += regions; totals[1] += maxima;
+            if (!listed) continue;
+            const int64_t ox = (uint32_t)meta[L.lparts + p] & 0xffffu, oy = (uint32_t)meta[L.lparts + p] >> 16;
+            const int32_t *st = row + (size_t)p * (L.nbins + 1);
+            const int nk = std::min(L.nt, (p + 1) * L.lnw) - p * L.lnw;
+            for (int R = 0; R < L.nbins / L.lnw; R++) {
+                if (st[(size_t)R * L.lnw] == st[(size_t)R * L.lnw + nk]) continue;
+                const int64_t X0 = (int64_t)(R % L.nrx) * YM_RG_W + ox, Y0 = (int64_t)(R / L.nrx) * YM_RG_H + oy;
+                const int64_t first = (int64_t)b * (int64_t)L.grid_stride + 2 * Y0 * row_bytes + (L.win ? 2 * X0 : X0);
+                lo = std::min(lo, first); hi = std::max(hi, first + reach);
+            }
+        }
+    }
+    totals[2] = lo == INT64_MAX ? 0 : lo; totals[3] = hi;
+    totals[4] = (int64_t)L.B * (int64_t)L.grid_stride + (int64_t)L.slack;
+    return YM_OK;
+}
+
+int ym_debug_region_rounds(ym_matcher *m, int32_t *out, int64_t out_count, int32_t *parts, int32_t *items) {
+    if (!m || !parts || !items) return set_err(YM_ERR_INVALID, "null argument");
+    if (!m->rg_count) return set_err(YM_ERR_INVALID, "the rounds are counted only with debug option 48 = 1");
+    if (!m->last_valid || m->last_lists.B <= 0) return set_err(YM_ERR_INVALID, "the last call did not take the region correlate");
+    *parts = m->last_lists.lparts; *items = m->last_lists.B;
+    if (!out) return YM_OK;
+    int64_t t[YM_REGION_TOTALS];
+    return region_rounds(m, out, out_count, t);
+}
+
 int ym_debug_counters(ym_matcher *m, int64_t *out, int32_t count) {
     if (!m || !out || count < 0) return set_err(YM_ERR_INVALID, "bad argument");
     int64_t v[YM_DEBUG_COUNTERS];
@@ -196,6 +250,12 @@
     }
     v[4] = m->list_cache_hits;
     v[5] = m->last_corr_form;
+    if (m->rg_count && m->last_valid && m->last_lists.B > 0) {
+        int64_t t[YM_REGION_TOTALS];
+        int rc = region_rounds(m, nullptr, 0, t);
+        if (rc) return rc;
+        for (int i = 0; i < YM_REGION_TOTALS; i++) v[6 + i] = t[i];
+    }
     for (int i = 0; i < std::min<int>(count, YM_DEBUG_COUNTERS); i++) out[i] = v[i];
     return YM_OK;
 }
diff --git a/yag_slam_amd/csrc/ym_host_call.hpp b/yag_slam_amd/csrc/ym_host_call.hpp
--- a/yag_slam_amd/csrc/ym_host_call.hpp
+++ b/yag_slam_amd/csrc/ym_host_call.hpp
@@ -8,6 +8,7 @@
     int rc;
     mark(0);
     m->last_corr_form = -1;
+    m->last_lists = ym_matcher::LastLists();
     if ((rc = plan_sizes(m, slot, P))) return rc;
     mark(1);
     Call &pc = slot.call;
@@ -43,7 +44,7 @@
         if (keyed) {
             key.qid = q0->id; key.pose[0] = q0->pose[0]; key.pose[1] = q0->pose[1]; key.pose[2] = q0->pose[2];
             key.g = P.g; key.lc = P.lc; key.nw = P.rg_nw; key.parts = P.rg_parts; key.nrx = P.rg_nrx; key.nry = P.rg_nry;
-            key.rg_h = P.rg2 ? P.rg2_h : YM_RG_H; key.force = m->corr_region; key.nregions = P.rg_nregions; key.ng = P.rg_ng;
+            key.rg_h = P.rg2 ? P.rg2_h : YM_RG_H; key.force = m->corr_region; key.nregions = P.rg_nregions; key.ng = P.rg_ng; key.place = P.rg_place;
             key.es = P.rg_entries_stride; key.ss = P.rg_starts_stride;
             key.pe = m->rg_entries.p; key.ps = m->rg_starts.p; key.pb = m->rg_rbox.p;
             P.lists_cached = m->list_key_valid && std::memcmp(&key, &m->list_key, sizeof key) == 0;
diff --git a/yag_slam_amd/csrc/ym_host_enqueue.hpp b/yag_slam_amd/csrc/ym_host_enqueue.hpp
--- a/yag_slam_amd/csrc/ym_host_enqueue.hpp
+++ b/yag_slam_amd/csrc/ym_host_enqueue.hpp
@@ -187,8 +187,8 @@
 #endif
     if (P.rg2) { r.rg_h = P.rg2_h; r.rg_cls = YM_RG_PITCH * (P.rg2_h + 26); r.rg_zero = 4 * r.rg_cls; }
     r.pad2 = ((1 << 21) + r.rg_h - 1) / r.rg_h;
-    r.rg_w = 0; r.rg_pitch = YM_RG_PITCH; r.nregions = P.rg_nregions; r.pad3 = 0;
-    r.walk = m->rg_walk.p; r.nitems = P.B; r.rsplit = P.rg_rsplit; r.pad4 = 0;
+    r.rg_w = 0; r.rg_pitch = YM_RG_PITCH; r.nregions = P.rg_nregions; r.count_maxima = m->rg_count ? 1 : 0;
+    r.walk = m->rg_walk.p; r.nitems = P.B; r.rsplit = P.rg_rsplit; r.place = P.rg_place;
     r.lnw = P.rg_lnw; r.lparts = P.rg_lparts; r.entries_pstride = P.rg_entries_pstride;
     r.gpx = std::max(1, std::min((2 * std::max(m->n_cus, 8) / 8) / std::max(1, P.rg_parts), (P.B + 7) / 8));
     return r;
@@ -256,6 +256,13 @@
     int rc;
     hipEvent_t ev_k = nullptr;
     m->last_corr_form = P.region26 ? 1 : P.region ? 2 : 0;
+    m->last_lists = ym_matcher::LastLists();
+    if (P.region26 && P.rg_lparts == P.rg_parts) {
+        ym_matcher::LastLists &L = m->last_lists;
+        L.B = P.B; L.lparts = P.rg_lparts; L.nbins = P.rg_nbins; L.lnw = P.rg_lnw; L.nrx = P.rg_nrx; L.nt = P.lc.nt; L.pitch = P.g.pitch;
+        L.win_w = P.g.win_w; L.win = P.win_only ? 1 : 0; L.nw = P.rg_nw; L.starts_stride = P.rg_starts_stride; L.grid_stride = P.grid_stride;
+        L.slack = P.rg_src_slack;
+    }
     if (P.region26) {
         const ym::RegionArgs r = region_args(m, P);
         if (P.lists_on_side_stream) HIP_TRY(hipStreamWaitEvent(st, m->ev_join, 0));
diff --git a/yag_slam_amd/csrc/ym_host_matcher.hpp b/yag_slam_amd/csrc/ym_host_matcher.hpp
--- a/yag_slam_amd/csrc/ym_host_matcher.hpp
+++ b/yag_slam_amd/csrc/ym_host_matcher.hpp
@@ -91,11 +91,14 @@
     int corr_region_form = 0;
     struct ListKey {
         uint64_t qid; double pose[3]; YmGeom g; YmLattice lc;
-        int32_t nw, parts, nrx, nry, rg_h, force, nregions, ng; size_t es, ss; const void *pe, *ps, *pb;
+        int32_t nw, parts, nrx, nry, rg_h, force, nregions, ng, place, pad; size_t es, ss; const void *pe, *ps, *pb;
     };
     ListKey list_key;
     bool list_key_valid = false, list_cache_on = true;
     int64_t list_cache_hits = 0;
+    int rg_count = 0;
+    int rg_fixed_grid = 0;
+    struct LastLists { int B = 0, lparts = 0, nbins = 0, lnw = 0, nrx = 0, nt = 0, pitch = 0, win_w = 0, win = 0, nw = 0; size_t starts_stride = 0, grid_stride = 0, slack = 0; } last_lists;
     int rg2_min_batch = 1 << 30;
     int rg2_h = 128;
     size_t rg2_lds_limit = 0;
diff --git a/yag_slam_amd/csrc/ym_host_plan.hpp b/yag_slam_amd/csrc/ym_host_plan.hpp
--- a/yag_slam_amd/csrc/ym_host_plan.hpp
+++ b/yag_slam_amd/csrc/ym_host_plan.hpp
@@ -162,7 +162,8 @@
             P.rg_nbins = P.rg_nregions * P.rg_lnw;
             P.rg_entries_pstride = std::min((size_t)YM_RG_MAX_ENTRIES, ((size_t)P.rg_lnw * max_n * 11 / 10 + 63) / 64 * 64);
             P.rg_entries_stride = P.rg_entries_pstride * P.rg_lparts;
-            P.rg_starts_stride = ((size_t)P.rg_lparts * (P.rg_nbins + 1) + P.rg_lparts + 15) / 16 * 16;
+            P.rg_starts_stride = (YM_RG_STARTS_WORDS(P.rg_lparts, P.rg_nbins) + 15) / 16 * 16;
+            P.rg_place = whole || m->rg_fixed_grid ? 0 : P.win_only ? 8 : 16;
         }
     }
     P.region = !wrap && !P.region26 && (!yag || lc.nx > 0) && !call.slice && P.sx == 2 && B >= m->lds_min_batch && m->corr_region != 1 && lc.nx <= 16 * YM_GA_MAX_SEG && lc.ny <= 64;
@@ -271,6 +272,7 @@
     window_slack = std::max(window_slack, YM_R2_WINDOW_SLACK(g.pitch, 128));
     planes_slack = std::max(planes_slack, YM_WS_PLANES_SLACK(g.pitch / 2));
 #endif
+    P.rg_src_slack = P.win_only ? window_slack : planes_slack;
     if ((rc = m->grid.ensure((size_t)B * P.grid_stride + window_slack))) return rc;
     if ((rc = m->planes.ensure((size_t)B * P.grid_stride + std::max(planes_slack, YM_GA_PLANES_SLACK(g.pitch / 2, std::max(P.ga_rows, P.ga_nry + P.ga_H), lc.ny, P.ga_P))))) return rc;
     if ((rc = m->ctrig.ensure((size_t)B * P.nt_stride))) return rc;
diff --git a/yag_slam_amd/csrc/ym_host_types.hpp b/yag_slam_amd/csrc/ym_host_types.hpp
--- a/yag_slam_amd/csrc/ym_host_types.hpp
+++ b/yag_slam_amd/csrc/ym_host_types.hpp
@@ -169,6 +169,8 @@
     bool rg2 = false;
     int rg2_h = 0;
     size_t rg_entries_stride = 0, rg_starts_stride = 0, rg_entries_pstride = 0;
+    int rg_place = 0;
+    size_t rg_src_slack = 0;
     int rg_lnw = 0, rg_lparts = 1;
     bool region = false;
     int ga_W = 0, ga_H = 0, ga_P = 0, ga_rows = 0, ga_nrx = 0, ga_nry = 0, ga_nseg = 1, ga_np = 1, ga_ng = 1, ga_parts = 1, ga_kpp = 1;
diff --git a/yag_slam_amd/csrc/ym_k_region.hpp b/yag_slam_amd/csrc/ym_k_region.hpp
--- a/yag_slam_amd/csrc/ym_k_region.hpp
+++ b/yag_slam_amd/csrc/ym_k_region.hpp
@@ -37,6 +37,7 @@
 #define YM_RG_WINDOW_SLACK(pitch) ((size_t)(2 * YM_RG_ROWS + 2 * YM_RG_H + 2) * (size_t)(pitch) + 512)
 static_assert(2 * YM_RG_ROWS + 2 * YM_RG_H + 2 >= 2 * (YM_RG_H - 1 + YM_RG_ROWS - 1) + 1 + 1, "YM_RG_PLANES_SLACK does not cover the rows a staged region reads");
 static_assert(256 >= 16 * YM_RG_SEGS, "YM_RG_PLANES_SLACK does not cover the bytes a staged row reads");
+static_assert(512 >= 2 * 16 * YM_RG_SEGS, "YM_RG_WINDOW_SLACK does not cover the bytes a staged window row reads");
 static_assert(16 * YM_RG_SEGS >= YM_RG_W + 2 * YM_RG_G + 3 && YM_RG_PITCH >= 16 * YM_RG_SEGS && (YM_RG_PITCH / 4) % 2 == 1,
               "a staged row must hold the region, the patch margin and the misalignment, at an odd number of dwords per row");
 #define YM_RG_MAX_BINS 8192
@@ -79,10 +80,12 @@
     size_t probs_stride;
     int32_t n_blocks, pad;
     int32_t rg_h, rg_cls, rg_zero, pad2;
-    int32_t rg_w, rg_pitch, nregions, pad3;
+    int32_t rg_w, rg_pitch, nregions;
+    int32_t count_maxima;
     uint32_t *walk;
     int32_t nitems, gpx;
-    int32_t rsplit, pad4;
+    int32_t rsplit;
+    int32_t place;
     unsigned long long *stamps;
     int32_t lnw, lparts;
     size_t entries_pstride;
@@ -93,11 +96,15 @@
 __device__ __forceinline__ bool rg_part_listed(const RegionArgs &a, int qslot, int p) {
     return a.starts[(size_t)qslot * a.starts_stride + (size_t)a.lparts * (a.nbins + 1) + p] >= 0;
 }
-
-__device__ __forceinline__ bool region_entry(const RegionArgs &a, int2 cell, int cx0, int cy0, int k, int &bin, unsigned &entry, int &region,
-                                             unsigned &er, unsigned &ex, int bin_nw = -1) {
-    const int X = cx0 + cell.x, Y = cy0 + cell.y;
-    if (X < 0 || Y < 0) return false;
+#define YM_RG_STARTS_WORDS(lparts, nbins) ((size_t)(lparts) * ((size_t)(nbins) + 1) + 4 * (size_t)(lparts))
+__device__ __forceinline__ uint32_t rg_part_origin(const RegionArgs &a, int qslot, int p) {
+    return (uint32_t)a.starts[(size_t)qslot * a.starts_stride + (size_t)a.lparts * (a.nbins + 1) + a.lparts + p];
+}
+
+template <bool TRUSTED = false>
+__device__ __forceinline__ bool region_entry_xy(const RegionArgs &a, int X, int Y, int k, int &bin, unsigned &entry, int &region,
+                                                unsigned &er, unsigned &ex, int bin_nw = -1, unsigned ox = 0u, unsigned oy = 0u) {
+    if (!TRUSTED && (X < 0 || Y < 0)) return false;
     const unsigned xc = (unsigned)X >> 1, yc = (unsigned)Y >> 1;
     const unsigned cls = (unsigned)((X & 1) | ((Y & 1) << 1));
 #ifdef YM_EXPERIMENTAL
@@ -112,19 +119,24 @@
         return true;
     }
 #endif
-    if (yc >= 4096u) return false;
-    const unsigned rx = xc / (unsigned)YM_RG_W, ry = __umul24(yc, (unsigned)a.pad2) >> 21;
+    if (!TRUSTED && (yc >= 4096u || xc < ox || yc < oy)) return false;
+    const unsigned xr = xc - ox, yr = yc - oy;
+    const unsigned rx = xr / (unsigned)YM_RG_W, ry = __umul24(yr, (unsigned)a.pad2) >> 21;
     if ((int)rx >= a.nrx || (int)ry >= a.nry) return false;
     region = (int)(__umul24(ry, (unsigned)a.nrx) + rx);
     bin = (int)__umul24((unsigned)region, (unsigned)(bin_nw < 0 ? a.lat.nt : bin_nw)) + k;
-    er = yc - __umul24(ry, (unsigned)a.rg_h);
-    ex = xc - rx * YM_RG_W;
+    er = yr - __umul24(ry, (unsigned)a.rg_h);
+    ex = xr - rx * YM_RG_W;
     entry = __umul24(cls, (unsigned)a.rg_cls) + __umul24(er, (unsigned)YM_RG_PITCH) + ex;
     return true;
 }
+__device__ __forceinline__ bool region_entry(const RegionArgs &a, int2 cell, int cx0, int cy0, int k, int &bin, unsigned &entry, int &region,
+                                             unsigned &er, unsigned &ex, int bin_nw = -1) {
+    return region_entry_xy(a, cx0 + cell.x, cy0 + cell.y, k, bin, entry, region, er, ex, bin_nw);
+}
 
 #define YM_BINP_THREADS 512
-#define YM_BINP_LDS_BYTES(nbins, entries, nboxes) ((size_t)(YM_BINP_THREADS / 64 + 16 + YM_RG_MAX_BINS / 32 + 1) * 4 + (size_t)(nbins) * 8 + ((size_t)(entries) * 2 + 15) / 16 * 16 + (size_t)(nboxes) * 16)
+#define YM_BINP_LDS_BYTES(nbins, entries, nboxes) ((size_t)(YM_BINP_THREADS / 64 + 16 + YM_RG_MAX_BINS / 32 + 4) * 4 + (size_t)(nbins) * 8 + ((size_t)(entries) * 2 + 15) / 16 * 16 + (size_t)(nboxes) * 16)
 template <bool YAG, int MAXP>
 __global__ __launch_bounds__(YM_BINP_THREADS, MAXP <= 18 ? 4 : 2) void bin_kernel(RegionArgs a) {
     constexpr int NT = YM_BINP_THREADS;
@@ -133,7 +145,8 @@
     int *angle_tot = wave_tot + NT / 64;
     unsigned *region_bits = reinterpret_cast<unsigned *>(angle_tot + 16);
     int *regions_used = reinterpret_cast<int *>(region_bits + YM_RG_MAX_BINS / 32);
-    unsigned (*cnt)[2] = reinterpret_cast<unsigned (*)[2]>(regions_used + 1);
+    int *origin_min = regions_used + 1, *maxima = regions_used + 3;
+    unsigned (*cnt)[2] = reinterpret_cast<unsigned (*)[2]>(regions_used + 4);
     unsigned short *ent = reinterpret_cast<unsigned short *>(cnt + a.nbins);
     const int nboxes = a.nregions;
     unsigned (*box)[4] = reinterpret_cast<unsigned (*)[4]>(bin_smem + ((reinterpret_cast<unsigned char *>(ent + a.entries_pstride) - bin_smem) + 15) / 16 * 16);
@@ -160,7 +173,7 @@
     for (int i = tid; i < a.nbins * 2; i += NT) (&cnt[0][0])[i] = 0u;
     if (tid < 16) angle_tot[tid] = 0;
     if (tid < YM_RG_MAX_BINS / 32) region_bits[tid] = 0u;
-    if (tid == 0) *regions_used = 0;
+    if (tid == 0) { *regions_used = 0; origin_min[0] = origin_min[1] = 0x7fffffff; *maxima = 0; }
     for (int i = tid; i < nboxes; i += NT) { box[i][0] = 255u; box[i][1] = 0u; box[i][2] = 255u; box[i][3] = 0u; }
     __syncthreads();
     unsigned key[MAXP];
@@ -169,7 +182,37 @@
     for (int q = 0; q < (MAXP + 3) / 4; q++) rank_hi[q] = 0u;
     const int per_thread = (total + NT - 1) / NT;
     const int p0 = tid * per_thread;
-    int k = p0 / max(nq, 1), i = p0 - k * nq;
+    const int k_first = p0 / max(nq, 1), i_first = p0 - k_first * nq;
+    bool overflow = per_thread > MAXP;
+    int mnx = 0x7fffffff, mny = 0x7fffffff;
+    auto pass0 = [&](auto point_of, auto trig_of) {
+        int k = k_first, i = i_first;
+#pragma unroll
+        for (int q = 0; q < MAXP; q++) {
+            const int pp = p0 + q;
+            key[q] = 0xffffffffu;
+            if (q < per_thread && pp < total) {
+                const double2 cs = trig_of(k);
+                const double2 pt = point_of(i);
+                const int2 lc = YAG ? lookup_cell_sem(a.g, pt, cs.x, cs.y, off_x, off_y, st.ylat[0], st.ylat[1]) : lookup_cell(pt, cs.x, cs.y, off_x, off_y, a.g.scale);
+                const int X = cx0 + lc.x, Y = cy0 + lc.y;
+                if ((unsigned)X < 16384u && (unsigned)Y < 8192u) {
+                    key[q] = (unsigned)X | (unsigned)Y << 14 | (unsigned)k << 27;
+                    mnx = min(mnx, X); mny = min(mny, Y);
+                }
+            }
+            if (++i >= nq) { i = 0; k++; }
+        }
+    };
+    if (ql_in_lds) pass0([&](int i_) { return qls[i_]; }, [&](int k_) { return trigs[k_]; });
+    else pass0([&](int i_) { return ql[i_]; }, [&](int k_) { return trig[k_]; });
+    unsigned ox = 0u, oy = 0u;
+    if (a.place) {
+        mnx = wave_reduce(mnx, OpMinI()); mny = wave_reduce(mny, OpMinI());
+        if (lane == 0) { atomicMin(&origin_min[0], mnx); atomicMin(&origin_min[1], mny); }
+        __syncthreads();
+        if (origin_min[0] != 0x7fffffff) { ox = ((unsigned)origin_min[0] >> 1) & ~(unsigned)(a.place - 1); oy = (unsigned)origin_min[1] >> 1; }
+    }
     int cur = -1;
     unsigned r0 = 255u, r1 = 0u, x0 = 255u, x1 = 0u;
     auto send_box = [&]() {
@@ -178,18 +221,14 @@
             atomicMin(&bx[0], r0); atomicMax(&bx[1], r1); atomicMin(&bx[2], x0); atomicMax(&bx[3], x1);
         }
     };
-    bool overflow = per_thread > MAXP;
-    auto pass1 = [&](auto point_of, auto trig_of) {
+    {
 #pragma unroll
         for (int q = 0; q < MAXP; q++) {
-            const int pp = p0 + q;
-            key[q] = 0xffffffffu;
-            if (q < per_thread && pp < total) {
-                const double2 cs = trig_of(k);
-                const double2 pt = point_of(i);
+            if (key[q] != 0xffffffffu) {
                 int bin, region; unsigned e, er, ex;
-                const int2 lc = YAG ? lookup_cell_sem(a.g, pt, cs.x, cs.y, off_x, off_y, st.ylat[0], st.ylat[1]) : lookup_cell(pt, cs.x, cs.y, off_x, off_y, a.g.scale);
-                if (region_entry(a, lc, cx0, cy0, k, bin, e, region, er, ex, nw)) {
+                const int X = (int)(key[q] & 0x3fffu), Y = (int)((key[q] >> 14) & 0x1fffu), k = (int)(key[q] >> 27);
+                key[q] = 0xffffffffu;
+                if (region_entry_xy<true>(a, X, Y, k, bin, e, region, er, ex, nw, ox, oy)) {
                     const unsigned rank = (atomicAdd(&cnt[bin][(e >> 1) & 1u], 1u << (16 * (e & 1u))) >> (16 * (e & 1u))) & 0xffffu;
                     key[q] = (rank & 7u) << 29 | (unsigned)bin << 16 | e;
                     rank_hi[q >> 2] |= ((rank >> 3) & 0xffu) << (8 * (q & 3));
@@ -197,16 +236,23 @@
                     else { r0 = min(r0, er); r1 = max(r1, er); x0 = min(x0, ex); x1 = max(x1, ex); }
                 }
             }
-            if (++i >= nq) { i = 0; k++; }
-        }
-    };
-    if (ql_in_lds) pass1([&](int i_) { return qls[i_]; }, [&](int k_) { return trigs[k_]; });
-    else pass1([&](int i_) { return ql[i_]; }, [&](int k_) { return trig[k_]; });
+        }
+    }
     send_box();
     __syncthreads();
     {
         uint32_t *rb = a.rbox + (size_t)qs * a.rbox_stride;
-        for (int r = tid; r < nboxes; r += NT) rb[(size_t)r * a.lparts + part] = box[r][0] | box[r][1] << 8 | box[r][2] << 16 | box[r][3] << 24;
+        int msum = 0;
+        for (int r = tid; r < nboxes; r += NT) {
+            rb[(size_t)r * a.lparts + part] = box[r][0] | box[r][1] << 8 | box[r][2] << 16 | box[r][3] << 24;
+            unsigned mx = 0u;
+            for (int kk = 0; kk < (a.count_maxima ? nk : 0); kk++) {
+                const unsigned c01 = cnt[r * nw + kk][0], c23 = cnt[r * nw + kk][1];
+                mx = max(mx, (c01 & 0xffffu) + (c01 >> 16) + (c23 & 0xffffu) + (c23 >> 16));
+            }
+            msum += (int)mx;
+        }
+        if (msum) atomicAdd(maxima, msum);
     }
     const int per = (a.nbins + NT - 1) / NT;
     const int first = tid * per;
@@ -266,6 +312,9 @@
         if (tid == 0) {
             starts[a.nbins] = pos0 + all;
             *flag = fits ? all : -1;
+            flag[a.lparts] = (int32_t)(ox | oy << 16);
+            flag[2 * a.lparts] = *regions_used;
+            flag[3 * a.lparts] = *maxima;
             if (a.stamps && qs == 0 && part == 0) a.stamps[26] = (unsigned long long)all;
         }
         if (!fits) return;
@@ -348,6 +397,7 @@
     const int plane_bytes = half_pitch * a.g.win_w;
     const uint8_t *__restrict__ planes = a.planes + (size_t)b * a.grid_stride;
     const int32_t *__restrict__ starts = rg_part_starts(a, st.qslot, p);
+    const uint32_t origin = __builtin_amdgcn_readfirstlane(rg_part_origin(a, st.qslot, p));
     const uint16_t *__restrict__ entries = a.entries + (size_t)st.qslot * a.entries_stride;
     const uint32_t lds0 = (uint32_t)(size_t)region;
     const uint32_t lane_off = lds0 + (uint32_t)((job ? row : 0) * YM_RG_PITCH + (half * YM_RG_G < nx ? half * YM_RG_G : 0));
@@ -414,6 +464,7 @@
         constexpr int LPS = TPC / NSEG;
         constexpr int RSTEP = LPS;
         static_assert(LPS >= 1 && LPS * PER >= YM_RG_ROWS, "the copy tasks must cover a class image");
+        static_assert(2 * (LPS * PER - 1) + 1 + 1 <= 2 * YM_RG_ROWS + 2 * YM_RG_H + 2, "YM_RG_WINDOW_SLACK / YM_RG_PLANES_SLACK do not cover the rows the copy tasks read");
         const uint32_t cls = WIN ? 2u * ((uint32_t)tid / TPC) : (uint32_t)tid / TPC, j = (uint32_t)tid % TPC;
         const uint32_t seg = j % NSEG, r0 = j / NSEG;
         const bool copier = j < (uint32_t)(LPS * NSEG);
@@ -436,8 +487,9 @@
         };
         auto stage_load = [&](int R, uint32_t bx) {
             const int RX = R % a.nrx, RY = R / a.nrx;
-            const uint8_t *src = WIN ? window + ((size_t)(2 * RY * YM_RG_H) * a.g.pitch + (size_t)RX * (2 * YM_RG_W))
-                                     : planes + ((size_t)(2 * RY * YM_RG_H) * half_pitch + (size_t)RX * YM_RG_W);
+            const uint32_t X0 = (uint32_t)(RX * YM_RG_W) + (origin & 0xffffu), Y0 = (uint32_t)(RY * YM_RG_H) + (origin >> 16);
+            const uint8_t *src = WIN ? window + ((size_t)(2u * Y0) * a.g.pitch + (size_t)(2u * X0))
+                                     : planes + ((size_t)(2u * Y0) * half_pitch + (size_t)X0);
             const bool seg_in = seg_inside(bx);
 #pragma unroll
             for (int q = 0; q < PER; q++)
diff --git a/yag_slam_amd/scan_matching.py b/yag_slam_amd/scan_matching.py
--- a/yag_slam_amd/scan_matching.py
+++ b/yag_slam_amd/scan_matching.py
@@ -398,11 +398,21 @@
         return int(h.value), int(ms.value)
 
     def debug_counters(self):
-        buf = (C.c_int64 * 8)()
-        _capi.check(self._lib.ym_debug_counters(self._m, buf, 8))
-        return dict(yag_fast_items=int(buf[0]), yag_fallback_items=int(buf[1]), yag_pairs_checked=int(buf[2]),
+        buf = (C.c_int64 * 12)()
+        _capi.check(self._lib.ym_debug_counters(self._m, buf, 12))
+        return dict(region_rounds=int(buf[6]), region_round_maxima=int(buf[7]), region_stage_first_byte=int(buf[8]),
+                    region_stage_end_byte=int(buf[9]), region_stage_bytes_kept=int(buf[10]),
+                    yag_fast_items=int(buf[0]), yag_fallback_items=int(buf[1]), yag_pairs_checked=int(buf[2]),
                     yag_pairs_failed=int(buf[3]), list_cache_hits=int(buf[4]),
                     last_correlate={-1: None, 0: "correlate_kernel", 1: "correlate_region_kernel", 2: "gather_kernel"}[int(buf[5])])
+
+    def debug_region_rounds(self):
+        parts, items = C.c_int32(), C.c_int32()
+        _capi.check(self._lib.ym_debug_region_rounds(self._m, None, 0, C.byref(parts), C.byref(items)))
+        cap = 2 * parts.value * items.value
+        buf = np.zeros(cap, dtype=np.int32)
+        _capi.check(self._lib.ym_debug_region_rounds(self._m, buf.ctypes.data_as(C.POINTER(C.c_int32)), cap, C.byref(parts), C.byref(items)))
+        return buf.reshape(-1, parts.value, 2)
 
     def profile(self, on=True):
         _capi.check(self._lib.ym_profile_enable(self._m, int(bool(on))))
```
